# khiner/MeshEditor

Hardware: AMD Instinct MI355X
Metric: eigenpairs/sec (K/M assembly + 50-mode solve, 100k-tet mesh) (higher is better)
Workload: dtype f64; 1 GPU; cube_s100k: Kuhn mesh 105456 tets / 446631 DOF, NumModes=50 NumFemModes=65, P=10 excitation points, one mesh per GPU; eigenpairs_per_mesh=65, kept_modes_per_mesh=50, parallelism=mesh-per-gpu x1

## Files before the change

### mesheditor_amd/csrc/mh_common.h

```cpp
#pragma once
#include "../../include/modalhip.h"

#include <hip/hip_runtime.h>
#include <rocblas/rocblas.h>
#include <rocsolver/rocsolver.h>

#include <algorithm>
#include <cstdarg>
#include <cstdio>
#include <cstdlib>
#include <cstring>
#include <iterator>
#include <limits>
#include <map>
#include <mutex>
#include <stdexcept>
#include <string>
#include <vector>

struct MhError : std::runtime_error {
    int code;
    MhError(int c, const std::string &m) : std::runtime_error(m), code(c) {}
};

// ... 322 lines not shown
        if (ptr && ctx) ctx->pool.release(ptr);
        ptr = nullptr;
        count = 0;
    }
    T *get() const { return ptr; }
    operator T *() const { return ptr; }
    void zero() const { if (ptr) HIP_CHECK(hipMemsetAsync(ptr, 0, count * sizeof(T), ctx->stream)); }
    void upload(const T *src, size_t n) const { HIP_CHECK(hipMemcpyAsync(ptr, src, n * sizeof(T), hipMemcpyHostToDevice, ctx->stream)); }
    void download(T *dst, size_t n) const {
        HIP_CHECK(hipMemcpyAsync(dst, ptr, n * sizeof(T), hipMemcpyDeviceToHost, ctx->stream));
        HIP_CHECK(hipStreamSynchronize(ctx->stream));
    }
    std::vector<T> to_host() const {
        std::vector<T> h(count);
        if (count) download(h.data(), count);
        return h;
    }
};

struct mh_mesh {
    mh_context *ctx;
    uint32_t n_points{0}, n_tets{0};
    DevArray<double> points;
    DevArray<uint32_t> tets;
};

struct BsrLevel {
    int id{0};
    uint32_t n_nodes{0};
    uint64_t n_blocks{0};
    DevArray<uint32_t> row_ptr;
    DevArray<uint32_t> col;
    DevArray<double> kval;
    DevArray<double> mval;
    DevArray<double> aval;
    DevArray<double> dinv;
    DevArray<float> aval32, dinv32;
    double lmax{0};
};

struct PatchSet {
    uint32_t npe{0}, n_patches{0}, n_touched{0};
    DevArray<uint32_t> nodes;
    DevArray<double> inv64;
    DevArray<double> weight;
    DevArray<int> dropped;
    DevArray<float> inv32;
    DevArray<uint32_t> touched, t_ptr, t_patch, t_local;
    uint32_t n_clusters{0}, cluster_rows{0}, cluster_tiles{0};
    uint32_t n_bad_elements{0};
    uint32_t largest_cluster{0};
    std::vector<uint32_t> h_cluster_ptr;
    DevArray<uint32_t> cluster_row;
    DevArray<uint32_t> cluster_ptr;
    DevArray<uint64_t> cluster_inv_ptr;
    DevArray<uint32_t> tile_cluster, tile_row0;
    DevArray<double> cinv64;
    DevArray<float> cinv32;
    bool any() const { return n_patches || n_clusters; }
    static constexpr int kClusterSlices = 8;
    size_t scratch_rows() const { return size_t(n_patches) * 3 * npe + size_t(cluster_rows) * kClusterSlices; }
};

struct mh_system {
    mh_context *ctx;
    uint32_t dropped_patches[2]{0, 0};
    double plain_residual{-1.0};
    mh_material material{};
    uint32_t n_points{0}, kept_tets{0}, n_nodes{0}, n_edges{0};
    bool lmax_widened{false};
    DevArray<double> points;
    DevArray<uint32_t> elem_nodes_ref;
    DevArray<uint32_t> elem_nodes;
    DevArray<double> elem_basis;
    DevArray<uint32_t> perm;
    DevArray<uint32_t> inv_perm;
    DevArray<double> node_xyz;
    DevArray<uint32_t> parent_a, parent_b;
    DevArray<uint32_t> p1_edge_ptr, p1_edge_mid;
    DevArray<uint32_t> p1_corner;
    DevArray<double> p1_xyz;
    BsrLevel L2, L1;
    uint32_t agg_target{16}, n_agg{0};
    DevArray<uint32_t> agg_of, agg_ptr, agg_nodes;
    DevArray<double> agg_t;
    DevArray<double> a0;
    uint32_t n_components{1};
    uint32_t unreferenced_points{0};
    DevArray<uint32_t> node_component;
    DevArray<double> component_centroid;
    PatchSet patches2, patches1;
    DevArray<uint32_t> elem_p1;
    float worst_quality{1.f};
    double sigma_built{0};
    bool hierarchy_ready{false};
    hipEvent_t coarse_done{nullptr};
    bool coarse_pending{false};
    double coarse_lift{0};
    DevArray<double> coarse_ws[5];
    DevArray<int> coarse_info;
    ~mh_system() {
        if (coarse_pending && coarse_done) (void)hipEventSynchronize(coarse_done);
        if (coarse_done) (void)hipEventDestroy(coarse_done);
    }
    DevArray<double> evecs;
    uint32_t evec_cols{0};
    mh_profile profile{};
};

inline int mh_guard(mh_context *ctx, const std::exception &e) {
    if (ctx) ctx->last_error = e.what();
    if (auto *m = dynamic_cast<const MhError *>(&e)) return m->code;
    return MH_EHIP;
}

#define MH_TRY(ctx_expr, body)                         \
    mh_context *ctx_guard_ = (ctx_expr);               \
    try {                                              \
        body;                                          \
        return MH_OK;                                  \
    } catch (const std::exception &e) {                \
        return mh_guard(ctx_guard_, e);                \
    }

inline unsigned div_up(size_t a, size_t b) { return unsigned((a + b - 1) / b); }

void mh_phase_shared_lock(int device);
void mh_phase_shared_unlock(int device);
struct MhSharedPhase {
    const int device;
    explicit MhSharedPhase(int dev) : device(dev) { mh_phase_shared_lock(device); }
    ~MhSharedPhase() { mh_phase_shared_unlock(device); }
    MhSharedPhase(const MhSharedPhase &) = delete;
    MhSharedPhase &operator=(const MhSharedPhase &) = delete;
};
std::mutex &mh_solve_mutex();
void mh_build_system(mh_context *ctx, const mh_mesh *mesh, const mh_material &mat, mh_system *sys);
void mh_build_hierarchy(mh_system *sys, double sigma, bool defer = false);
void mh_finish_hierarchy(mh_system *sys);
uint32_t mh_shift_invert_panel(mh_system *sys, double sigma, const double *b, double *x, uint32_t w, double rel_tol, uint32_t max_iters, double *worst_rel);
struct MhCycleShape {
    int deg2{2}, deg1{5}, gamma{3};
    double ratio{8.0}, ratio1{0.0};
};
void mh_cycle_shape(const mh_system *sys, uint32_t w, MhCycleShape *shape);
double mh_coarse_lift(const mh_system *sys);
void mh_precondition_panel(mh_system *sys, double sigma, int precision, const double *r, double *z, uint32_t w);
uint32_t mh_graph_aggregates(const std::vector<uint32_t> &row_ptr, const std::vector<uint32_t> &col, uint32_t n, uint32_t target, uint32_t max_order, std::vector<uint32_t> &agg_of);
void mh_select_patches(mh_system *sys, float threshold);
void mh_build_patch_inverses(mh_context *ctx, const BsrLevel &lvl, PatchSet &ps);
template<typename T>
void mh_apply_patches(mh_context *ctx, const PatchSet &ps, const T *in, const T *minus, uint32_t w, T coef, T *d, T *x, double *z, uint32_t wz, T *scratch);
void mh_gram(mh_context *ctx, size_t n, const double *x, uint32_t wa, const double *y, uint32_t wb, double *g, uint32_t ld, uint32_t ldy = 0, const uint32_t *ymap = nullptr);
void mh_combine(mh_context *ctx, size_t n, const double *x, uint32_t wx, const double *w, uint32_t ww, const double *p, uint32_t wp, const double *ct, uint32_t nc,
                double *out1, uint32_t n1, double *out2, bool accumulate = false, uint32_t ldx = 0, const uint32_t *xmap = nullptr, uint32_t ld1 = 0,
                const uint32_t *omap = nullptr, uint32_t col_begin = 0, uint32_t col_count = 0);
bool mh_tridiag_lowest_wide(mh_context *ctx, const double *d, const double *e, uint32_t m, uint32_t k, double *w, double *z, uint32_t ldz, double *work, int *info2,
                            double *quality_host);
void mh_apply_q(mh_context *ctx, const double *a, const double *tau, uint32_t m, double *z, uint32_t ldz, uint32_t ncols);
bool mh_tridiag_lowest(mh_context *ctx, const double *d, const double *e, uint32_t m, uint32_t k, double *w, double *z, uint32_t ldz, double *ufac,
                       double *quality, double *lam_scratch);
struct MhRrTrace {
    enum Reduction { GIVEN_IDENTITY = 0, MEASURED_IDENTITY = 1, SERIES = 2, CHOLESKY = 3 };
    enum Solver { SYEVD = 0, SMALL_PARTIAL = 1, SMALL_STEDC = 2, WIDE_PARTIAL = 3, WIDE_STEDC_ORMTR = 4 };
    int reduction{-1};
    double defect{-1};
    int solver{-1};
    double quality{std::numeric_limits<double>::quiet_NaN()};
};
int mh_rr_solve(mh_context *ctx, double *gA, double *gM, uint32_t m, double *evals, double *ework, DevArray<int> &info, uint32_t nwant = 0, bool gm_is_identity = false,
                std::vector<double> *host_evals = nullptr);
void mh_spd_inverse_small(mh_context *ctx, const double *a, uint32_t lda, uint32_t w, double *out, uint32_t ldo, int *info);
void mh_potrf(mh_context *ctx, double *a, uint32_t ld, uint32_t w, int *info);
void mh_potrf_small(mh_context *ctx, double *a, uint32_t w, int *info);
void mh_potrf_small_inverse(mh_context *ctx, double *a, uint32_t w, int *info, const double *dscale, double *linv);
bool mh_sytrd_gave_up(mh_context *ctx);
void mh_sytrd_wide(mh_context *ctx, double *a, uint32_t m, double *d, double *e, double *tau);
void mh_sytrd_small(mh_context *ctx, double *a, uint32_t m, double *d, double *e, double *tau, int variant = -1);
void mh_small_gemm(mh_context *ctx, bool ta, bool tb, uint32_t M, uint32_t N, uint32_t K, double alpha, const double *a, uint32_t lda, const double *b, uint32_t ldb, double beta, double *c,
                   uint32_t ldc);
void mh_short_product(mh_context *ctx, size_t n, const double *a, uint32_t m, const double *ct, uint32_t nc, double *out, double *partial, uint32_t slices);
void mh_pack_stacked(mh_context *ctx, const double *c1, uint32_t r1, const double *c2, uint32_t r2, uint32_t cols, double scale, double *ct);
void mh_pack_coefficients(mh_context *ctx, const double *c1, uint32_t n1, const double *c2, uint32_t n2, uint32_t m, uint32_t ld, double *ct);
void mh_spmm_mapped(mh_context *ctx, const BsrLevel &lvl, const double *vals9, const double *x, double *y, const double *mscal, double *y2, uint32_t w, uint32_t ldy,
                    uint32_t wreal, const uint32_t *omap, const double *res_theta = nullptr, double *res_out = nullptr, double *res_partial = nullptr,
                    const double *res_dinv = nullptr);
bool mh_spmm_f32_cheb_step(mh_context *ctx, const BsrLevel &lvl, const float *d_in, float *d_out, float *r, float *x, const float *dinv, float c1, float c2,
                           uint32_t w);
void mh_spmm_f32(mh_context *ctx, const BsrLevel &lvl, const float *x, float *y, uint32_t w);
void mh_spmm_mixed(mh_context *ctx, const BsrLevel &lvl, const float *x, double *y, uint32_t w);
const uint32_t *mh_identity_map(mh_context *ctx);
void mh_spmm(mh_context *ctx, const BsrLevel &lvl, const double *vals9, const double *x, double *y, const double *mscal, double *y2, uint32_t w);
```

### mesheditor_amd/csrc/mh_dense.hip

```cpp
#include "mh_common.h"

#include <optional>

#include <map>

struct PerDeviceOnce {
    static constexpr int MaxDevices = 64;
    std::once_flag flag[MaxDevices];
    template<typename F> void run(int device, F &&f) { std::call_once(flag[device >= 0 && device < MaxDevices ? device : 0], std::forward<F>(f)); }
};

static bool mh_test_own_gemm() {
    static const bool on = getenv("MH_TEST") && strstr(getenv("MH_TEST"), "own_gemm");
    return on;
}
namespace {
constexpr int KC = 32;

typedef double double4_t __attribute__((ext_vector_type(4)));

__host__ __device__ inline int pad_pitch(int w) {
    int p = ((w + 15) / 16) * 16;
    if ((p % 32) != 16) p += 16;
    return p;
// ... 17 lines not shown
#pragma unroll
        for (int j = 0; j < TJ; ++j) acc[i][j] = double4_t{0, 0, 0, 0};
    const size_t r_begin = size_t(blockIdx.x) * rows_per_wg;
    const size_t r_end = min(n, r_begin + rows_per_wg);
    const int kk_lane = lane >> 4, c_lane = lane & 15;
    constexpr int RPP = NTH / 16;
    static_assert(KC % RPP == 0 || RPP > KC, "staging passes");
    constexpr int PASSES = RPP >= KC ? 1 : KC / RPP;
    const int srow = tid >> 4, scol = tid & 15;
    const bool stager = srow < KC;
    const uint32_t xpitch = uint32_t(ldx) * 8u, ypitch = uint32_t(ldy) * 8u;
    uint32_t xoff[CA], yoff[CB];
#pragma unroll
    for (int c = 0; c < CA; ++c) xoff[c] = uint32_t(min(scol + 16 * c, wa - 1)) * 8u;
#pragma unroll
    for (int c = 0; c < CB; ++c) {
        const int col = min(scol + 16 * c, wb - 1);
        yoff[c] = (ymap ? ymap[col] : uint32_t(col)) * 8u;
    }
    double px[PASSES][CA], py[PASSES][CB];
    auto fetch = [&](size_t r0) {
        const char *xb = reinterpret_cast<const char *>(X + r0 * size_t(ldx)), *yb = reinterpret_cast<const char *>(Y + r0 * size_t(ldy));
        if (r0 + KC <= r_end) {
#pragma unroll
            for (int ps = 0; ps < PASSES; ++ps) {
                const uint32_t xr = uint32_t(stager ? ps * RPP + srow : 0) * xpitch, yr = uint32_t(stager ? ps * RPP + srow : 0) * ypitch;
#pragma unroll
                for (int c = 0; c < CA; ++c) px[ps][c] = *reinterpret_cast<const double *>(xb + size_t(xr + xoff[c]));
#pragma unroll
                for (int c = 0; c < CB; ++c) py[ps][c] = *reinterpret_cast<const double *>(yb + size_t(yr + yoff[c]));
            }
        } else {
#pragma unroll
            for (int ps = 0; ps < PASSES; ++ps) {
                const int k = ps * RPP + srow;
                const uint32_t row = (stager && r0 + k < r_end) ? uint32_t(k) : 0u;
#pragma unroll
                for (int c = 0; c < CA; ++c) px[ps][c] = *reinterpret_cast<const double *>(xb + size_t(row * xpitch + xoff[c]));
#pragma unroll
                for (int c = 0; c < CB; ++c) py[ps][c] = *reinterpret_cast<const double *>(yb + size_t(row * ypitch + yoff[c]));
            }
        }
    };
    auto commit = [&](size_t r0) {
        if (!stager) return;
        if (r0 + KC <= r_end) {
#pragma unroll
            for (int ps = 0; ps < PASSES; ++ps) {
                const int k = ps * RPP + srow;
#pragma unroll
                for (int c = 0; c < CA; ++c) Xs[k * PA + scol + 16 * c] = px[ps][c];
#pragma unroll
                for (int c = 0; c < CB; ++c) Ys[k * PB + scol + 16 * c] = py[ps][c];
            }
        } else {
#pragma unroll
            for (int ps = 0; ps < PASSES; ++ps) {
                const int k = ps * RPP + srow;
                const bool rok = r0 + k < r_end;
#pragma unroll
                for (int c = 0; c < CA; ++c) Xs[k * PA + scol + 16 * c] = rok ? px[ps][c] : 0.0;
#pragma unroll
                for (int c = 0; c < CB; ++c) Ys[k * PB + scol + 16 * c] = rok ? py[ps][c] : 0.0;
            }
        }
    };
    if (r_begin < r_end) fetch(r_begin);
    for (size_t r0 = r_begin; r0 < r_end; r0 += KC) {
        commit(r0);
        __syncthreads();
        if (r0 + KC < r_end) fetch(r0 + KC);
        __builtin_amdgcn_sched_barrier(0);
#pragma unroll
        for (int step = 0; step < KC / (4 * KS); ++step) {
            const int kk = 4 * (ks + KS * step);
            const double *xr = Xs + (kk + kk_lane) * PA + ti0 * 16 + c_lane;
            const double *yr = Ys + (kk + kk_lane) * PB + tj0 * 16 + c_lane;
            double af[TI], bf[TJ];
#pragma unroll
            for (int i = 0; i < TI; ++i) af[i] = xr[i * 16];
#pragma unroll
            for (int j = 0; j < TJ; ++j) bf[j] = yr[j * 16];
#pragma unroll
            for (int i = 0; i < TI; ++i)
#pragma unroll
                for (int j = 0; j < TJ; ++j) acc[i][j] = __builtin_amdgcn_mfma_f64_16x16x4f64(af[i], bf[j], acc[i][j], 0, 0, 0);
        }
        __builtin_amdgcn_sched_barrier(0);
        __syncthreads();
    }
    if (KS > 1) {
        double *fold = smem + size_t(gi * GJ + gj) * (TI * TJ * 256);
        for (int src = 1; src < KS; ++src) {
            if (ks == src) {
#pragma unroll
                for (int i = 0; i < TI; ++i)
#pragma unroll
                    for (int j = 0; j < TJ; ++j)
#pragma unroll
                        for (int reg = 0; reg < 4; ++reg) fold[((i * TJ + j) * 4 + reg) * 64 + lane] = acc[i][j][reg];
            }
            __syncthreads();
            if (ks == 0) {
#pragma unroll
                for (int i = 0; i < TI; ++i)
#pragma unroll
                    for (int j = 0; j < TJ; ++j)
#pragma unroll
                        for (int reg = 0; reg < 4; ++reg) acc[i][j][reg] += fold[((i * TJ + j) * 4 + reg) * 64 + lane];
            }
            __syncthreads();
        }
    }
    if (ks != 0) return;
    double *out = partial + size_t(blockIdx.x) * wa * wb;
#pragma unroll
    for (int i = 0; i < TI; ++i) {
#pragma unroll
        for (int j = 0; j < TJ; ++j) {
            const int col = (tj0 + j) * 16 + c_lane;
#pragma unroll
            for (int reg = 0; reg < 4; ++reg) {
                const int row = (ti0 + i) * 16 + kk_lane + 4 * reg;
                if (row < wa && col < wb) out[size_t(col) * wa + row] = acc[i][j][reg];
            }
        }
    }
}

__global__ void __launch_bounds__(1024) k_gram_reduce(const double *__restrict__ partial, int nwg, int wa, int wb, double *__restrict__ g, int ld) {
    __shared__ double s[16][64];
    const int lane = threadIdx.x & 63, wv = threadIdx.x >> 6, idx = blockIdx.x * 64 + lane, total = wa * wb;
    double acc = 0;
    if (idx < total) {
#pragma unroll 8
        for (int w = wv; w < nwg; w += 16) acc += partial[size_t(w) * total + idx];
    }
    s[wv][lane] = acc;
    __syncthreads();
    if (wv == 0 && idx < total) {
        double t = 0;
#pragma unroll
        for (int k = 0; k < 16; ++k) t += s[k][lane];
        g[size_t(idx / wa) * ld + idx % wa] = t;
    }
}

typedef __attribute__((address_space(1))) double GlobalDouble;
constexpr int CK = 16;
template<int NT, bool ACCUMULATE, bool MAPPED>
__global__ void __launch_bounds__(256) k_combine(const double *__restrict__ X, int wx, int ldx, const uint32_t *__restrict__ xmap, const double *__restrict__ W, int ww,
                                                const double *__restrict__ P, int wp,
                                                const double *__restrict__ Ct, int ldc, int c0, int nc, size_t n, double *__restrict__ out1, int n1,
                                                double *__restrict__ out2, size_t split_stride, int ld1, const uint32_t *__restrict__ omap) {
    extern __shared__ __attribute__((aligned(16))) double smem[];
    const int m = wx + ww + wp;
    const int kslice = (((m + int(gridDim.y) - 1) / int(gridDim.y)) + CK - 1) / CK * CK;
    const int kb = int(blockIdx.y) * kslice, ke = min(m, kb + kslice);
    if (gridDim.y > 1) out1 += size_t(blockIdx.y) * split_stride;
    constexpr int CP = (NT * 16) % 32 == 16 ? NT * 16 : NT * 16 + 16;
    constexpr int SP = CK + 2;
    constexpr int STAGE = 64 * SP + CK * CP;
    unsigned long long *kaddr = reinterpret_cast<unsigned long long *>(smem + 2 * STAGE);
    uint32_t *kpitch = reinterpret_cast<uint32_t *>(kaddr + (ke - kb + CK));
    for (int i = threadIdx.x; i < ke - kb + CK; i += 256) {
        const int k = min(kb + i, m - 1);
        const double *base = X;
        int col = MAPPED ? (k < wx ? int(xmap[k]) : 0) : k, pitch = ldx;
        if (k >= wx + ww) base = P, col = k - wx - ww, pitch = wp;
        else if (k >= wx) base = W, col = k - wx, pitch = ww;
        kaddr[i] = reinterpret_cast<unsigned long long>(base + col);
        kpitch[i] = uint32_t(pitch) * 8u;
    }
    __syncthreads();
    const int tid = threadIdx.x, lane = tid & 63, wave = tid >> 6;
    static_assert(CK == 16, "one pass of 16 coefficient rows per chunk");
    constexpr int SJ = CK / 4;
    const int srow = tid >> 2, sk = (tid & 3) * SJ;
    const int ck = tid >> 4, cc = tid & 15;
    const char *cbytes = reinterpret_cast<const char *>(Ct + c0);
    const uint32_t row_bytes = uint32_t(ldc) * 8u;
    const uint32_t coff = uint32_t(ck) * row_bytes + uint32_t(cc) * 8u;
    const uint32_t ctail0 = uint32_t(ck) * row_bytes + uint32_t(min(cc + 16 * (NT - 2), nc - 1)) * 8u, ctail1 = uint32_t(ck) * row_bytes + uint32_t(min(cc + 16 * (NT - 1), nc - 1)) * 8u;
    const int col_l = lane & 15, row_l = lane >> 4;
    const int pitch2 = ldc - n1;
    uint32_t ocol[MAPPED ? NT : 1];
    if (MAPPED) {
#pragma unroll
        for (int t = 0; t < NT; ++t) ocol[t] = omap[min(c0 + 16 * t + col_l, max(n1, 1) - 1)] * 8u;
    }
    double ps[SJ], pc[NT];
    const size_t tiles = (n + 63) / 64;
    for (size_t tile = blockIdx.x; tile < tiles; tile += gridDim.x) {
        const size_t r0 = tile * 64;
        const uint32_t rs = uint32_t(min(r0 + srow, n - 1));
        double4_t acc[NT];
#pragma unroll
        for (int t = 0; t < NT; ++t) acc[t] = double4_t{0, 0, 0, 0};
        auto fetch = [&](int k0) {
#pragma unroll
            for (int j = 0; j < SJ; ++j) {
                const int i = k0 - kb + sk + j;
                ps[j] = *reinterpret_cast<const GlobalDouble *>(kaddr[i] + (unsigned long long)(rs) * kpitch[i]);
            }
            const char *cchunk = cbytes + size_t(k0) * row_bytes;
            uint32_t o = coff, o0 = ctail0, o1 = ctail1;
            if (k0 + CK > m) {
                const uint32_t back = uint32_t(ck - min(ck, m - 1 - k0)) * row_bytes;
                o -= back, o0 -= back, o1 -= back;
            }
#pragma unroll
            for (int t = 0; t < NT; ++t) pc[t] = *reinterpret_cast<const double *>(cchunk + (t < NT - 2 ? size_t(o) + 128 * t : size_t(t == NT - 2 ? o0 : o1)));
        };
        auto commit = [&](int k0, double *stage) {
            double *Ss = stage + srow * SP + sk, *Cs = stage + 64 * SP + ck * CP + cc;
            if (k0 + CK <= ke) {
#pragma unroll
                for (int j = 0; j < SJ; ++j) Ss[j] = ps[j];
            } else {
#pragma unroll
                for (int j = 0; j < SJ; ++j) Ss[j] = k0 + sk + j < ke ? ps[j] : 0.0;
            }
#pragma unroll
            for (int t = 0; t < NT; ++t) Cs[16 * t] = pc[t];
        };
        auto chunk = [&](int k0, int B) {
            const bool more = k0 + CK < ke;
            if (more) fetch(k0 + CK);
            const double *Ss = smem + B * STAGE, *Cs = Ss + 64 * SP;
#pragma unroll
            for (int kk = 0; kk < CK; kk += 4) {
                const double a = Ss[(wave * 16 + col_l) * SP + kk + row_l];
                const double *brow = Cs + (kk + row_l) * CP + col_l;
                double bf[NT];
#pragma unroll
                for (int t = 0; t < NT; ++t) bf[t] = brow[t * 16];
#pragma unroll
                for (int t = 0; t < NT; ++t) acc[t] = __builtin_amdgcn_mfma_f64_16x16x4f64(a, bf[t], acc[t], 0, 0, 0);
            }
            if (more) commit(k0 + CK, smem + (B ^ 1) * STAGE);
            __syncthreads();
        };
        if (kb < ke) {
            fetch(kb);
            commit(kb, smem);
        }
        __syncthreads();
        for (int k0 = kb, buf = 0; k0 < ke; k0 += CK, buf ^= 1) chunk(k0, buf);
#pragma unroll
        for (int reg = 0; reg < 4; ++reg) {
            const size_t r = r0 + wave * 16 + row_l + 4 * reg;
            if (r >= n) continue;
            char *row1 = reinterpret_cast<char *>(out1 + r * size_t(ld1)) + (MAPPED ? 0 : (c0 + col_l) * 8);
            char *row2 = reinterpret_cast<char *>(out2 + r * size_t(pitch2)) + (c0 + col_l - n1) * 8;
#pragma unroll
            for (int t = 0; t < NT; ++t) {
                if (t >= NT - 2 && t * 16 + col_l >= nc) continue;
                const int s0 = c0 + 16 * t;
                double *dst;
                if (s0 + 16 <= n1) dst = reinterpret_cast<double *>(row1 + (MAPPED ? size_t(ocol[t]) : size_t(128 * t)));
                else if (s0 >= n1) dst = reinterpret_cast<double *>(row2 + 128 * t);
                else dst = s0 + col_l < n1 ? reinterpret_cast<double *>(row1 + (MAPPED ? size_t(ocol[t]) : size_t(128 * t))) : reinterpret_cast<double *>(row2 + 128 * t);
                *dst = ACCUMULATE ? *dst + acc[t][reg] : acc[t][reg];
            }
        }
    }
}
__global__ void k_transpose_small(const double *__restrict__ c, int rows, int cols, int ld, double *__restrict__ ct, int col_off, int ct_cols, double scale = 1.0) {
    const int i = blockIdx.x * blockDim.x + threadIdx.x;
    if (i >= rows * cols) return;
    const int r = i % rows, cc = i / rows;
    ct[size_t(r) * ct_cols + col_off + cc] = scale * c[size_t(cc) * ld + r];
}
}

namespace {
void gram_block(mh_context *ctx, size_t n, const double *x, uint32_t ldx, uint32_t wa, const double *y, uint32_t ldy, const uint32_t *ymap, uint32_t wb, double *g,
                uint32_t ld) {
    const int ti_n = int((wa + 15) / 16), tj_n = int((wb + 15) / 16);
    constexpr size_t nwg_cap = 512;
    int nwg = int(std::min<size_t>(nwg_cap, (n + KC - 1) / KC));
    size_t rows_per_wg = ((n + nwg - 1) / nwg + KC - 1) / KC * KC;
    nwg = int((n + rows_per_wg - 1) / rows_per_wg);
    const size_t need = size_t(nwg) * wa * wb * sizeof(double);
    if (ctx->gram_ws_bytes < need) {
        ctx->pool.release(ctx->gram_ws);
        ctx->gram_ws = ctx->pool.alloc(need + need / 4);
        ctx->gram_ws_bytes = need + need / 4;
    }
    double *workspace = static_cast<double *>(ctx->gram_ws);
    auto blocked = [&](auto ti, auto tj, auto gi, auto gj, auto ks, auto occ) {
        constexpr int TI = decltype(ti)::value, TJ = decltype(tj)::value, GI = decltype(gi)::value, GJ = decltype(gj)::value, KS = decltype(ks)::value, OCC = decltype(occ)::value;
        constexpr int CA = TI * GI, CB = TJ * GJ;
        constexpr int PA = (CA * 16) % 32 == 16 ? CA * 16 : CA * 16 + 16, PB = (CB * 16) % 32 == 16 ? CB * 16 : CB * 16 + 16;
        const size_t fold = KS > 1 ? size_t(GI * GJ) * TI * TJ * 256 * sizeof(double) : 0;
        const size_t bytes = std::max(size_t(KC) * (PA + PB) * sizeof(double), fold);
        static PerDeviceOnce attr;
        attr.run(ctx->device, [] { HIP_CHECK(hipFuncSetAttribute(reinterpret_cast<const void *>(&k_gram_blocked<TI, TJ, GI, GJ, KS, OCC>), hipFuncAttributeMaxDynamicSharedMemorySize, 160 * 1024)); });
        k_gram_blocked<TI, TJ, GI, GJ, KS, OCC><<<nwg, GI * GJ * KS * 64, bytes, ctx->stream>>>(x, int(ldx), int(wa), y, int(ldy), ymap, int(wb), n, rows_per_wg, workspace);
    };
#define IC(v) std::integral_constant<int, v>{}
    if (ti_n <= 1 && tj_n <= 1) blocked(IC(1), IC(1), IC(1), IC(1), IC(4), IC(2));
    else if (ti_n <= 2 && tj_n <= 2) blocked(IC(2), IC(2), IC(1), IC(1), IC(4), IC(2));
    else if (ti_n <= 3 && tj_n <= 3) blocked(IC(3), IC(3), IC(1), IC(1), IC(4), IC(2));
    else if (ti_n <= 4 && tj_n <= 4) blocked(IC(4), IC(4), IC(1), IC(1), IC(4), IC(2));
    else if (ti_n <= 5 && tj_n <= 3) blocked(IC(5), IC(3), IC(1), IC(1), IC(4), IC(2));
    else if (ti_n <= 3 && tj_n <= 5) blocked(IC(3), IC(5), IC(1), IC(1), IC(4), IC(2));
    else if (ti_n <= 5 && tj_n <= 6) blocked(IC(5), IC(3), IC(1), IC(2), IC(2), IC(2));
    else if (ti_n <= 6 && tj_n <= 5) blocked(IC(3), IC(5), IC(2), IC(1), IC(2), IC(2));
    else if (ti_n <= 10 && tj_n <= 6) blocked(IC(5), IC(3), IC(2), IC(2), IC(1), IC(2));
    else if (ti_n <= 6 && tj_n <= 10) blocked(IC(3), IC(5), IC(2), IC(2), IC(1), IC(2));
    else mh_throw(MH_EINVAL, "gram block %u x %u too wide", wa, wb);
#undef IC
    KERNEL_CHECK();
    k_gram_reduce<<<div_up(size_t(wa) * wb, 64), 1024, 0, ctx->stream>>>(workspace, nwg, int(wa), int(wb), g, int(ld));
    KERNEL_CHECK();
}
}

void mh_gram(mh_context *ctx, size_t n, const double *x, uint32_t wa, const double *y, uint32_t wb, double *g, uint32_t ld, uint32_t ldy, const uint32_t *ymap) {
    if (!wa || !wb) return;
    if (!ldy) ldy = wb;
    if (wa >= 128 && wb >= 128 && n >= 65536 && !ymap && !mh_test_own_gemm()) {
        const uint32_t slabs = 128;
        const size_t rows = n / slabs, rest = n - rows * slabs;
        const size_t members = slabs + (rest ? 1 : 0), need = members * size_t(wa) * wb * sizeof(double);
        if (ctx->gram_ws_bytes < need) {
            ctx->pool.release(ctx->gram_ws);
            ctx->gram_ws = ctx->pool.alloc(need + need / 4);
            ctx->gram_ws_bytes = need + need / 4;
        }
        double *ws = static_cast<double *>(ctx->gram_ws);
        const double one = 1, zero = 0;
        ROCBLAS_CHECK(rocblas_dgemm_strided_batched(ctx->blas, rocblas_operation_none, rocblas_operation_transpose, rocblas_int(wa), rocblas_int(wb), rocblas_int(rows), &one, x,
                                                    rocblas_int(wa), rocblas_stride(rows * wa), y, rocblas_int(ldy), rocblas_stride(rows * ldy), &zero, ws, rocblas_int(wa),
                                                    rocblas_stride(size_t(wa) * wb), rocblas_int(slabs)));
        if (rest)
            ROCBLAS_CHECK(rocblas_dgemm(ctx->blas, rocblas_operation_none, rocblas_operation_transpose, rocblas_int(wa), rocblas_int(wb), rocblas_int(rest), &one, x + rows * slabs * wa,
                                        rocblas_int(wa), y + rows * slabs * ldy, rocblas_int(ldy), &zero, ws + size_t(slabs) * wa * wb, rocblas_int(wa)));
        k_gram_reduce<<<div_up(size_t(wa) * wb, 64), 1024, 0, ctx->stream>>>(ws, int(members), int(wa), int(wb), g, int(ld));
        KERNEL_CHECK();
        return;
    }
    const bool a_long = wa >= wb;
    const uint32_t cap_long = 160, cap_short = 96;
    const uint32_t w_long = a_long ? wa : wb, w_short = a_long ? wb : wa;
    const uint32_t n_short = div_up(w_short, cap_short), step_short = (div_up(w_short, n_short) + 15) / 16 * 16;
    const uint32_t rest = w_long % cap_long, n_long = div_up(w_long, cap_long);
    const uint32_t step_long = rest && rest < 32 ? (div_up(w_long, n_long) + 15) / 16 * 16 : cap_long;
    for (uint32_t l0 = 0; l0 < w_long; l0 += step_long)
        for (uint32_t s0 = 0; s0 < w_short; s0 += step_short) {
            const uint32_t i0 = a_long ? l0 : s0, j0 = a_long ? s0 : l0;
            const uint32_t ca = std::min(a_long ? step_long : step_short, wa - i0), cb = std::min(a_long ? step_short : step_long, wb - j0);
            gram_block(ctx, n, x + i0, wa, ca, ymap ? y : y + j0, ldy, ymap ? ymap + j0 : nullptr, cb, g + size_t(j0) * ld + i0, ld);
        }
}

void mh_pack_coefficients(mh_context *ctx, const double *c1, uint32_t n1, const double *c2, uint32_t n2, uint32_t m, uint32_t ld, double *ct) {
    if (n1) {
        k_transpose_small<<<div_up(size_t(m) * n1, 256), 256, 0, ctx->stream>>>(c1, int(m), int(n1), int(ld), ct, 0, int(n1 + n2));
        KERNEL_CHECK();
    }
    if (n2) {
        k_transpose_small<<<div_up(size_t(m) * n2, 256), 256, 0, ctx->stream>>>(c2, int(m), int(n2), int(ld), ct, int(n1), int(n1 + n2));
        KERNEL_CHECK();
    }
}

namespace {
__global__ void k_spread_rows(const double *__restrict__ ct, const uint32_t *__restrict__ xmap, uint32_t wx, uint32_t nc, double *__restrict__ full) {
    const size_t i = size_t(blockIdx.x) * blockDim.x + threadIdx.x;
    if (i >= size_t(wx) * nc) return;
    full[size_t(xmap[i / nc]) * nc + i % nc] = ct[i];
}
__global__ void k_iota(uint32_t *p, uint32_t n) {
    const uint32_t i = blockIdx.x * blockDim.x + threadIdx.x;
    if (i < n) p[i] = i;
}
}

namespace {
template<int NT, bool ACCUMULATE, bool MAPPED> int combine_residency(mh_context *ctx, size_t lds) {
    static PerDeviceOnce attr;
    attr.run(ctx->device, [] { HIP_CHECK(hipFuncSetAttribute(reinterpret_cast<const void *>(&k_combine<NT, ACCUMULATE, MAPPED>), hipFuncAttributeMaxDynamicSharedMemorySize, 160 * 1024)); });
    static std::mutex guard;
    static std::map<std::pair<int, size_t>, int> known;
    std::lock_guard<std::mutex> lock(guard);
    auto [it, fresh] = known.try_emplace({ctx->device, lds >> 12}, 1);
    if (fresh) {
        int nb = 0;
        if (hipOccupancyMaxActiveBlocksPerMultiprocessor(&nb, reinterpret_cast<const void *>(&k_combine<NT, ACCUMULATE, MAPPED>), 256, ((lds >> 12) + 1) << 12) == hipSuccess && nb > 0) it->second = std::min(nb, 8);
    }
    return it->second;
}
}

const uint32_t *mh_identity_map(mh_context *ctx) {
    if (!ctx->iota) {
        ctx->iota = static_cast<uint32_t *>(ctx->pool.alloc(1024 * sizeof(uint32_t)));
        k_iota<<<4, 256, 0, ctx->stream>>>(ctx->iota, 1024);
        KERNEL_CHECK();
    }
    return ctx->iota;
}

void mh_combine(mh_context *ctx, size_t n, const double *x, uint32_t wx, const double *w, uint32_t ww, const double *p, uint32_t wp, const double *ct, uint32_t nc,
                double *out1, uint32_t n1, double *out2, bool accumulate, uint32_t ldx, const uint32_t *xmap, uint32_t ld1, const uint32_t *omap, uint32_t col_begin,
                uint32_t col_count) {
    if (!nc) return;
    if (!col_count) { col_begin = 0; col_count = nc; }
    const bool caller_omap = omap != nullptr;
    if (col_begin + col_count > nc) mh_throw(MH_EINVAL, "combine: columns %u + %u exceed %u", col_begin, col_count, nc);
    const bool mapped = xmap != nullptr;
    if (mapped && accumulate) mh_throw(MH_EINVAL, "combine: column maps are not supported with accumulate");
    if (mapped && !omap) {
        if (n1 > 1024) mh_throw(MH_EINVAL, "combine: %u mapped output columns exceed 1024", n1);
        omap = mh_identity_map(ctx);
    }
    constexpr bool wide_blas = true;
    const uint32_t m_total = wx + ww + wp;
    TimedLaunch timed(ctx, MH_KERNEL_COMBINE, 2.0 * double(n) * double(m_total) * double(col_count));
    std::optional<TimedLaunch> timed_full;
    if (m_total >= 200 && col_count >= 128) timed_full.emplace(ctx, MH_KERNEL_COMBINE_FULL, 2.0 * double(n) * double(m_total) * double(col_count));
    if (ctx->time_kernels) ctx->totals[MH_KERNEL_COMBINE_BYTES].work += 8.0 * double(n) * (double(m_total) + double(col_count)), ctx->totals[MH_KERNEL_COMBINE_BYTES].launches += 1;
    if (wide_blas && !mh_test_own_gemm() && m_total >= 400 && col_count >= 128 && !caller_omap && out1 != x && out2 != x && n >= 65536) {
        const uint32_t px = ldx ? ldx : wx;
        const double *cx = ct;
        DevArray<double> ct_full;
        if (mapped) {
            ct_full.reset(ctx, size_t(px) * nc);
            ct_full.zero();
            k_spread_rows<<<div_up(size_t(wx) * nc, 256), 256, 0, ctx->stream>>>(ct, xmap, wx, nc, ct_full.get());
            KERNEL_CHECK();
            cx = ct_full.get();
        }
        const double one = 1, zero = 0;
        struct Part { const double *panel; uint32_t width, pitch; const double *coeff; };
        const Part parts[3] = {{x, mapped ? px : wx, px, cx}, {w, ww, ww, ct + size_t(wx) * nc}, {p, wp, wp, ct + size_t(wx + ww) * nc}};
        auto emit = [&](double *out, uint32_t pitch, uint32_t c_begin, uint32_t c_count) {
            if (!c_count) return;
            bool first = true;
            for (const Part &part : parts) {
                if (!part.panel || !part.width) continue;
                ROCBLAS_CHECK(rocblas_dgemm(ctx->blas, rocblas_operation_none, rocblas_operation_none, rocblas_int(c_count), rocblas_int(n), rocblas_int(part.width), &one,
                                            part.coeff + c_begin, rocblas_int(nc), part.panel, rocblas_int(part.pitch), (first && !accumulate) ? &zero : &one, out, rocblas_int(pitch)));
                first = false;
            }
        };
        const uint32_t c_end = col_begin + col_count;
        if (col_begin < n1) emit(out1 + col_begin, ld1 ? ld1 : n1, col_begin, std::min(c_end, n1) - col_begin);
        if (c_end > n1) emit(out2 + (std::max(col_begin, n1) - n1), nc - n1, std::max(col_begin, n1), c_end - std::max(col_begin, n1));
        if (mapped) HIP_CHECK(hipStreamSynchronize(ctx->stream));
        return;
    }
    const uint32_t chunks = div_up(col_count, 256), step = (div_up(col_count, chunks) + 15) / 16 * 16;
    for (uint32_t c0 = col_begin; c0 < col_begin + col_count; c0 += step) {
        const uint32_t ncc = std::min(step, col_begin + col_count - c0);
        auto go = [&](auto nt_tag) {
            constexpr int NT = decltype(nt_tag)::value;
            constexpr int CP = (NT * 16) % 32 == 16 ? NT * 16 : NT * 16 + 16;
            const size_t lds = 2 * (size_t(64) * (CK + 2) + size_t(CK) * CP) * sizeof(double) + size_t(m_total + CK) * 12;
            const size_t lds_m = lds;
            const int per_cu = accumulate ? combine_residency<NT, true, false>(ctx, lds) : mapped ? combine_residency<NT, false, true>(ctx, lds) : combine_residency<NT, false, false>(ctx, lds);
            const unsigned grid = unsigned(std::min<size_t>(div_up(n, 64), size_t(per_cu) * ctx->cu_count));
#define MH_COMBINE_ARGS x, int(wx), int(ldx ? ldx : wx), xmap, w, int(ww), p, int(wp), ct, int(nc), int(c0), int(ncc), n, out1, int(n1), out2, 0, int(ld1 ? ld1 : n1), omap
            if (accumulate) k_combine<NT, true, false><<<grid, 256, lds, ctx->stream>>>(MH_COMBINE_ARGS);
            else if (mapped) k_combine<NT, false, true><<<grid, 256, lds_m, ctx->stream>>>(MH_COMBINE_ARGS);
            else k_combine<NT, false, false><<<grid, 256, lds, ctx->stream>>>(MH_COMBINE_ARGS);
#undef MH_COMBINE_ARGS
        };
        const int ntile = int((ncc + 15) / 16);
        switch ((ntile + 1) / 2) {
            case 1: go(std::integral_constant<int, 2>{}); break;
            case 2: go(std::integral_constant<int, 4>{}); break;
            case 3: go(std::integral_constant<int, 6>{}); break;
            case 4: go(std::integral_constant<int, 8>{}); break;
            case 5: go(std::integral_constant<int, 10>{}); break;
            case 6: go(std::integral_constant<int, 12>{}); break;
            case 7: go(std::integral_constant<int, 14>{}); break;
            default: go(std::integral_constant<int, 16>{}); break;
        }
        KERNEL_CHECK();
    }
}

namespace {
__global__ void k_sum_slices(const double *__restrict__ partial, int slices, size_t count, double *__restrict__ out) {
    const size_t i = size_t(blockIdx.x) * blockDim.x + threadIdx.x;
    if (i >= count) return;
    double s = 0;
    for (int q = 0; q < slices; ++q) s += partial[size_t(q) * count + i];
    out[i] = s;
}
}

void mh_short_product(mh_context *ctx, size_t n, const double *a, uint32_t m, const double *ct, uint32_t nc, double *out, double *partial, uint32_t slices) {
    if (!nc || !n) return;
    if (nc > 256) mh_throw(MH_EINVAL, "short product: %u columns exceed 256", nc);
    const size_t stride = n * nc;
    auto go = [&](auto nt_tag) {
        constexpr int NT = decltype(nt_tag)::value;
        constexpr int CP = (NT * 16) % 32 == 16 ? NT * 16 : NT * 16 + 16;
        const uint32_t kslice = (div_up(m, slices) + CK - 1) / CK * CK;
        const size_t lds = 2 * (size_t(64) * (CK + 2) + size_t(CK) * CP) * sizeof(double) + size_t(std::min(kslice, m) + CK) * 12;
        if (lds > 160 * 1024) mh_throw(MH_EINVAL, "short product: %u basis columns per slice exceed the staging table", kslice);
        (void)combine_residency<NT, false, false>(ctx, lds);
        const dim3 grid(div_up(n, 64), slices);
        k_combine<NT, false, false><<<grid, 256, lds, ctx->stream>>>(a, int(m), int(m), nullptr, nullptr, 0, nullptr, 0, ct, int(nc), 0, int(nc), n, slices > 1 ? partial : out, int(nc), nullptr, stride,
                                                             int(nc), nullptr);
    };
    const int ntile = int((nc + 15) / 16);
    switch ((ntile + 1) / 2) {
        case 1: go(std::integral_constant<int, 2>{}); break;
        case 2: go(std::integral_constant<int, 4>{}); break;
        case 3: go(std::integral_constant<int, 6>{}); break;
        case 4: go(std::integral_constant<int, 8>{}); break;
        case 5: go(std::integral_constant<int, 10>{}); break;
        case 6: go(std::integral_constant<int, 12>{}); break;
        case 7: go(std::integral_constant<int, 14>{}); break;
        default: go(std::integral_constant<int, 16>{}); break;
    }
    KERNEL_CHECK();
    if (slices > 1) {
        k_sum_slices<<<div_up(stride, 256), 256, 0, ctx->stream>>>(partial, int(slices), stride, out);
        KERNEL_CHECK();
    }
}

void mh_pack_stacked(mh_context *ctx, const double *c1, uint32_t r1, const double *c2, uint32_t r2, uint32_t cols, double scale, double *ct) {
    if (r1) {
        k_transpose_small<<<div_up(size_t(r1) * cols, 256), 256, 0, ctx->stream>>>(c1, int(r1), int(cols), int(r1), ct, 0, int(cols), scale);
        KERNEL_CHECK();
    }
    if (r2) {
        k_transpose_small<<<div_up(size_t(r2) * cols, 256), 256, 0, ctx->stream>>>(c2, int(r2), int(cols), int(r2), ct + size_t(r1) * cols, 0, int(cols), scale);
        KERNEL_CHECK();
    }
}

namespace {
__device__ inline double wave_sum_lds(const double *buf, int count, int lane) {
    double s = 0.0;
#pragma unroll
    for (int q = 0; q < 4; ++q) {
        const int i = lane + 64 * q;
        s += i < count ? buf[i] : 0.0;
    }
    return mh_wave_sum(s);
}

__global__ void __launch_bounds__(1024) k_sytrd_small(double *__restrict__ A, int m, double *__restrict__ D, double *__restrict__ E, double *__restrict__ TAU) {
    __shared__ double xs[256], v[256], wv[256], sq[256], part[1024];
    const int tid = threadIdx.x, lane = tid & 63;
    for (int k = 0; k + 1 < m; ++k) {
        const int l = m - k - 1;
        int rb = 32;
        while (rb < l) rb <<= 1;
        const int ng = 1024 / rb, rr = tid & (rb - 1), cq = tid / rb;
        double *col = A + size_t(k) * m + (k + 1);
        if (tid < l) {
            const double x = col[tid];
            xs[tid] = x;
            sq[tid] = tid >= 1 ? x * x : 0.0;
        }
        __syncthreads();
        const double xnorm2 = wave_sum_lds(sq, l, lane);
        const double alpha = xs[0];
        double tau = 0.0, beta = alpha, scale = 0.0;
        if (xnorm2 > 0.0) {
            beta = -copysign(sqrt(alpha * alpha + xnorm2), alpha);
            tau = (beta - alpha) / beta;
            scale = 1.0 / (alpha - beta);
        }
        if (tid == 0) {
            D[k] = A[size_t(k) * m + k];
            E[k] = beta;
            TAU[k] = tau;
        }
        if (tau == 0.0) {
            __syncthreads();
            continue;
        }
        if (tid < l) {
            const double vi = tid == 0 ? 1.0 : xs[tid] * scale;
            v[tid] = vi;
            col[tid] = tid == 0 ? beta : vi;
        }
        __syncthreads();
        double *a22 = A + size_t(k + 1) * m + (k + 1);
        double acc = 0.0;
        if (rr < l)
            for (int c = cq; c < l; c += ng) acc += a22[size_t(c) * m + rr] * v[c];
        part[cq * rb + rr] = acc;
        __syncthreads();
        double p = 0.0;
        if (tid < l) {
            double sum = 0.0;
            for (int g = 0; g < ng; ++g) sum += part[g * rb + tid];
            p = tau * sum;
            sq[tid] = p * v[tid];
        }
        __syncthreads();
        const double pv = wave_sum_lds(sq, l, lane);
        if (tid < l) wv[tid] = p - 0.5 * tau * pv * v[tid];
        __syncthreads();
        if (rr < l) {
            const double vr = v[rr], wr = wv[rr];
            double *arow = a22 + rr;
            for (int c = cq; c < l; c += ng) arow[size_t(c) * m] -= vr * wv[c] + wr * v[c];
        }
        __syncthreads();
    }
    if (tid == 0) {
        D[m - 1] = A[size_t(m - 1) * m + (m - 1)];
        TAU[m - 1] = 0.0;
    }
}
}

#ifndef MH_SYTRD_THREADS
#define MH_SYTRD_THREADS 1024
#endif
__global__ void __launch_bounds__(MH_SYTRD_THREADS) k_sytrd_small_fused(double *__restrict__ A, int m, double *__restrict__ D, double *__restrict__ E, double *__restrict__ TAU) {
    __shared__ double xs[256], v[256], vp[256], wp[256], sq[256], xnext[256], part[MH_SYTRD_THREADS];
    const int tid = threadIdx.x, lane = tid & 63;
    bool pending = false;
    for (int k = 0; k + 1 < m; ++k) {
        const int l = m - k - 1;
        int rb = 32;
        while (rb < l) rb <<= 1;
        const int ng = max(1, MH_SYTRD_THREADS / rb), rr = tid & (rb - 1), cq = tid / rb;
        double *col = A + size_t(k) * m + (k + 1);
        if (tid < l) {
            double x = pending ? xnext[tid + 1] : col[tid];
            if (pending) x -= vp[tid + 1] * wp[0] + wp[tid + 1] * vp[0];
            xs[tid] = x;
// ... 1502 lines not shown
```

### mesheditor_amd/csrc/mh_eigs.hip

```cpp
#include "mh_common.h"

#include <algorithm>
#include <cmath>
#include <memory>
#include <condition_variable>
#include <mutex>
#include <numeric>
#include <optional>
#include <type_traits>

__global__ void k_shift_values(const double *kval, const double *mval, size_t nblocks, double sigma, double *aval);
__global__ void k_diag_inverse(const uint32_t *row_ptr, const uint32_t *col, const double *aval, uint32_t nnodes, double *dinv);
__global__ void k_coarse_matrix(const uint32_t *row_ptr, const uint32_t *col, const double *aval, const double *tmat, const uint32_t *agg_of, const uint32_t *agg_ptr,
                                const uint32_t *agg_nodes, uint32_t nagg, double *a0);
__global__ void k_fix_coarse_diag(double *a0, uint32_t n0, double rel);

namespace {
constexpr int TB = 256;

std::mutex g_solve_mutex;
struct Switches {
    bool verbose = getenv("MH_VERBOSE") != nullptr;
    bool fp32_prec = !(getenv("MH_PRECOND_FP64") && atoi(getenv("MH_PRECOND_FP64")) != 0);
    int deg2 = 0, deg1 = 0, gamma = 0;
    double cheb_ratio = 0.0, cheb_ratio1 = 0.0;
    bool test_sytrd_giveup = getenv("MH_TEST") && strstr(getenv("MH_TEST"), "sytrd_giveup");
    bool no_tridiag_wide = getenv("MH_TEST") && strstr(getenv("MH_TEST"), "no_tridiag_wide");
    bool test_last_resort = getenv("MH_TEST") && strstr(getenv("MH_TEST"), "last_resort");
    bool test_coarse_pivot = getenv("MH_TEST") && strstr(getenv("MH_TEST"), "coarse_pivot");
    bool test_selfcheck_fail = getenv("MH_TEST") && strstr(getenv("MH_TEST"), "selfcheck_fail");
    bool lmax_low = getenv("MH_TEST") && strstr(getenv("MH_TEST"), "lmax_low");
    bool potrf_chain = getenv("MH_TEST") && strstr(getenv("MH_TEST"), "potrf_chain");
    bool no_poly_start = getenv("MH_TEST") && strstr(getenv("MH_TEST"), "no_poly_start");
    Switches() {
        if (const char *c = getenv("MH_CYCLE")) {
            double v[5] = {0, 0, 0, 0, 0};
            sscanf(c, "%lf,%lf,%lf,%lf,%lf", &v[0], &v[1], &v[2], &v[3], &v[4]);
            deg2 = std::max(0, int(v[0])), deg1 = std::max(0, int(v[1])), gamma = std::max(0, int(v[2]));
            cheb_ratio = v[3];
            cheb_ratio1 = v[4];
        }
    }
};
const Switches &switches() {
    static const Switches s;
    return s;
}
constexpr int kPowerIterations = 20;
constexpr uint32_t kPrecondColumns = 256;
constexpr uint32_t kSkipP = 4;
constexpr uint32_t kGuardPercent = 10;
constexpr float kFlatShape = 1e-4f;
constexpr size_t kDenseLastResort = 12288;
constexpr int kLastResortCg = 8;

struct PhaseLock {
    std::mutex m;
    std::condition_variable cv;
    int readers = 0, writers_waiting = 0;
    bool writer = false;
    void lock_shared() {
        std::unique_lock<std::mutex> l(m);
        cv.wait(l, [&] { return !writer && writers_waiting == 0; });
        ++readers;
    }
    void unlock_shared() {
        std::unique_lock<std::mutex> l(m);
        if (--readers == 0) cv.notify_all();
    }
    void lock() {
        std::unique_lock<std::mutex> l(m);
        ++writers_waiting;
        cv.wait(l, [&] { return !writer && readers == 0; });
        --writers_waiting;
        writer = true;
    }
    void unlock() {
        std::unique_lock<std::mutex> l(m);
        writer = false;
        cv.notify_all();
    }
};
constexpr int kMaxDevices = 64;
PhaseLock g_phase_of_device[kMaxDevices];
PhaseLock &phase_of(int device) { return g_phase_of_device[unsigned(device) % kMaxDevices]; }
const bool g_concurrent = !(getenv("MH_CONCURRENT_SOLVES") && atoi(getenv("MH_CONCURRENT_SOLVES")) == 0);
struct SharedPhase {
    PhaseLock &phase;
    bool held = false, enabled = true;
    explicit SharedPhase(int device, bool on = true) : phase(phase_of(device)), enabled(on) { acquire(); }
    ~SharedPhase() { release(); }
    void acquire() { if (g_concurrent && enabled && !held) { phase.lock_shared(); held = true; } }
    void release() { if (held) { phase.unlock_shared(); held = false; } }
};
struct ExclusivePhase {
    PhaseLock &phase;
    bool held = false;
    explicit ExclusivePhase(int device) : phase(phase_of(device)) {
        if (g_concurrent) {
            phase.lock();
            held = true;
            (void)hipSetDevice(device);
            (void)hipDeviceSynchronize();
        }
    }
    ~ExclusivePhase() { if (held) phase.unlock(); }
};

struct Timer {
    mh_context *ctx;
    hipEvent_t a, b;
    explicit Timer(mh_context *c) : ctx(c) {
        HIP_CHECK(hipEventCreate(&a));
        HIP_CHECK(hipEventCreate(&b));
        HIP_CHECK(hipEventRecord(a, ctx->stream));
    }
    double stop() {
        HIP_CHECK(hipEventRecord(b, ctx->stream));
        HIP_CHECK(hipEventSynchronize(b));
        float ms = 0;
        HIP_CHECK(hipEventElapsedTime(&ms, a, b));
        return ms * 1e-3;
    }
    ~Timer() {
        (void)hipEventDestroy(a);
        (void)hipEventDestroy(b);
    }
};

__global__ void k_random_panel(double *__restrict__ x, size_t count, uint64_t seed) {
    const size_t i = size_t(blockIdx.x) * blockDim.x + threadIdx.x;
    if (i >= count) return;
    auto mix = [](uint64_t z) {
        z += 0x9e3779b97f4a7c15ull;
        z = (z ^ (z >> 30)) * 0xbf58476d1ce4e5b9ull;
        z = (z ^ (z >> 27)) * 0x94d049bb133111ebull;
        return z ^ (z >> 31);
    };
    const uint64_t a = mix(seed + 2 * i), b = mix(seed + 2 * i + 1);
    const double u1 = (double(a >> 11) + 1.0) * (1.0 / 9007199254740993.0), u2 = double(b >> 11) * (1.0 / 9007199254740992.0);
    x[i] = sqrt(-2.0 * log(u1)) * cos(6.283185307179586 * u2);
}

template<typename T>
__global__ void k_cheb_init(const T *__restrict__ b, const T *__restrict__ t, const T *__restrict__ dinv, T inv_theta, T *__restrict__ r, T *__restrict__ d,
                            T *__restrict__ x, int accumulate, size_t rows, uint32_t w) {
    const size_t i = size_t(blockIdx.x) * blockDim.x + threadIdx.x;
    if (i >= rows * w) return;
    const T rv = t ? b[i] - t[i] : b[i];
    const T dv = dinv[i / w] * rv * inv_theta;
    r[i] = rv;
    d[i] = dv;
    x[i] = accumulate ? x[i] + dv : dv;
}
typedef float f4_t __attribute__((ext_vector_type(4)));
__global__ void k_cheb_init_v4(const f4_t *__restrict__ b, const f4_t *__restrict__ t, const float *__restrict__ dinv, float inv_theta, f4_t *__restrict__ r,
                               f4_t *__restrict__ d, f4_t *__restrict__ x, int accumulate, size_t rows, uint32_t w4) {
    const size_t i = size_t(blockIdx.x) * blockDim.x + threadIdx.x;
    if (i >= rows * w4) return;
    const f4_t rv = t ? b[i] - t[i] : b[i];
    const f4_t dv = (dinv[i / w4] * inv_theta) * rv;
    r[i] = rv;
    d[i] = dv;
    x[i] = accumulate ? x[i] + dv : dv;
}
__global__ void k_cheb_last_v4(const f4_t *__restrict__ t, const float *__restrict__ dinv, float c1, float c2, const f4_t *__restrict__ r, const f4_t *__restrict__ d,
                               const f4_t *__restrict__ x, double *__restrict__ z, size_t rows, uint32_t w4, uint32_t wo) {
    const size_t i = size_t(blockIdx.x) * blockDim.x + threadIdx.x;
    if (i >= rows * w4) return;
    const size_t row = i / w4;
    const uint32_t c = uint32_t(i % w4) * 4;
    const f4_t rv = r[i] - t[i];
    const f4_t zv = x[i] + (c1 * d[i] + (c2 * dinv[row]) * rv);
#pragma unroll
    for (int e = 0; e < 4; ++e)
        if (c + e < wo) z[row * wo + c + e] = double(zv[e]);
}
__global__ void k_prolong_p1_v4(const f4_t *__restrict__ x1, const uint32_t *__restrict__ pa, const uint32_t *__restrict__ pb, f4_t *__restrict__ x2, uint32_t nnodes,
                                uint32_t w4) {
    const size_t i = size_t(blockIdx.x) * blockDim.x + threadIdx.x;
    if (i >= size_t(nnodes) * 3 * w4) return;
    const uint32_t c = uint32_t(i % w4), comp = uint32_t((i / w4) % 3), node = uint32_t(i / (size_t(3) * w4));
    const uint32_t a = pa[node], bb = pb[node];
    const f4_t va = x1[(size_t(3) * a + comp) * w4 + c];
    x2[i] += a == bb ? va : 0.5f * (va + x1[(size_t(3) * bb + comp) * w4 + c]);
}
__global__ void k_cheb_init_convert(const double *__restrict__ src, uint32_t ws, const float *__restrict__ dinv, float inv_theta, float *__restrict__ b32,
                                    float *__restrict__ r, float *__restrict__ d, float *__restrict__ x, size_t rows, uint32_t w) {
    const size_t i = size_t(blockIdx.x) * blockDim.x + threadIdx.x;
    if (i >= rows * w) return;
    const size_t row = i / w;
    const uint32_t c = uint32_t(i % w);
    const float rv = c < ws ? float(src[row * ws + c]) : 0.f;
    const float dv = dinv[row] * rv * inv_theta;
    b32[i] = rv;
    r[i] = rv;
    d[i] = dv;
    x[i] = dv;
}
template<typename T>
__global__ void k_cheb_step(const T *__restrict__ t, const T *__restrict__ dinv, T c1, T c2, T *__restrict__ r, T *__restrict__ d, T *__restrict__ x, size_t rows,
                            uint32_t w) {
    const size_t i = size_t(blockIdx.x) * blockDim.x + threadIdx.x;
    if (i >= rows * w) return;
    const T rv = r[i] - t[i];
    const T dv = c1 * d[i] + c2 * dinv[i / w] * rv;
    r[i] = rv;
    d[i] = dv;
    x[i] += dv;
}
template<typename T>
__global__ void k_cheb_last(const T *__restrict__ t, const T *__restrict__ dinv, T c1, T c2, const T *__restrict__ r, const T *__restrict__ d, const T *__restrict__ x,
                            double *__restrict__ z, size_t rows, uint32_t w, uint32_t wo) {
    const size_t i = size_t(blockIdx.x) * blockDim.x + threadIdx.x;
    if (i >= rows * w) return;
    const size_t row = i / w;
    const uint32_t c = uint32_t(i % w);
    if (c >= wo) return;
    const T rv = r[i] - t[i];
    z[row * wo + c] = double(x[i] + (c1 * d[i] + c2 * dinv[row] * rv));
}
template<typename S, typename D> __global__ void k_convert(const S *__restrict__ src, D *__restrict__ dst, size_t count) {
    const size_t i = size_t(blockIdx.x) * blockDim.x + threadIdx.x;
    if (i < count) dst[i] = D(src[i]);
}
template<typename S, typename D> __global__ void k_convert_pitch(const S *__restrict__ src, uint32_t ws, D *__restrict__ dst, uint32_t wd, size_t rows) {
    const size_t i = size_t(blockIdx.x) * blockDim.x + threadIdx.x;
    if (i >= rows * wd) return;
    const size_t row = i / wd;
    const uint32_t c = uint32_t(i % wd);
    dst[i] = c < ws ? D(src[row * ws + c]) : D(0);
}

template<typename T>
__global__ void k_restrict_p1(const T *__restrict__ b, const T *__restrict__ t, const uint32_t *__restrict__ p1_corner, const uint32_t *__restrict__ eptr,
                              const uint32_t *__restrict__ emid, T *__restrict__ r1, uint32_t npts, uint32_t w, uint32_t wb = 0) {
    const size_t i = size_t(blockIdx.x) * blockDim.x + threadIdx.x;
    if (i >= size_t(npts) * 3 * w) return;
    const uint32_t c = uint32_t(i % w), comp = uint32_t((i / w) % 3), p = uint32_t(i / (size_t(3) * w));
    const uint32_t pb = wb ? wb : w;
    auto res = [&](uint32_t node) {
        const size_t row = size_t(3) * node + comp;
        return (c < pb ? b[row * pb + c] : T(0)) - t[row * w + c];
    };
    T s = res(p1_corner[p]);
    T h = 0;
    for (uint32_t e = eptr[p]; e < eptr[p + 1]; ++e) h += res(emid[e]);
    r1[i] = s + T(0.5) * h;
}
template<typename T>
__global__ void k_prolong_p1(const T *__restrict__ x1, const uint32_t *__restrict__ pa, const uint32_t *__restrict__ pb, T *__restrict__ x2, uint32_t nnodes,
                             uint32_t w) {
    const size_t i = size_t(blockIdx.x) * blockDim.x + threadIdx.x;
    if (i >= size_t(nnodes) * 3 * w) return;
    const uint32_t c = uint32_t(i % w), comp = uint32_t((i / w) % 3), node = uint32_t(i / (size_t(3) * w));
    const uint32_t a = pa[node], bb = pb[node];
    const T va = x1[(size_t(3) * a + comp) * w + c];
    x2[i] += a == bb ? va : T(0.5) * (va + x1[(size_t(3) * bb + comp) * w + c]);
}
template<typename T>
__global__ void k_restrict_agg(const T *__restrict__ b, const T *__restrict__ t, const double *__restrict__ tmat, double *__restrict__ r0,
                               const uint32_t *__restrict__ agg_ptr, const uint32_t *__restrict__ agg_nodes, uint32_t nagg, uint32_t w) {
    const size_t i = size_t(blockIdx.x) * blockDim.x + threadIdx.x;
    if (i >= size_t(nagg) * 6 * w) return;
    const uint32_t c = uint32_t(i % w), q = uint32_t((i / w) % 6), a = uint32_t(i / (size_t(6) * w));
    double s = 0;
    for (uint32_t l = agg_ptr[a]; l < agg_ptr[a + 1]; ++l) {
        const uint32_t nd = agg_nodes[l];
        const double *tm = tmat + 18 * size_t(nd);
        for (int p = 0; p < 3; ++p) {
            const size_t o = (size_t(3) * nd + p) * w + c;
            s += tm[6 * p + q] * double(b[o] - t[o]);
        }
    }
    r0[i] = s;
}
template<typename T>
__global__ void k_prolong_agg(const double *__restrict__ x0, const double *__restrict__ tmat, T *__restrict__ x1, const uint32_t *__restrict__ agg_of, uint32_t npts,
                              uint32_t w) {
    const size_t i = size_t(blockIdx.x) * blockDim.x + threadIdx.x;
    if (i >= size_t(npts) * 3 * w) return;
    const uint32_t c = uint32_t(i % w), p = uint32_t((i / w) % 3), nd = uint32_t(i / (size_t(3) * w));
    const uint32_t a = agg_of[nd];
    const double *tm = tmat + 18 * size_t(nd) + 6 * p;
    double s = 0;
    for (int q = 0; q < 6; ++q) s += tm[q] * x0[(size_t(6) * a + q) * w + c];
    x1[i] += T(s);
}

__global__ void k_residual(const double *__restrict__ ax, const double *__restrict__ mx, const double *__restrict__ theta, const uint32_t *__restrict__ idx,
                           double *__restrict__ r, size_t rows, uint32_t b, uint32_t w) {
    const size_t i = size_t(blockIdx.x) * blockDim.x + threadIdx.x;
    if (i >= rows * w) return;
    const uint32_t k = uint32_t(i % w);
    const size_t row = i / w;
    const uint32_t src = idx ? idx[k] : k;
    r[i] = ax[row * b + src] - theta[src] * mx[row * b + src];
}

__global__ void k_residual_norms(const double *__restrict__ ax, const double *__restrict__ mx, const double *__restrict__ xx, const double *__restrict__ theta,
                                 double near_limit, double *__restrict__ r, size_t rows, uint32_t b, uint32_t rows_per_block, double *__restrict__ partial,
                                 const double *__restrict__ dinv) {
    const uint32_t c = blockIdx.y * blockDim.x + threadIdx.x;
    if (c >= b) return;
    const size_t r0 = size_t(blockIdx.x) * rows_per_block, r1 = min(rows, r0 + rows_per_block);
    const double th = theta[c];
    const bool need_x = fabs(th) < near_limit;
    double sr = 0, sm = 0, sx = 0;
    for (size_t row = r0; row < r1; ++row) {
        const size_t i = row * b + c;
        const double m = mx[i], res = ax[i] - th * m;
        const double wgt = dinv ? dinv[row] : 1.0;
        r[i] = res;
        sr += res * res * wgt;
        sm += m * m * wgt;
        if (need_x) {
            const double x = xx[i];
            sx += dinv ? x * x / wgt : x * x;
        }
    }
    double *p = partial + size_t(blockIdx.x) * 3 * b;
    p[c] = sr;
    p[b + c] = sm;
    p[2 * size_t(b) + c] = sx;
}

__global__ void k_colsumsq_partial(const double *__restrict__ x, size_t rows, uint32_t w, double *__restrict__ partial, uint32_t rows_per_block) {
    const uint32_t c = blockIdx.y * blockDim.x + threadIdx.x;
    if (c >= w) return;
    const size_t r0 = size_t(blockIdx.x) * rows_per_block, r1 = min(rows, r0 + rows_per_block);
    double s = 0;
    for (size_t r = r0; r < r1; ++r) {
        const double v = x[r * w + c];
        s += v * v;
    }
    partial[size_t(blockIdx.x) * w + c] = s;
}
__global__ void k_colsum_partial(const double *__restrict__ x, size_t rows, uint32_t w, double *__restrict__ partial, uint32_t rows_per_block) {
    const uint32_t c = blockIdx.y * blockDim.x + threadIdx.x;
    if (c >= w) return;
    const size_t r0 = size_t(blockIdx.x) * rows_per_block, r1 = min(rows, r0 + rows_per_block);
    double s = 0;
    for (size_t r = r0; r < r1; ++r) s += x[r * w + c];
    partial[size_t(blockIdx.x) * w + c] = s;
}
__global__ void k_colsumsq_final(const double *__restrict__ partial, uint32_t nblocks, uint32_t w, double *__restrict__ out) {
    __shared__ double s[256];
    const uint32_t c = blockIdx.x;
    double acc = 0;
    for (uint32_t b = threadIdx.x; b < nblocks; b += 256) acc += partial[size_t(b) * w + c];
    s[threadIdx.x] = acc;
// ... 134 lines not shown
        for (int d = 2; d < 7; ++d) L[a][d] = ((2 * d - 1) * t[a] * L[a][d - 1] - (d - 1) * L[a][d - 2]) / d;
    }
    double *row[3] = {x + (size_t(3) * i) * b + col0, x + (size_t(3) * i + 1) * b + col0, x + (size_t(3) * i + 2) * b + col0};
    uint32_t col = 0;
    auto put = [&](double v0, double v1, double v2) {
        row[0][col] = v0, row[1][col] = v1, row[2][col] = v2;
        ++col;
    };
    put(t[0], 0, 0), put(0, t[1], 0), put(0, 0, t[2]), put(t[1], t[0], 0), put(t[2], 0, t[0]), put(0, t[2], t[1]);
    for (uint32_t q = 0; q < ntriples; ++q) {
        const uint32_t tr = triples[q];
        const double v = L[0][tr & 0xff] * L[1][(tr >> 8) & 0xff] * L[2][(tr >> 16) & 0xff];
        put(v, 0, 0), put(0, v, 0), put(0, 0, v);
    }
}
__global__ void k_copy_cols(const double *__restrict__ src, uint32_t wsrc, double *__restrict__ dst, uint32_t wdst, size_t rows, uint32_t ncols) {
    const size_t i = size_t(blockIdx.x) * blockDim.x + threadIdx.x;
    if (i >= rows * ncols) return;
    dst[(i / ncols) * wdst + i % ncols] = src[(i / ncols) * wsrc + i % ncols];
}
__global__ void k_bsr_to_dense(const uint32_t *__restrict__ row_ptr, const uint32_t *__restrict__ col, const double *__restrict__ v9, const double *__restrict__ ms,
                               uint32_t nnodes, double *__restrict__ a, double *__restrict__ m) {
    const uint32_t r = blockIdx.x * blockDim.x + threadIdx.x;
    if (r >= nnodes) return;
    const size_t n = size_t(3) * nnodes;
    for (uint32_t p = row_ptr[r]; p < row_ptr[r + 1]; ++p) {
        const uint32_t c = col[p];
        for (int i = 0; i < 3; ++i) {
            for (int j = 0; j < 3; ++j) a[(size_t(3) * c + j) * n + size_t(3) * r + i] = v9[9 * size_t(p) + 3 * i + j];
            m[(size_t(3) * c + i) * n + size_t(3) * r + i] = ms[p];
        }
    }
}
__global__ void k_colmajor_to_panel(const double *__restrict__ z, size_t n, uint32_t ncols, double *__restrict__ x) {
    const size_t i = size_t(blockIdx.x) * blockDim.x + threadIdx.x;
    if (i >= n * ncols) return;
    x[i] = z[size_t(i % ncols) * n + i / ncols];
}

__global__ void k_symmetrize_lower(double *__restrict__ a, uint32_t n, uint32_t ld) {
    const size_t i = size_t(blockIdx.x) * blockDim.x + threadIdx.x;
    if (i >= size_t(n) * n) return;
    const uint32_t r = uint32_t(i % n), c = uint32_t(i / n);
    if (r < c) a[size_t(c) * ld + r] = a[size_t(r) * ld + c];
}

unsigned grid1(size_t count) { return div_up(count, TB); }

void gram(mh_context *ctx, size_t n, const double *xa, uint32_t wa, const double *yb, uint32_t wb, double *g, uint32_t ld) {
    mh_gram(ctx, n, xa, wa, yb, wb, g, ld);
}
void panel_mul(mh_context *ctx, size_t n, const double *x, uint32_t wa, const double *c, uint32_t ld, double *z, uint32_t wz, double alpha, double beta) {
    if (!wz) return;
    if (!wa) return;
    ROCBLAS_CHECK(rocblas_dgemm(ctx->blas, rocblas_operation_transpose, rocblas_operation_none, wz, rocblas_int(n), wa, &alpha, c, ld, x, wa, &beta, z, wz));
}
void panel_trsm(mh_context *ctx, size_t n, double *wp, uint32_t w, const double *l, uint32_t ld) {
    const double one = 1;
    ROCBLAS_CHECK(rocblas_dtrsm(ctx->blas, rocblas_side_left, rocblas_fill_lower, rocblas_operation_none, rocblas_diagonal_non_unit, w, rocblas_int(n), &one, l, ld, wp, w));
}


void small_dgemm(mh_context *ctx, rocblas_operation ta, rocblas_operation tb, rocblas_int M, rocblas_int N, rocblas_int K, const double *alpha, const double *a, rocblas_int lda, const double *b,
                 rocblas_int ldb, const double *beta, double *c, rocblas_int ldc) {
    if (M <= 1024 && N <= 1024 && K <= 4096)
        mh_small_gemm(ctx, ta != rocblas_operation_none, tb != rocblas_operation_none, uint32_t(M), uint32_t(N), uint32_t(K), *alpha, a, uint32_t(lda), b, uint32_t(ldb), *beta, c, uint32_t(ldc));
    else
        ROCBLAS_CHECK(rocblas_dgemm(ctx->blas, ta, tb, M, N, K, alpha, a, lda, b, ldb, beta, c, ldc));
}

__global__ void k_identity_defect(const double *__restrict__ g, uint32_t m, unsigned long long *__restrict__ out) {
    const uint32_t i = blockIdx.x * blockDim.x + threadIdx.x;
    double d = 0;
    if (i < m * m) {
        const uint32_t r = i % m, c = i / m;
        if (r >= c) d = fabs(g[i] - (r == c ? 1.0 : 0.0));
    }
    for (int off = 32; off > 0; off >>= 1) d = fmax(d, __shfl_xor(d, off, 64));
    if ((threadIdx.x & 63) == 0 && d > 0) atomicMax(out, (unsigned long long)__double_as_longlong(d));
}

__global__ void k_defect_matrix(const double *__restrict__ g, uint32_t m, double *__restrict__ e) {
    const uint32_t i = blockIdx.x * blockDim.x + threadIdx.x;
    if (i >= m * m) return;
    const uint32_t r = i % m, c = i / m;
    e[i] = (r >= c ? g[i] : g[size_t(r) * m + c]) - (r == c ? 1.0 : 0.0);
}
__global__ void k_inverse_sqrt_series(const double *__restrict__ e, const double *__restrict__ e2, uint32_t m, double *__restrict__ s) {
    const uint32_t i = blockIdx.x * blockDim.x + threadIdx.x;
    if (i >= m * m) return;
    s[i] = (i % m == i / m ? 1.0 : 0.0) - 0.5 * e[i] + 0.375 * e2[i];
}

__global__ void __launch_bounds__(256) k_rr_selfcheck(const double *__restrict__ a, uint32_t m, const double *__restrict__ z, uint32_t ldz, const double *__restrict__ theta, uint32_t ncols,
                                                      unsigned long long *__restrict__ worst) {
    __shared__ double zs[768], red[3][256];
    const uint32_t tid = threadIdx.x, j = blockIdx.x == 0 ? 0 : (blockIdx.x == 1 ? ncols / 2 : ncols - 1);
    for (uint32_t i = tid; i < m; i += 256) zs[i] = z[size_t(j) * ldz + i];
    __syncthreads();
    const double th = theta[j];
    double rmax = 0, azmax = 0, zmax = 0;
    bool nan = false;
    for (uint32_t i = tid; i < m; i += 256) {
        double az = 0, abs_az = 0;
        for (uint32_t c = 0; c < m; ++c) {
            const double t = a[size_t(c) * m + i] * zs[c];
            az += t, abs_az += fabs(t);
        }
        const double r = az - th * zs[i];
        nan = nan || !(r == r);
        rmax = fmax(rmax, fabs(r)), azmax = fmax(azmax, abs_az), zmax = fmax(zmax, fabs(zs[i]));
    }
    red[0][tid] = nan ? INFINITY : rmax, red[1][tid] = azmax, red[2][tid] = zmax;
    __syncthreads();
    for (int h = 128; h > 0; h >>= 1) {
        if (tid < uint32_t(h))
            for (int q = 0; q < 3; ++q) red[q][tid] = fmax(red[q][tid], red[q][tid + h]);
        __syncthreads();
    }
    if (tid == 0) {
        const double rel = red[0][0] / fmax(red[1][0] + fabs(th) * red[2][0], 1e-300);
        atomicMax(worst, (unsigned long long)__double_as_longlong(rel == rel ? rel : INFINITY));
    }
}
void rr_selfcheck(mh_context *ctx, const double *saved, uint32_t m, const double *z, uint32_t ldz, const double *theta, uint32_t ncols) {
    if (!ncols) return;
    if (!ctx->rr_check) {
        ctx->rr_check = static_cast<unsigned long long *>(ctx->pool.alloc(256));
        HIP_CHECK(hipMemsetAsync(ctx->rr_check, 0, 256, ctx->stream));
    }
    k_rr_selfcheck<<<3, 256, 0, ctx->stream>>>(saved, m, z, ldz, theta, ncols, ctx->rr_check);
    KERNEL_CHECK();
}

int host_info(DevArray<int> &info) { int hinfo = 0; info.download(&hinfo, 1); return hinfo; }
bool sytrd_gave_up(mh_context *ctx, int flag, double *gA, const double *saved, uint32_t m) {
    if (!flag && !switches().test_sytrd_giveup) return false;
    ++ctx->sytrd_redos;
    HIP_CHECK(hipMemcpyAsync(gA, saved, size_t(m) * m * sizeof(double), hipMemcpyDeviceToDevice, ctx->stream));
    return true;
}
bool accept_partial(mh_context *ctx, double quality, double *evals, const double *lam, uint32_t nwant) {
    if (!(quality < 1e-10)) return false;
    HIP_CHECK(hipMemcpyAsync(evals, lam, size_t(nwant) * sizeof(double), hipMemcpyDeviceToDevice, ctx->stream));
    return true;
}

int eig_tridiag_small(mh_context *ctx, double *gA, uint32_t m, double *evals, double *ework, DevArray<int> &info, uint32_t nwant, std::vector<double> *host_evals) {
    DevArray<double> z(ctx, size_t(m) * m), tau(ctx, m);
    const bool partial = nwant && nwant < m;
    DevArray<double> zl(ctx, partial ? size_t(m) * nwant : 0);
    double *zres = z.get();
    uint32_t ncols = m;
    HIP_CHECK(hipMemcpyAsync(z.get(), gA, size_t(m) * m * sizeof(double), hipMemcpyDeviceToDevice, ctx->stream));
    for (int attempt = 0; attempt < 2; ++attempt) {
        mh_sytrd_small(ctx, gA, m, evals, ework, tau, attempt == 0 ? -1 : 0);
        int gave_up = 0;
        const bool flagged = attempt == 0 && ctx->sytrd_flag;
        if (flagged) HIP_CHECK(hipMemcpyAsync(&gave_up, ctx->sytrd_flag, sizeof(int), hipMemcpyDeviceToHost, ctx->stream));
        if (partial) {
            DevArray<double> wv(ctx, 2 * m + 8), ufac(ctx, size_t(3) * m * nwant);
            double *zout = attempt == 0 ? zl.get() : z.get();
            if (mh_tridiag_lowest(ctx, evals, ework, m, nwant, wv, zout, m, ufac, wv.get() + m, wv.get() + m + 8)) {
                double qv[5] = {1, 0, 0, 0, 0};
                std::vector<double> lam_host(host_evals ? nwant : 0);
                HIP_CHECK(hipMemcpyAsync(qv, wv.get() + m, sizeof(qv), hipMemcpyDeviceToHost, ctx->stream));
                if (host_evals) HIP_CHECK(hipMemcpyAsync(lam_host.data(), wv.get(), size_t(nwant) * sizeof(double), hipMemcpyDeviceToHost, ctx->stream));
                HIP_CHECK(hipStreamSynchronize(ctx->stream));
                if (flagged && sytrd_gave_up(ctx, gave_up, gA, z, m)) continue;
                if (switches().verbose)
                    fprintf(stderr, "[rr] tridiagonal m %u lowest %u: residual / ||T|| %.2e; us: multisection %.0f, inverse iteration %.0f, Gram-Schmidt %.0f, output %.0f\n", m,
                            nwant, qv[0], qv[1] * 0.01, qv[2] * 0.01, qv[3] * 0.01, qv[4] * 0.01);
                if (ctx->rr_trace) ctx->rr_trace->quality = qv[0];
                if (accept_partial(ctx, qv[0], evals, wv, nwant)) {
                    if (host_evals) host_evals->swap(lam_host);
                    zres = zout, ncols = nwant;
                    break;
                }
            }
        }
        if (flagged) {
            HIP_CHECK(hipStreamSynchronize(ctx->stream));
            if (sytrd_gave_up(ctx, gave_up, gA, z, m)) continue;
        }
        ROCBLAS_CHECK(rocsolver_dstedc(ctx->blas, rocblas_evect_tridiagonal, m, evals, ework, z, m, info));
        if (const int hinfo = host_info(info)) return hinfo;
        break;
    }
    if (ctx->rr_trace) ctx->rr_trace->solver = ncols < m ? MhRrTrace::SMALL_PARTIAL : MhRrTrace::SMALL_STEDC;
    mh_apply_q(ctx, gA, tau, m, zres, m, ncols);
    if (zres == zl.get()) rr_selfcheck(ctx, z.get(), m, zres, m, evals, ncols);
    HIP_CHECK(hipMemcpyAsync(gA, zres, size_t(m) * ncols * sizeof(double), hipMemcpyDeviceToDevice, ctx->stream));
    return 0;
}

std::optional<int> eig_tridiag_wide(mh_context *ctx, double *gA, uint32_t m, double *evals, double *ework, DevArray<int> &info, uint32_t nwant) {
    DevArray<double> z(ctx, size_t(m) * m), saved(ctx, size_t(m) * m), tau(ctx, m);
    HIP_CHECK(hipMemcpyAsync(saved.get(), gA, size_t(m) * m * sizeof(double), hipMemcpyDeviceToDevice, ctx->stream));
    mh_sytrd_wide(ctx, gA, m, evals, ework, tau);
    int gave_up = 0;
    HIP_CHECK(hipMemcpyAsync(&gave_up, ctx->sytrd_flag, sizeof(int), hipMemcpyDeviceToHost, ctx->stream));
    HIP_CHECK(hipStreamSynchronize(ctx->stream));
    if (sytrd_gave_up(ctx, gave_up, gA, saved, m)) return std::nullopt;
    if (nwant && nwant < m && nwant <= 256 && !switches().no_tridiag_wide) {
        DevArray<double> work(ctx, size_t(5) * nwant * m + size_t(2) * nwant * nwant + 8), lam(ctx, nwant);
        double quality = 1.0;
        if (mh_tridiag_lowest_wide(ctx, evals, ework, m, nwant, lam, z, m, work, info, &quality)) {
            if (switches().verbose) fprintf(stderr, "[rr] tridiagonal m %u lowest %u (wide): residual / ||T|| %.2e\n", m, nwant, quality);
            if (ctx->rr_trace) ctx->rr_trace->quality = quality;
            if (accept_partial(ctx, quality, evals, lam, nwant)) {
                if (ctx->rr_trace) ctx->rr_trace->solver = MhRrTrace::WIDE_PARTIAL;
                mh_apply_q(ctx, gA, tau, m, z, m, nwant);
                rr_selfcheck(ctx, saved.get(), m, z, m, evals, nwant);
                HIP_CHECK(hipMemcpyAsync(gA, z.get(), size_t(m) * nwant * sizeof(double), hipMemcpyDeviceToDevice, ctx->stream));
                HIP_CHECK(hipStreamSynchronize(ctx->stream));
                return 0;
            }
        }
    }
    ROCBLAS_CHECK(rocsolver_dstedc(ctx->blas, rocblas_evect_tridiagonal, m, evals, ework, z, m, info));
    if (const int hinfo = host_info(info)) return hinfo;
    ROCBLAS_CHECK(rocsolver_dormtr(ctx->blas, rocblas_side_left, rocblas_fill_lower, rocblas_operation_none, m, m, gA, m, tau, z, m));
    if (ctx->rr_trace) ctx->rr_trace->solver = MhRrTrace::WIDE_STEDC_ORMTR;
    HIP_CHECK(hipMemcpyAsync(gA, z.get(), size_t(m) * m * sizeof(double), hipMemcpyDeviceToDevice, ctx->stream));
    HIP_CHECK(hipStreamSynchronize(ctx->stream));
    return 0;
}

}

int mh_rr_solve(mh_context *ctx, double *gA, double *gM, uint32_t m, double *evals, double *ework, DevArray<int> &info, uint32_t nwant, bool gm_is_identity,
                std::vector<double> *host_evals) {
    const double one = 1, zero = 0;
    k_symmetrize_lower<<<grid1(size_t(m) * m), TB, 0, ctx->stream>>>(gA, m, m);
    KERNEL_CHECK();
    bool identity = gm_is_identity, series = false;
    if (!identity) {
        static_assert(sizeof(unsigned long long) == sizeof(double), "defect word");
        unsigned long long *defect = reinterpret_cast<unsigned long long *>(ework);
        HIP_CHECK(hipMemsetAsync(defect, 0, sizeof(unsigned long long), ctx->stream));
        k_identity_defect<<<grid1(size_t(m) * m), TB, 0, ctx->stream>>>(gM, m, defect);
        KERNEL_CHECK();
        unsigned long long bits = 0;
        HIP_CHECK(hipMemcpyAsync(&bits, defect, sizeof(bits), hipMemcpyDeviceToHost, ctx->stream));
        HIP_CHECK(hipStreamSynchronize(ctx->stream));
        double d;
        memcpy(&d, &bits, sizeof(d));
        identity = d < 1e-11;
        if (switches().verbose) fprintf(stderr, "[rr] m %u identity defect %.2e\n", m, d);
        series = !identity && d < 1e-7;
        if (ctx->rr_trace) ctx->rr_trace->defect = d;
    }
    if (ctx->rr_trace) ctx->rr_trace->reduction = gm_is_identity ? MhRrTrace::GIVEN_IDENTITY : identity ? MhRrTrace::MEASURED_IDENTITY : series ? MhRrTrace::SERIES : MhRrTrace::CHOLESKY;
    DevArray<double> sroot, stmp;
    if (series) {
        sroot.reset(ctx, size_t(m) * m);
        stmp.reset(ctx, size_t(m) * m * 2);
        double *e = stmp.get(), *e2 = stmp.get() + size_t(m) * m;
        k_defect_matrix<<<grid1(size_t(m) * m), TB, 0, ctx->stream>>>(gM, m, e);
        KERNEL_CHECK();
        small_dgemm(ctx, rocblas_operation_none, rocblas_operation_none, m, m, m, &one, e, m, e, m, &zero, e2, m);
        k_inverse_sqrt_series<<<grid1(size_t(m) * m), TB, 0, ctx->stream>>>(e, e2, m, sroot);
        KERNEL_CHECK();
        small_dgemm(ctx, rocblas_operation_none, rocblas_operation_none, m, m, m, &one, sroot, m, gA, m, &zero, e, m);
        small_dgemm(ctx, rocblas_operation_none, rocblas_operation_none, m, m, m, &one, e, m, sroot, m, &zero, gA, m);
        k_symmetrize_lower<<<grid1(size_t(m) * m), TB, 0, ctx->stream>>>(gA, m, m);
        KERNEL_CHECK();
        identity = true;
    }
    if (!identity) {
        mh_potrf(ctx, gM, m, m, info);
        if (const int hinfo = host_info(info)) return hinfo;
        ROCBLAS_CHECK(rocblas_dtrsm(ctx->blas, rocblas_side_left, rocblas_fill_lower, rocblas_operation_none, rocblas_diagonal_non_unit, m, m, &one, gM, m, gA, m));
        ROCBLAS_CHECK(rocblas_dtrsm(ctx->blas, rocblas_side_right, rocblas_fill_lower, rocblas_operation_transpose, rocblas_diagonal_non_unit, m, m, &one, gM, m, gA, m));
    }
    std::optional<int> hinfo;
    if (m >= 8 && m <= 256) hinfo = eig_tridiag_small(ctx, gA, m, evals, ework, info, nwant, host_evals);
    else if (m > 256 && m <= 768 && !ctx->exchange_disabled) hinfo = eig_tridiag_wide(ctx, gA, m, evals, ework, info, nwant);
    if (!hinfo) {
        ROCBLAS_CHECK(rocsolver_dsyevd(ctx->blas, rocblas_evect_original, rocblas_fill_lower, m, gA, m, evals, ework, info));
        hinfo = host_info(info);
        if (ctx->rr_trace) ctx->rr_trace->solver = MhRrTrace::SYEVD;
    }
    if (*hinfo != 0) return *hinfo;
    if (series) {
        small_dgemm(ctx, rocblas_operation_none, rocblas_operation_none, m, m, m, &one, sroot, m, gA, m, &zero, stmp, m);
        HIP_CHECK(hipMemcpyAsync(gA, stmp.get(), size_t(m) * m * sizeof(double), hipMemcpyDeviceToDevice, ctx->stream));
        HIP_CHECK(hipStreamSynchronize(ctx->stream));
    } else if (!identity)
        ROCBLAS_CHECK(rocblas_dtrsm(ctx->blas, rocblas_side_left, rocblas_fill_lower, rocblas_operation_transpose, rocblas_diagonal_non_unit, m, m, &one, gM, m, gA, m));
    return 0;
}

namespace {

void colsumsq(mh_context *ctx, const double *x, size_t rows, uint32_t w, double *out, DevArray<double> &scratch) {
    const uint32_t rpb = 256;
    const uint32_t nb = div_up(rows, rpb);
    if (scratch.count < size_t(nb) * w) scratch.reset(ctx, size_t(nb) * w);
    dim3 grid(nb, div_up(w, 64));
    k_colsumsq_partial<<<grid, 64, 0, ctx->stream>>>(x, rows, w, scratch, rpb);
    KERNEL_CHECK();
    k_colsumsq_final<<<w, 256, 0, ctx->stream>>>(scratch, nb, w, out);
    KERNEL_CHECK();
}

template<typename F> void precondition_in_slabs(mh_context *ctx, size_t n, const double *r, double *z, uint32_t w, F &&one) {
    if (w <= kPrecondColumns) return one(r, z, w);
    const hipStream_t st = ctx->stream;
    const uint32_t slabs = div_up(w, kPrecondColumns), step = (div_up(w, slabs) + 3u) & ~3u;
    if (w > 1024) mh_throw(MH_EINVAL, "a block of %u columns exceeds the 1 024 the column maps cover", w);
    DevArray<double> rs(ctx, n * step), zs(ctx, n * step);
    const uint32_t *iota = mh_identity_map(ctx);
    for (uint32_t c0 = 0; c0 < w; c0 += step) {
        const uint32_t wc = std::min(step, w - c0);
        k_gather_cols<<<grid1(n * wc), TB, 0, st>>>(r, iota + c0, rs.get(), n, w, wc);
        KERNEL_CHECK();
        one(rs, zs, wc);
        k_scatter_cols<<<grid1(n * wc), TB, 0, st>>>(zs.get(), iota + c0, z, n, w, wc);
        KERNEL_CHECK();
    }
    HIP_CHECK(hipStreamSynchronize(st));
}

template<typename T> struct Precond {
    mh_system *sys;
    mh_context *ctx;
    uint32_t wmax;
    int deg2, deg1, gamma;
    double ratio, ratio1;
    DevArray<T> rin, z2, d2, t2, r2, r1, x1, d1, t1, rr1;
    DevArray<double> r0, x0, x0_partial;
    static constexpr uint32_t COARSE_SLICES = 8;
    DevArray<double> t2d, r1d, t1d;
    DevArray<T> patch_y;
    static constexpr bool kDouble = std::is_same<T, double>::value;
    static uint32_t pitch(uint32_t w) { return kDouble ? w : (w + 3u) & ~3u; }
    Precond(mh_system *s, uint32_t w_in) : sys(s), ctx(s->ctx), wmax(w_in) {
        const uint32_t w = pitch(w_in);
        const size_t n2 = size_t(3) * s->n_nodes, n1 = size_t(3) * s->n_points, n0 = size_t(6) * s->n_agg;
        d2.reset(ctx, n2 * w); t2.reset(ctx, n2 * w); r2.reset(ctx, n2 * w); z2.reset(ctx, n2 * w);
        if (!kDouble) {
            rin.reset(ctx, n2 * w);
            t2d.reset(ctx, n2 * w);
            r1d.reset(ctx, n1 * w); t1d.reset(ctx, n1 * w);
        }
        r1.reset(ctx, n1 * w); x1.reset(ctx, n1 * w); d1.reset(ctx, n1 * w); t1.reset(ctx, n1 * w); rr1.reset(ctx, n1 * w);
        r0.reset(ctx, n0 * w);
        x0.reset(ctx, n0 * w);
        x0_partial.reset(ctx, n0 * w * COARSE_SLICES);
        patch_y.reset(ctx, std::max(s->patches2.scratch_rows(), s->patches1.scratch_rows()) * w);
        MhCycleShape shape;
        mh_cycle_shape(s, w_in, &shape);
        deg2 = shape.deg2, deg1 = shape.deg1, gamma = shape.gamma, ratio = shape.ratio, ratio1 = shape.ratio1;
    }
    void spmm(const BsrLevel &lvl, const T *x, T *y, uint32_t w) {
        if constexpr (kDouble) mh_spmm(ctx, lvl, lvl.aval, x, y, nullptr, nullptr, w);
        else mh_spmm_f32(ctx, lvl, x, y, w);
    }
    static const T *dinv_of(const BsrLevel &lvl) {
        if constexpr (kDouble) return lvl.dinv.get();
        else return lvl.dinv32.get();
    }
    const PatchSet &patches_of(const BsrLevel &lvl) const { return lvl.id == 2 ? sys->patches2 : sys->patches1; }
    void cheb(const BsrLevel &lvl, int deg, const T *b, T *x, bool zero_init, T *r, T *d, T *t, uint32_t w, double *z_out = nullptr, uint32_t w_out = 0,
              const double *b_src = nullptr, uint32_t w_src = 0, T *b_copy = nullptr) {
        const size_t rows = size_t(3) * lvl.n_nodes;
        const double lmax = lvl.lmax, lmin = lvl.lmax / (lvl.id == 1 && ratio1 > 0 ? ratio1 : ratio);
        const double theta = 0.5 * (lmax + lmin), delta = 0.5 * (lmax - lmin), sig = theta / delta;
        double rho = 1.0 / sig;
        const T *dinv = dinv_of(lvl);
        if (!zero_init) spmm(lvl, x, t, w);
        if constexpr (!kDouble) {
            if (b_src && zero_init) k_cheb_init_convert<<<grid1(rows * w), TB, 0, ctx->stream>>>(b_src, w_src, dinv, float(1.0 / theta), b_copy, r, d, x, rows, w);
            else k_cheb_init_v4<<<grid1(rows * (w / 4)), TB, 0, ctx->stream>>>(reinterpret_cast<const f4_t *>(b), zero_init ? nullptr : reinterpret_cast<const f4_t *>(t), dinv,
                                                                               float(1.0 / theta), reinterpret_cast<f4_t *>(r), reinterpret_cast<f4_t *>(d),
                                                                               reinterpret_cast<f4_t *>(x), zero_init ? 0 : 1, rows, w / 4);
        } else {
            k_cheb_init<T><<<grid1(rows * w), TB, 0, ctx->stream>>>(b, zero_init ? nullptr : t, dinv, T(1.0 / theta), r, d, x, zero_init ? 0 : 1, rows, w);
        }
        KERNEL_CHECK();
        const PatchSet &ps = patches_of(lvl);
        mh_apply_patches<T>(ctx, ps, r, nullptr, w, T(1.0 / theta), d, x, nullptr, 0, patch_y.get());
        constexpr bool fuse_steps = true;
        T *cur = d, *alt = t;
        for (int k = 1; k < deg; ++k) {
            const double rho_new = 1.0 / (2 * sig - rho);
            const bool last = z_out && k + 1 == deg;
            bool fused = false;
            if constexpr (!kDouble) {
                if (fuse_steps && !last) fused = mh_spmm_f32_cheb_step(ctx, lvl, cur, alt, r, x, dinv, float(rho_new * rho), float(2 * rho_new / delta), w);
            }
            if (fused) {
                std::swap(cur, alt);
                mh_apply_patches<T>(ctx, ps, r, nullptr, w, T(2 * rho_new / delta), cur, x, nullptr, 0, patch_y.get());
            } else {
                spmm(lvl, cur, alt, w);
                if (!last) {
                    k_cheb_step<T><<<grid1(rows * w), TB, 0, ctx->stream>>>(alt, dinv, T(rho_new * rho), T(2 * rho_new / delta), r, cur, x, rows, w);
                } else if constexpr (kDouble) {
                    k_cheb_last<T><<<grid1(rows * w), TB, 0, ctx->stream>>>(alt, dinv, T(rho_new * rho), T(2 * rho_new / delta), r, cur, x, z_out, rows, w, w_out);
                } else {
                    k_cheb_last_v4<<<grid1(rows * (w / 4)), TB, 0, ctx->stream>>>(reinterpret_cast<const f4_t *>(alt), dinv, float(rho_new * rho), float(2 * rho_new / delta),
                                                                             reinterpret_cast<const f4_t *>(r), reinterpret_cast<const f4_t *>(cur),
                                                                             reinterpret_cast<const f4_t *>(x), z_out, rows, w / 4, w_out);
                }
                KERNEL_CHECK();
                if (!last) mh_apply_patches<T>(ctx, ps, r, nullptr, w, T(2 * rho_new / delta), cur, x, nullptr, 0, patch_y.get());
                else mh_apply_patches<T>(ctx, ps, r, alt, w, T(2 * rho_new / delta), nullptr, nullptr, z_out, w_out, patch_y.get());
            }
            rho = rho_new;
        }
        if (z_out && deg == 1) {
            k_convert_pitch<T, double><<<grid1(rows * w_out), TB, 0, ctx->stream>>>(x, w, z_out, w_out, rows);
            KERNEL_CHECK();
        }
    }
    void apply(const double *r_in, double *z_out, uint32_t w_in) {
        mh_finish_hierarchy(sys);
        const uint32_t w = pitch(w_in);
        const uint32_t nn = sys->n_nodes, np = sys->n_points, na = sys->n_agg;
        const size_t n2 = size_t(3) * nn, n1 = size_t(3) * np, n0 = size_t(6) * na;
        const T *r;
        if constexpr (kDouble) r = r_in;
        else r = rin.get();
        T *z = z2.get();
        if constexpr (kDouble) cheb(sys->L2, deg2, r, z, true, r2, d2, t2, w);
        else cheb(sys->L2, deg2, r, z, true, r2, d2, t2, w, nullptr, 0, r_in, w_in, rin.get());
        if constexpr (kDouble) {
            spmm(sys->L2, z, t2, w);
            k_restrict_p1<double><<<grid1(n1 * w), TB, 0, ctx->stream>>>(r, t2.get(), sys->p1_corner, sys->p1_edge_ptr, sys->p1_edge_mid, r1.get(), np, w);
            KERNEL_CHECK();
        } else {
            mh_spmm_mixed(ctx, sys->L2, z, t2d, w);
            k_restrict_p1<double><<<grid1(n1 * w), TB, 0, ctx->stream>>>(r_in, t2d.get(), sys->p1_corner, sys->p1_edge_ptr, sys->p1_edge_mid, r1d.get(), np, w, w_in);
            KERNEL_CHECK();
            k_convert<double, T><<<grid1(n1 * w), TB, 0, ctx->stream>>>(r1d.get(), r1.get(), n1 * w);
            KERNEL_CHECK();
        }
        for (int g = 0; g < gamma; ++g) {
            cheb(sys->L1, deg1, r1, x1, g == 0, rr1, d1, t1, w);
            if constexpr (kDouble) {
                spmm(sys->L1, x1, t1, w);
                k_restrict_agg<double><<<grid1(n0 * w), TB, 0, ctx->stream>>>(r1.get(), t1.get(), sys->agg_t, r0, sys->agg_ptr, sys->agg_nodes, na, w);
            } else {
                mh_spmm_mixed(ctx, sys->L1, x1, t1d, w);
                k_restrict_agg<double><<<grid1(n0 * w), TB, 0, ctx->stream>>>(r1d.get(), t1d.get(), sys->agg_t, r0, sys->agg_ptr, sys->agg_nodes, na, w);
            }
            KERNEL_CHECK();
            mh_short_product(ctx, n0, sys->a0, uint32_t(n0), r0, w, x0, x0_partial, COARSE_SLICES);
            k_prolong_agg<T><<<grid1(n1 * w), TB, 0, ctx->stream>>>(x0, sys->agg_t, x1.get(), sys->agg_of, np, w);
            KERNEL_CHECK();
            cheb(sys->L1, deg1, r1, x1, false, rr1, d1, t1, w);
        }
        if constexpr (kDouble) k_prolong_p1<T><<<grid1(n2 * w), TB, 0, ctx->stream>>>(x1.get(), sys->parent_a, sys->parent_b, z, nn, w);
        else k_prolong_p1_v4<<<grid1(n2 * (w / 4)), TB, 0, ctx->stream>>>(reinterpret_cast<const f4_t *>(x1.get()), sys->parent_a, sys->parent_b, reinterpret_cast<f4_t *>(z), nn, w / 4);
        KERNEL_CHECK();
        cheb(sys->L2, deg2, r, z, false, r2, d2, t2, w, z_out, w_in);
    }
};

double estimate_lmax(mh_context *ctx, BsrLevel &lvl, const PatchSet &ps) {
    const uint32_t w = 8;
    const size_t rows = size_t(3) * lvl.n_nodes;
    DevArray<double> v(ctx, rows * w), t(ctx, rows * w), nrm(ctx, w), scratch, py(ctx, ps.scratch_rows() * w);
    k_random_panel<<<grid1(rows * w), TB, 0, ctx->stream>>>(v, rows * w, 0x5eedull);
    KERNEL_CHECK();
    colsumsq(ctx, v, rows, w, nrm, scratch);
    k_scale_cols_inv_sqrt<<<grid1(rows * w), TB, 0, ctx->stream>>>(v, nrm, rows, w);
    KERNEL_CHECK();
    constexpr int power_its = kPowerIterations;
    for (int it = 0; it < power_its; ++it) {
        mh_spmm(ctx, lvl, lvl.aval, v, t, nullptr, nullptr, w);
        k_dinv_mul<<<grid1(rows * w), TB, 0, ctx->stream>>>(t, lvl.dinv, v, rows, w);
        KERNEL_CHECK();
        mh_apply_patches<double>(ctx, ps, t, nullptr, w, 1.0, v, nullptr, nullptr, 0, py.get());
        const bool last = it + 1 == power_its, rescale = !last && (it % 4 == 3 || it + 2 == power_its);
        if (last || rescale) colsumsq(ctx, v, rows, w, nrm, scratch);
        if (rescale) {
            k_scale_cols_inv_sqrt<<<grid1(rows * w), TB, 0, ctx->stream>>>(v, nrm, rows, w);
            KERNEL_CHECK();
        }
    }
    auto h = nrm.to_host();
    double m = 0;
    for (double s : h) m = std::max(m, std::sqrt(s));
    return 1.1 * m * (switches().lmax_low ? 0.88 : 1.0);
}
}

void mh_cycle_shape(const mh_system *s, uint32_t w_in, MhCycleShape *shape) {
    MhCycleShape sh;
    const Switches &sw = switches();
    const bool surface_dominated = s->kept_tets < 4.5 * s->n_points;
    if (s->patches2.any()) {
        sh.deg2 = 5;
        sh.ratio = 60.0;
        const bool few_patches = uint64_t(s->patches2.n_bad_elements) * 500 < s->kept_tets;
        if (w_in > 128 || few_patches) sh.deg1 = 28, sh.gamma = 1, sh.ratio1 = 800.0;
    } else if (surface_dominated) {
        sh.deg2 = 5;
        sh.ratio = 60.0;
        sh.deg1 = 16, sh.gamma = 1, sh.ratio1 = 250.0;
    } else {
        sh.deg1 = 12, sh.gamma = 1, sh.ratio1 = 100.0;
    }
    if (sw.deg2 > 0) sh.deg2 = sw.deg2;
    if (sw.deg1 > 0) sh.deg1 = sw.deg1;
    if (sw.gamma > 0) sh.gamma = sw.gamma;
    if (sw.cheb_ratio > 0) sh.ratio = std::max(1.5, sw.cheb_ratio), sh.ratio1 = 0.0;
    if (sw.cheb_ratio1 > 0) sh.ratio1 = std::max(1.5, sw.cheb_ratio1);
    *shape = sh;
}

double mh_coarse_lift(const mh_system *sys) { return std::max(sys->coarse_lift, sys->worst_quality < kFlatShape ? 1e-8 : 1e-12); }

void mh_finish_hierarchy(mh_system *sys) {
    if (!sys->coarse_pending) return;
    mh_context *ctx = sys->ctx;
    sys->coarse_pending = false;
    HIP_CHECK(hipStreamWaitEvent(ctx->stream, sys->coarse_done, 0));
    int hinfo = 0;
    sys->coarse_info.download(&hinfo, 1);
    for (auto &ws : sys->coarse_ws) ws.reset(ctx, 0);
    for (PatchSet *ps : {&sys->patches2, &sys->patches1}) {
        if (!ps->any() || !ps->dropped.count) continue;
        int dropped[2] = {0, 0};
        ps->dropped.download(dropped, 2);
        sys->dropped_patches[ps->npe == 10 ? 0 : 1] = uint32_t(dropped[0]);
        if (dropped[0] && switches().verbose)
            fprintf(stderr, "[lobpcg] %d of %u + %u sliver patches / clusters of the %s level dropped (e.g. patch %d; clusters count from 1000000): their nodes keep the diagonal scaling only\n", dropped[0], ps->n_patches, ps->n_clusters,
                    ps->npe == 10 ? "P2" : "P1", dropped[1] - 1);
    }
    if (switches().test_coarse_pivot && sys->coarse_lift == 0) hinfo = 1;
    if (hinfo != 0) {
        sys->hierarchy_ready = false;
        mh_throw(MH_EFACTOR, "coarse operator not positive definite (pivot %d of a diagonal block): shift must be negative", hinfo);
    }
}

void mh_build_hierarchy(mh_system *sys, double sigma, bool defer) {
    mh_context *ctx = sys->ctx;
    if (sys->hierarchy_ready && sys->sigma_built == sigma) {
        if (!defer) mh_finish_hierarchy(sys);
        return;
    }
    mh_finish_hierarchy(sys);
    hipStream_t main_stream = ctx->stream;
    for (BsrLevel *lvl : {&sys->L2, &sys->L1}) {
        lvl->aval.reset(ctx, lvl->n_blocks * 9);
        lvl->dinv.reset(ctx, size_t(3) * lvl->n_nodes);
        k_shift_values<<<grid1(lvl->n_blocks * 9), TB, 0, ctx->stream>>>(lvl->kval, lvl->mval, lvl->n_blocks, sigma, lvl->aval);
        KERNEL_CHECK();
        k_diag_inverse<<<grid1(lvl->n_nodes), TB, 0, ctx->stream>>>(lvl->row_ptr, lvl->col, lvl->aval, lvl->n_nodes, lvl->dinv);
        KERNEL_CHECK();
        mh_build_patch_inverses(ctx, *lvl, lvl->id == 2 ? sys->patches2 : sys->patches1);
    }
    const size_t n0 = size_t(6) * sys->n_agg;
    sys->a0.reset(ctx, n0 * n0);
    sys->a0.zero();
    k_coarse_matrix<<<sys->n_agg, 64, 0, ctx->stream>>>(sys->L1.row_ptr, sys->L1.col, sys->L1.aval, sys->agg_t, sys->agg_of, sys->agg_ptr, sys->agg_nodes, sys->n_agg, sys->a0);
    KERNEL_CHECK();
    k_fix_coarse_diag<<<grid1(n0), TB, 0, ctx->stream>>>(sys->a0, uint32_t(n0), mh_coarse_lift(sys));
    KERNEL_CHECK();
    DevArray<int> &info = sys->coarse_info;
    info.reset(ctx, 1);
    auto smoother_setup = [&] {
        for (BsrLevel *lvl : {&sys->L2, &sys->L1}) {
            lvl->lmax = estimate_lmax(ctx, *lvl, lvl->id == 2 ? sys->patches2 : sys->patches1);
            if (sys->lmax_widened) lvl->lmax *= 1.25;
            lvl->aval32.reset(ctx, lvl->n_blocks * 9);
            lvl->dinv32.reset(ctx, size_t(3) * lvl->n_nodes);
            k_convert<double, float><<<grid1(lvl->n_blocks * 9), TB, 0, ctx->stream>>>(lvl->aval.get(), lvl->aval32.get(), lvl->n_blocks * 9);
            KERNEL_CHECK();
            k_convert<double, float><<<grid1(size_t(3) * lvl->n_nodes), TB, 0, ctx->stream>>>(lvl->dinv.get(), lvl->dinv32.get(), size_t(3) * lvl->n_nodes);
            KERNEL_CHECK();
        }
    };
    {
        const uint32_t nb = 128;
        DevArray<double> &cblk = sys->coarse_ws[0], &rblk = sys->coarse_ws[1], &pnext = sys->coarse_ws[4];
        DevArray<double> *pinv2[2] = {&sys->coarse_ws[2], &sys->coarse_ws[3]};
        cblk.reset(ctx, n0 * nb);
        rblk.reset(ctx, n0 * nb);
        pinv2[0]->reset(ctx, size_t(nb) * nb);
        pinv2[1]->reset(ctx, size_t(nb) * nb);
        pnext.reset(ctx, size_t(nb) * nb);
        info.zero();
        const bool side = ctx->aux_stream_ready();
        struct StreamGuard {
            mh_context *c;
            hipStream_t s;
            bool swapped{false};
            ~StreamGuard() {
                if (c->stream != s) {
                    c->stream = s;
                    if (swapped) std::swap(c->blas, c->blas_aux);
                    (void)hipStreamSynchronize(c->aux_stream);
                    if (c->aux2_stream) (void)hipStreamSynchronize(c->aux2_stream);
                }
            }
        } guard{ctx, main_stream};
        hipEvent_t forked = nullptr;
        if (side) {
            HIP_CHECK(hipEventCreateWithFlags(&forked, hipEventDisableTiming));
            HIP_CHECK(hipEventRecord(forked, main_stream));
            HIP_CHECK(hipStreamWaitEvent(ctx->aux_stream, forked, 0));
            ctx->stream = ctx->aux_stream;
            std::swap(ctx->blas, ctx->blas_aux);
            guard.swapped = true;
        }
        const size_t steps_total = div_up(n0, size_t(nb));
        const bool ahead = side && ctx->aux2_stream_ready(2 * steps_total);
        hipEvent_t *ev_piv = ctx->ahead_ev.data(), *ev_inv = ctx->ahead_ev.data() + steps_total;
        const double one = 1, zero = 0, mone = -1;
        const rocblas_int ld = rocblas_int(n0);
        double *a = sys->a0.get();
        uint32_t step = 0;
        for (size_t k0 = 0; k0 < n0; k0 += nb, ++step) {
            const rocblas_int w = rocblas_int(std::min<size_t>(nb, n0 - k0));
            double *pinv = pinv2[step & 1]->get();
            if (step == 0 || !ahead) mh_spd_inverse_small(ctx, a + k0 * n0 + k0, uint32_t(n0), uint32_t(w), pinv, uint32_t(w), info);
            else HIP_CHECK(hipStreamWaitEvent(ctx->stream, ev_inv[step], 0));
            HIP_CHECK(hipMemcpyAsync(cblk, a + k0 * n0, n0 * size_t(w) * sizeof(double), hipMemcpyDeviceToDevice, ctx->stream));
            ROCBLAS_CHECK(rocblas_dgemm(ctx->blas, rocblas_operation_none, rocblas_operation_none, w, ld, w, &one, pinv, w, a + k0, ld, &zero, rblk, w));
            const size_t k1 = k0 + nb;
            if (ahead && k1 < n0) {
                const uint32_t wn = uint32_t(std::min<size_t>(nb, n0 - k1));
                HIP_CHECK(hipMemcpy2DAsync(pnext.get(), size_t(wn) * sizeof(double), a + k1 * n0 + k1, n0 * sizeof(double), size_t(wn) * sizeof(double), wn, hipMemcpyDeviceToDevice, ctx->stream));
                mh_small_gemm(ctx, false, false, wn, wn, uint32_t(w), -1.0, cblk.get() + k1, uint32_t(n0), rblk.get() + k1 * size_t(w), uint32_t(w), 1.0, pnext.get(), wn);
                HIP_CHECK(hipEventRecord(ev_piv[step], ctx->stream));
                HIP_CHECK(hipStreamWaitEvent(ctx->aux2_stream, ev_piv[step], 0));
                hipStream_t elimination = ctx->stream;
                ctx->stream = ctx->aux2_stream;
                try {
                    mh_spd_inverse_small(ctx, pnext.get(), wn, wn, pinv2[(step + 1) & 1]->get(), wn, info);
                } catch (...) {
                    ctx->stream = elimination;
                    throw;
                }
                ctx->stream = elimination;
                HIP_CHECK(hipEventRecord(ev_inv[step + 1], ctx->aux2_stream));
            }
            ROCBLAS_CHECK(rocblas_dgemm(ctx->blas, rocblas_operation_none, rocblas_operation_none, ld, ld, w, &mone, cblk, ld, rblk, w, &one, a, ld));
            HIP_CHECK(hipMemcpy2DAsync(a + k0, n0 * sizeof(double), rblk.get(), size_t(w) * sizeof(double), size_t(w) * sizeof(double), n0, hipMemcpyDeviceToDevice, ctx->stream));
            ROCBLAS_CHECK(rocblas_dgemm(ctx->blas, rocblas_operation_none, rocblas_operation_none, ld, w, w, &mone, cblk, ld, pinv, w, &zero, a + k0 * n0, ld));
            HIP_CHECK(hipMemcpy2DAsync(a + k0 * n0 + k0, n0 * sizeof(double), pinv, size_t(w) * sizeof(double), size_t(w) * sizeof(double), size_t(w), hipMemcpyDeviceToDevice, ctx->stream));
        }
        k_symmetrize_lower<<<grid1(n0 * n0), TB, 0, ctx->stream>>>(sys->a0, uint32_t(n0), uint32_t(n0));
        KERNEL_CHECK();
        if (side) {
            ctx->stream = main_stream;
            std::swap(ctx->blas, ctx->blas_aux);
        }
        if (!sys->coarse_done) HIP_CHECK(hipEventCreateWithFlags(&sys->coarse_done, hipEventDisableTiming));
        HIP_CHECK(hipEventRecord(sys->coarse_done, side ? ctx->aux_stream : main_stream));
        sys->coarse_pending = true;
        smoother_setup();
        if (side) (void)hipEventDestroy(forked);
    }
    sys->sigma_built = sigma;
    sys->hierarchy_ready = true;
    if (!defer) {
        mh_finish_hierarchy(sys);
        HIP_CHECK(hipStreamSynchronize(ctx->stream));
    }
}

namespace {
__global__ void k_last_columns_to_panel(const double *__restrict__ z, size_t n, uint32_t ncols, const double *__restrict__ scale, double *__restrict__ x) {
    const size_t i = size_t(blockIdx.x) * blockDim.x + threadIdx.x;
    if (i >= n * ncols) return;
    const uint32_t j = uint32_t(i % ncols);
    x[i] = scale[j] * z[(n - 1 - j) * n + i / ncols];
}

void dense_eigs(mh_system *sys, uint32_t nev, double sigma, double *eigenvalues, bool inverse = false) {
    mh_context *ctx = sys->ctx;
    const size_t n = size_t(3) * sys->n_nodes;
    auto &lvl = sys->L2;
    DevArray<double> a(ctx, n * n), m(ctx, n * n), d(ctx, n), e(ctx, n);
    DevArray<int> info(ctx, 1);
    a.zero();
    m.zero();
    lvl.aval.reset(ctx, lvl.n_blocks * 9);
    k_shift_values<<<grid1(lvl.n_blocks * 9), TB, 0, ctx->stream>>>(lvl.kval, lvl.mval, lvl.n_blocks, sigma, lvl.aval);
    KERNEL_CHECK();
    k_bsr_to_dense<<<grid1(lvl.n_nodes), TB, 0, ctx->stream>>>(lvl.row_ptr, lvl.col, lvl.aval, lvl.mval, lvl.n_nodes, a, m);
    KERNEL_CHECK();
    HIP_CHECK(hipStreamSynchronize(ctx->stream));
    ExclusivePhase alone_on_the_device(ctx->device);
    double *lhs = inverse ? m.get() : a.get(), *rhs = inverse ? a.get() : m.get();
    ROCBLAS_CHECK(rocsolver_dsygvd(ctx->blas, rocblas_eform_ax, rocblas_evect_original, rocblas_fill_lower, rocblas_int(n), lhs, rocblas_int(n), rhs, rocblas_int(n), d, e, info));
    int hinfo = 0;
    info.download(&hinfo, 1);
    if (hinfo != 0) mh_throw(hinfo > int(n) ? MH_EFACTOR : MH_ENOTCONVERGED, "dense sygvd failed (info %d)", hinfo);
    std::vector<double> th(n);
    d.download(th.data(), n);
    sys->evecs.reset(ctx, n * nev);
    sys->evec_cols = nev;
    if (!inverse) {
        for (uint32_t i = 0; i < nev; ++i) eigenvalues[i] = th[i] + sigma;
        k_colmajor_to_panel<<<grid1(n * nev), TB, 0, ctx->stream>>>(lhs, n, nev, sys->evecs);
    } else {
        std::vector<double> scale(nev);
        for (uint32_t i = 0; i < nev; ++i) {
            const double nu = th[n - 1 - i];
            if (!(nu > 0)) mh_throw(MH_ENOTCONVERGED, "dense inverse eigensolve: non-positive eigenvalue %g at position %u", nu, i);
            eigenvalues[i] = 1.0 / nu + sigma;
            scale[i] = 1.0 / std::sqrt(nu);
        }
        DevArray<double> dscale(ctx, nev);
        dscale.upload(scale.data(), nev);
        k_last_columns_to_panel<<<grid1(n * nev), TB, 0, ctx->stream>>>(lhs, n, nev, dscale, sys->evecs);
    }
    KERNEL_CHECK();
    HIP_CHECK(hipStreamSynchronize(ctx->stream));
}
}

namespace {
__global__ void k_axpy_panel(double *__restrict__ y, const double *__restrict__ b, size_t count) {
    const size_t i = size_t(blockIdx.x) * blockDim.x + threadIdx.x;
    if (i < count) y[i] = b[i] - y[i];
}
__global__ void k_coldot_partial(const double *__restrict__ x, const double *__restrict__ y, size_t rows, uint32_t w, double *__restrict__ partial, uint32_t rows_per_block) {
    const uint32_t c = blockIdx.y * blockDim.x + threadIdx.x;
    if (c >= w) return;
    const size_t r0 = size_t(blockIdx.x) * rows_per_block, r1 = min(rows, r0 + rows_per_block);
    double s = 0;
    for (size_t r = r0; r < r1; ++r) s += x[r * w + c] * y[r * w + c];
    partial[size_t(blockIdx.x) * w + c] = s;
}
__global__ void k_cg_advance(double *__restrict__ x, double *__restrict__ r, const double *__restrict__ p, const double *__restrict__ ap, const double *__restrict__ rz, const double *__restrict__ pap,
                             size_t count, uint32_t w) {
    const size_t i = size_t(blockIdx.x) * blockDim.x + threadIdx.x;
    if (i >= count) return;
    const uint32_t c = uint32_t(i % w);
    const double alpha = pap[c] > 0 ? rz[c] / pap[c] : 0.0;
    x[i] += alpha * p[i];
    r[i] -= alpha * ap[i];
}
__global__ void k_cg_direction(double *__restrict__ p, const double *__restrict__ z, const double *__restrict__ rz_new, const double *__restrict__ rz_old, size_t count, uint32_t w) {
    const size_t i = size_t(blockIdx.x) * blockDim.x + threadIdx.x;
    if (i >= count) return;
    const uint32_t c = uint32_t(i % w);
    const double beta = rz_old[c] > 0 ? rz_new[c] / rz_old[c] : 0.0;
    p[i] = z[i] + beta * p[i];
}
}

namespace {
struct PanelCg {
    mh_system *sys;
    mh_context *ctx;
    size_t n;
    uint32_t wmax;
    DevArray<double> rr, zz, p, ap, rz, rz_new, pap, scratch;
    static constexpr uint32_t rpb = 256;
    PanelCg(mh_system *s, uint32_t w) : sys(s), ctx(s->ctx), n(size_t(3) * s->n_nodes), wmax(w), rr(s->ctx, n * w), zz(s->ctx, n * w), p(s->ctx, n * w), ap(s->ctx, n * w), rz(s->ctx, w), rz_new(s->ctx, w),
                                        pap(s->ctx, w), scratch(s->ctx, size_t(div_up(n, rpb)) * w) {}
    void dot(const double *u, const double *v, double *out, uint32_t w) {
        const uint32_t nb = uint32_t(div_up(n, rpb));
        k_coldot_partial<<<dim3(nb, div_up(w, 64)), 64, 0, ctx->stream>>>(u, v, n, w, scratch, rpb);
        KERNEL_CHECK();
        k_colsumsq_final<<<w, 256, 0, ctx->stream>>>(scratch, nb, w, out);
        KERNEL_CHECK();
    }
    template<typename Prec> void solve(Prec &prec, const double *r, double *z, uint32_t w, int iters) {
        hipStream_t st = ctx->stream;
        HIP_CHECK(hipMemsetAsync(z, 0, n * w * sizeof(double), st));
        HIP_CHECK(hipMemcpyAsync(rr.get(), r, n * w * sizeof(double), hipMemcpyDeviceToDevice, st));
        prec.apply(rr, zz, w);
        HIP_CHECK(hipMemcpyAsync(p.get(), zz.get(), n * w * sizeof(double), hipMemcpyDeviceToDevice, st));
        dot(rr, zz, rz, w);
        for (int k = 0; k < iters; ++k) {
            mh_spmm(ctx, sys->L2, sys->L2.aval, p, ap, nullptr, nullptr, w);
            dot(p, ap, pap, w);
            k_cg_advance<<<grid1(n * w), TB, 0, st>>>(z, rr, p, ap, rz, pap, n * w, w);
            KERNEL_CHECK();
            if (k + 1 == iters) break;
            prec.apply(rr, zz, w);
            dot(rr, zz, rz_new, w);
            k_cg_direction<<<grid1(n * w), TB, 0, st>>>(p, zz, rz_new, rz, n * w, w);
            KERNEL_CHECK();
            HIP_CHECK(hipMemcpyAsync(rz.get(), rz_new.get(), w * sizeof(double), hipMemcpyDeviceToDevice, st));
        }
    }
};
}

namespace {
struct BlockLobpcg {
    mh_system *sys;
    mh_context *ctx;
    hipStream_t st;
    const size_t n;
    const uint32_t nev, b, mmax;
    const double sigma, residual_tol;
    const uint32_t max_iters;
    const float *seed_basis;
    const uint32_t seed_rows, seed_cols;
    const volatile unsigned char *cancel;
    volatile float *progress;
    mh_profile &prof;
    mh_profile *profile;
    SharedPhase iterating;
    Timer t_iter;
    double precond_seconds = 0;
    double best_worst_active = 1e300;
    int floor_strikes = 0;
    std::vector<double> hist_active;
    uint32_t pairs_at_floor = 0;
    DevArray<double> X, AX, MX, Xn, AXn, MXn, W, AW, MW, P, MP, Pn, MPn, R, Rw;
    DevArray<double> gA, gM, gM0, gA0, App, evals, ework, Cp, T1, H, H2, G, dscale, Linv, theta_d, rn_d, mn_d, scratch, Ct, norms_d, theta_act_d, Hp, Up, Vp, T1p;
    DevArray<double> Linv_p, T1p2;
    DevArray<uint32_t> idx_d, pos_d;
    DevArray<double> Rr, res_partial, res_blocks, res_norms_d;
    std::vector<double> rr_evals;
    std::vector<uint32_t> res_act, res_pos;
    std::vector<double> res_norms;
    uint32_t res_pitch = 0;
    bool res_ready = false, rw_from_rr = false;
    DevArray<int> info;
    int inner_cg = 0;
    std::unique_ptr<Precond<float>> prec32;
    std::unique_ptr<Precond<double>> prec64;
    std::unique_ptr<PanelCg> panel_cg;
    const bool verbose = switches().verbose, fp32_prec = switches().fp32_prec;
    const bool pproj_ok;
    const bool scaled_norms;
    bool warm = false;
    bool w_implicit = false;
    int last_spread = 1 << 20;
    bool p_needs_explicit = false;
    uint32_t wp = 0;
    uint32_t iters = 0, nconv = 0, redos_at_start = 0;
    bool poly_allowed = true;
    std::vector<double> theta, rn, mn, xn, norms, theta_act, hist_worst;
    double anorm = 0;
    std::vector<uint32_t> act, order, hist_nconv;
    std::vector<uint8_t> locked;
    bool converged = false;
    bool gm_identity = false;
    bool p_implicit = false;
    bool lazy_images = false;
    uint32_t w = 0, wa = 0, m = 0, wp_new = 0;

    BlockLobpcg(mh_system *system, uint32_t nev_, uint32_t block, double sigma_, double residual_tol_, uint32_t max_iters_, const float *seed_basis_, uint32_t seed_rows_,
                uint32_t seed_cols_, const volatile unsigned char *cancel_, volatile float *progress_, mh_profile &prof_, mh_profile *profile_, int inner_cg_ = 0)
        : sys(system), ctx(system->ctx), st(system->ctx->stream), n(size_t(3) * system->n_nodes), nev(nev_), b(block), mmax(3 * block), sigma(sigma_), residual_tol(residual_tol_),
          max_iters(max_iters_), seed_basis(seed_basis_), seed_rows(seed_rows_), seed_cols(seed_cols_), cancel(cancel_), progress(progress_), prof(prof_), profile(profile_),
          iterating(system->ctx->device, true), t_iter(system->ctx), pproj_ok(block <= 128), scaled_norms(system->patches2.any()), theta(block), rn(block), mn(block), xn(block), norms(3 * size_t(block)),
          theta_act(block), order(block), locked(block, 0) {
        inner_cg = inner_cg_;
        for (DevArray<double> *panel : {&X, &AX, &MX, &Xn, &AXn, &MXn, &W, &AW, &MW, &P, &Pn, &R, &Rw}) panel->reset(ctx, n * b);
        if (!pproj_ok)
            for (DevArray<double> *panel : {&MP, &MPn}) panel->reset(ctx, n * b);
        for (DevArray<double> *small : {&gA, &gM, &gM0, &gA0}) small->reset(ctx, size_t(mmax) * mmax);
        for (DevArray<double> *small : {&App, &H, &H2, &Linv, &Hp, &Up, &Vp, &T1p}) small->reset(ctx, size_t(b) * b);
        Linv_p.reset(ctx, size_t(b) * b);
        T1p2.reset(ctx, size_t(mmax) * b);
        for (DevArray<double> *small : {&Cp, &T1}) small->reset(ctx, size_t(mmax) * b);
        for (DevArray<double> *small : {&evals, &ework}) small->reset(ctx, mmax);
        for (DevArray<double> *small : {&dscale, &theta_d, &rn_d, &mn_d, &theta_act_d}) small->reset(ctx, b);
        G.reset(ctx, size_t(b) * 2 * b);
        Ct.reset(ctx, size_t(mmax) * 2 * b);
        norms_d.reset(ctx, 3 * size_t(b));
        idx_d.reset(ctx, b);
        pos_d.reset(ctx, b);
        if (b <= 128) {
            const uint32_t pmax = (b + 1u) & ~1u;
            Rr.reset(ctx, n * pmax);
            res_partial.reset(ctx, size_t(2) * sys->n_nodes * pmax);
            res_blocks.reset(ctx, size_t(div_up(sys->n_nodes, 48)) * 2 * pmax);
            res_norms_d.reset(ctx, size_t(2) * pmax);
            res_norms.resize(size_t(2) * pmax);
        }
        info.reset(ctx, 2);
        if (fp32_prec && !(sys->worst_quality < kFlatShape) && !inner_cg) prec32 = std::make_unique<Precond<float>>(sys, std::min(b, kPrecondColumns));
        else prec64 = std::make_unique<Precond<double>>(sys, std::min(b, kPrecondColumns));
        if (inner_cg) panel_cg = std::make_unique<PanelCg>(sys, std::min(b, kPrecondColumns));
        auto hd = sys->L2.dinv.to_host();
        double dmin = 1e300;
        for (double v : hd) dmin = std::min(dmin, v);
        anorm = sys->L2.lmax / dmin;
    }


    bool chol_orthonormalise(double *V, double *MV, double *AV, uint32_t w, bool transform_images = true, bool allow_implicit = false,
                             const double *hp = nullptr, uint32_t hp_rows = 0) {
        gram(ctx, n, V, w, MV, w, G, w);
        if (hp) {
            const double minus = -1, plus = 1;
            small_dgemm(ctx, rocblas_operation_transpose, rocblas_operation_none, rocblas_int(w), rocblas_int(w), rocblas_int(hp_rows), &minus, hp,
                                        rocblas_int(hp_rows), hp, rocblas_int(hp_rows), &plus, G, rocblas_int(w));
        }
        k_scale_gram<<<grid1(size_t(w) * w), TB, 0, st>>>(G, w, w, dscale);
        KERNEL_CHECK();
        double *Gs = G.get() + size_t(w) * w;
        int hinfo = 0;
        bool fused_inverse = false;
        {
            last_spread = 1 << 20;
            if (w <= 128) {
                fused_inverse = !switches().potrf_chain;
                if (fused_inverse) mh_potrf_small_inverse(ctx, Gs, w, info, dscale, Linv);
                else mh_potrf_small(ctx, Gs, w, info);
                int both[2] = {0, 0};
                info.download(both, 2);
                hinfo = both[0];
                last_spread = both[1];
            } else {
                mh_potrf(ctx, Gs, w, w, info);
                info.download(&hinfo, 1);
            }
        }
        p_needs_explicit = false;
        if (hp && (hinfo != 0 || last_spread >= 16 * 8)) {
            p_needs_explicit = true;
            return true;
        }
        if (hinfo != 0) return false;
        if (!fused_inverse) {
            k_unscale_chol<<<grid1(size_t(w) * w), TB, 0, st>>>(Gs, w, w, dscale);
            KERNEL_CHECK();
        }
        if (w > 256) {
            panel_trsm(ctx, n, V, w, Gs, w);
            if (MV) panel_trsm(ctx, n, MV, w, Gs, w);
            if (AV) panel_trsm(ctx, n, AV, w, Gs, w);
        } else {
            if (!fused_inverse) {
                HIP_CHECK(hipMemsetAsync(Linv, 0, size_t(w) * w * sizeof(double), st));
                ROCBLAS_CHECK(rocblas_dtrtri(ctx->blas, rocblas_fill_lower, rocblas_diagonal_non_unit, w, Gs, w, Linv, w));
            }
            w_implicit = allow_implicit && !transform_images && last_spread < 16 * 8;
            if (!w_implicit) mh_combine(ctx, n, V, w, nullptr, 0, nullptr, 0, Linv, w, V, w, nullptr);
            if (MV && transform_images) mh_combine(ctx, n, MV, w, nullptr, 0, nullptr, 0, Linv, w, MV, w, nullptr);
            if (AV && transform_images) mh_combine(ctx, n, AV, w, nullptr, 0, nullptr, 0, Linv, w, AV, w, nullptr);
        }
        return true;
    }

    void precondition(const double *r, double *z, uint32_t w) {
        precondition_in_slabs(ctx, n, r, z, w, [&](const double *rp, double *zp, uint32_t wc) {
            if (panel_cg) panel_cg->solve(*prec64, rp, zp, wc, inner_cg);
            else if (prec32) prec32->apply(rp, zp, wc);
            else prec64->apply(rp, zp, wc);
        });
    }

    void start() {
        redos_at_start = ctx->sytrd_redos;
        if (ctx->rr_check) HIP_CHECK(hipMemsetAsync(ctx->rr_check, 0, sizeof(unsigned long long), st));
        k_random_panel<<<grid1(n * b), TB, 0, st>>>(X, n * b, 20260710ull);
        KERNEL_CHECK();
        warm = seed_basis && seed_rows == n && seed_cols >= nev;
        if (warm) {
            const uint32_t ncols = std::min(seed_cols, b);
            DevArray<float> seed(ctx, n * ncols);
            seed.upload(seed_basis, n * ncols);
            k_load_seed<<<grid1(n * ncols), TB, 0, st>>>(seed, sys->perm, sys->n_nodes, ncols, b, X);
            KERNEL_CHECK();
            HIP_CHECK(hipStreamSynchronize(st));
        }
        const uint32_t n_rigid = 6 * sys->n_components;
        const bool seed_rigid = b >= n_rigid + 6;
        if (!seed_rigid && sys->n_components > 1)
            mh_throw(MH_EINVAL, "the mesh consists of %u disconnected bodies (%u zero modes): more than a block of %u columns can seed", sys->n_components, n_rigid, b);
        const auto inject_rigid_modes = [&] {
            k_inject_rbm<<<grid1(sys->n_nodes), TB, 0, st>>>(sys->node_xyz, sys->node_component, sys->component_centroid, sys->n_components, sys->n_nodes, X, b, 0);
            KERNEL_CHECK();
        };
        if (seed_rigid) inject_rigid_modes();
        bool with_poly = !warm && seed_rigid && !switches().no_poly_start && sys->n_components == 1 && poly_allowed;
        if (with_poly) {
            DevArray<unsigned long long> keys(ctx, 6);
            const unsigned long long init[6] = {~0ull, ~0ull, ~0ull, 0, 0, 0};
            keys.upload(init, 6);
            k_bbox<<<grid1(sys->n_nodes), TB, 0, st>>>(sys->node_xyz, sys->n_nodes, keys);
            KERNEL_CHECK();
            unsigned long long hk[6];
            keys.download(hk, 6);
            double box[6], longest = 0, shortest = 1e300;
            for (int a = 0; a < 6; ++a) {
                const unsigned long long u = (hk[a] >> 63) ? (hk[a] & 0x7fffffffffffffffull) : ~hk[a];
                memcpy(&box[a], &u, sizeof(double));
            }
            for (int a = 0; a < 3; ++a) longest = std::max(longest, box[3 + a] - box[a]), shortest = std::min(shortest, box[3 + a] - box[a]);
            with_poly = shortest >= 0.25 * longest;
            if (with_poly) {
                const uint32_t room = b - n_rigid, want = room - room / 4;
                std::vector<uint32_t> triples;
                for (uint32_t deg = 2; deg <= 6 && 6 + 3 * (triples.size() + (deg + 1) * (deg + 2) / 2) <= want; ++deg)
                    for (uint32_t a = deg + 1; a-- > 0;)
                        for (uint32_t bb = deg - a + 1; bb-- > 0;) triples.push_back(a | bb << 8 | (deg - a - bb) << 16);
                DevArray<double> box_d(ctx, 6);
                DevArray<uint32_t> tri_d(ctx, std::max<size_t>(1, triples.size()));
                box_d.upload(box, 6);
                if (!triples.empty()) tri_d.upload(triples.data(), triples.size());
                k_inject_poly<<<grid1(sys->n_nodes), TB, 0, st>>>(sys->node_xyz, box_d, sys->n_nodes, tri_d, uint32_t(triples.size()), X, b, n_rigid);
                KERNEL_CHECK();
                HIP_CHECK(hipStreamSynchronize(st));
            }
        }
        if (!warm) {
            {
                mh_spmm(ctx, sys->L2, nullptr, X, nullptr, sys->L2.mval, MX, b);
                Timer tp(ctx);
                precondition(MX, Xn, b);
                precond_seconds += tp.stop();
                prof.op_applications += b;
                HIP_CHECK(hipMemcpyAsync(X, Xn.get(), n * b * sizeof(double), hipMemcpyDeviceToDevice, st));
            }
            if (seed_rigid) inject_rigid_modes();
        }
        mh_spmm(ctx, sys->L2, nullptr, X, nullptr, sys->L2.mval, MX, b);
        if (!chol_orthonormalise(X, MX, nullptr, b)) {
            if (with_poly) {
                if (verbose) fprintf(stderr, "[lobpcg] polynomial start block rank deficient: random block instead\n");
                poly_allowed = false;
                start();
                return;
            }
            mh_throw(MH_ENOTCONVERGED, "initial block is rank deficient");
        }
        mh_spmm(ctx, sys->L2, sys->L2.aval, X, AX, sys->L2.mval, MX, b);
        {
            gram(ctx, n, X, b, AX, b, gA, b);
            gram(ctx, n, X, b, MX, b, gM, b);
            const int hinfo = mh_rr_solve(ctx, gA, gM, b, evals, ework, info);
            if (hinfo != 0) mh_throw(MH_ENOTCONVERGED, "initial Rayleigh-Ritz failed (info %d)", hinfo);
            panel_mul(ctx, n, X, b, gA, b, Xn, b, 1.0, 0.0);
            panel_mul(ctx, n, AX, b, gA, b, AXn, b, 1.0, 0.0);
            panel_mul(ctx, n, MX, b, gA, b, MXn, b, 1.0, 0.0);
            std::swap(X, Xn); std::swap(AX, AXn); std::swap(MX, MXn);
            evals.download(theta.data(), b);
        }
    }

    bool converged_or_locked(uint32_t it) {
        if (cancel && *cancel) mh_throw(MH_ECANCELLED, "cancelled");
        if (g_concurrent) {
            iterating.release();
            iterating.acquire();
        }
        bool fused = res_ready;
        if (fused)
            for (const uint32_t i : res_act) fused = fused && !(std::abs(theta[i]) < 10.0 * std::abs(sigma));
        res_ready = false;
        rw_from_rr = fused;
        if (fused) {
            res_norms_d.download(res_norms.data(), size_t(2) * res_pitch);
            for (size_t k = 0; k < res_act.size(); ++k) {
                rn[res_act[k]] = res_norms[k];
                mn[res_act[k]] = res_norms[res_pitch + k];
            }
        } else {
        theta_d.upload(theta.data(), b);
        {
            const uint32_t rpb = 256, nblk = div_up(n, rpb);
            if (scratch.count < size_t(nblk) * 3 * b) scratch.reset(ctx, size_t(nblk) * 3 * b);
            dim3 grid(nblk, div_up(b, 64));
            k_residual_norms<<<grid, 64, 0, st>>>(AX, MX, X, theta_d, 10.0 * std::abs(sigma), R, n, b, rpb, scratch, scaled_norms ? sys->L2.dinv.get() : nullptr);
            KERNEL_CHECK();
            k_colsumsq_final<<<3 * b, 256, 0, st>>>(scratch, nblk, 3 * b, norms_d);
            KERNEL_CHECK();
            norms_d.download(norms.data(), 3 * size_t(b));
            std::copy(norms.begin(), norms.begin() + b, rn.begin());
            std::copy(norms.begin() + b, norms.begin() + 2 * b, mn.begin());
            std::copy(norms.begin() + 2 * b, norms.end(), xn.begin());
        }
        }
        act.clear();
        for (uint32_t i = 0; i < b; ++i) {
            const double rel = std::sqrt(rn[i]) / (std::abs(theta[i]) * std::sqrt(mn[i]));
            const bool near_shift = std::abs(theta[i]) < 10.0 * std::abs(sigma);
            const double floor_norm = scaled_norms ? sys->L2.lmax * std::sqrt(xn[i]) : anorm * std::sqrt(xn[i]);
            const double floor_factor = it == 0 && !warm && sys->worst_quality < kFlatShape ? 65536.0 : 256.0;
            const bool ok = rel < residual_tol || (near_shift && std::sqrt(rn[i]) < floor_factor * 2.2e-16 * floor_norm);
            if (ok) locked[i] = 1;
            if (!locked[i]) act.push_back(i);
        }
        std::iota(order.begin(), order.end(), 0u);
        std::stable_sort(order.begin(), order.end(), [&](uint32_t a, uint32_t c) { return theta[a] < theta[c]; });
        nconv = 0;
        for (uint32_t k = 0; k < nev; ++k) nconv += locked[order[k]];
        if (progress) *progress = 0.3f + 0.65f * float(nconv) / float(nev);
        if (verbose) {
            double worst = 0;
            for (uint32_t k = 0; k < nev; ++k) { const uint32_t i = order[k]; worst = std::max(worst, std::sqrt(rn[i]) / (std::abs(theta[i]) * std::sqrt(mn[i]))); }
            if (it == 0) fprintf(stderr, "[lobpcg] ||A|| <= %.3e, sliver patches %u + %u clusters (largest %u nodes; worst element shape %.2e), aggregates %u, lmax %.4f / %.4f\n", anorm, sys->patches2.n_patches, sys->patches2.n_clusters, sys->patches2.largest_cluster, double(sys->worst_quality), sys->n_agg, sys->L2.lmax, sys->L1.lmax);
            fprintf(stderr, "[lobpcg] it %3u conv %3u/%u active %zu wp %u worst %.2e  floor-ratio[0..7]:", it, nconv, nev, act.size(), wp, worst);
            for (uint32_t i = 0; i < std::min(8u, b); ++i) fprintf(stderr, " %.1f", xn[i] > 0 ? std::sqrt(rn[i]) / (2.2e-16 * (scaled_norms ? sys->L2.lmax : anorm) * std::sqrt(xn[i])) : 0.0);
            fprintf(stderr, "  theta0 %.6e\n", theta[0]);
        }
        iters = it;
        if (nconv >= nev || act.empty()) { converged = nconv >= nev; return true; }
        if (it == max_iters) return true;
        {
            double worst = 0;
            for (uint32_t k = 0; k < nev; ++k) { const uint32_t i = order[k]; worst = std::max(worst, std::sqrt(rn[i]) / (std::abs(theta[i]) * std::sqrt(mn[i]))); }
            hist_worst.push_back(worst);
            hist_nconv.push_back(nconv);
            const size_t h = hist_worst.size();
            if (prec32 && it >= 10 && h > 6 && hist_nconv[h - 7] == nconv && worst > 0.5 * hist_worst[h - 7]) {
                if (verbose) fprintf(stderr, "[lobpcg] it %3u stagnation: switching the preconditioner to double precision\n", it);
                prec32.reset();
                prec64 = std::make_unique<Precond<double>>(sys, std::min(b, kPrecondColumns));
            }
            double worst_active = 0;
            for (uint32_t k = 0; k < nev; ++k) {
                const uint32_t i = order[k];
                if (!locked[i]) worst_active = std::max(worst_active, std::sqrt(rn[i]) / (std::abs(theta[i]) * std::sqrt(mn[i])));
            }
            best_worst_active = std::min(best_worst_active, worst_active);
            hist_active.push_back(worst_active);
            if (inner_cg > 0 && it >= 40) {
                const size_t h = hist_active.size();
                if (h > 30 && hist_nconv[h - 31] == nconv && worst_active > 0.9 * hist_active[h - 31] && worst_active <= 10.0 * residual_tol) {
                    pairs_at_floor = nev > nconv ? nev - nconv : 0;
                    if (verbose) fprintf(stderr, "[lobpcg] it %3u: %u pairs have sat at a residual of %.2e (tolerance %.1e) for thirty iterations -- the rounding floor of this mesh; handed on as they are\n", it, pairs_at_floor, worst_active, residual_tol);
                    converged = true;
                    return true;
                }
            }
            floor_strikes = it >= 20 && worst_active > 1e3 * best_worst_active ? floor_strikes + 1 : 0;
            if (floor_strikes >= 3)
                mh_throw(MH_ENOTCONVERGED, "LOBPCG: %u of %u pairs converged; the others sit at the rounding floor (residual %.1e and growing, best %.1e, tolerance %.1e)", nconv, nev,
                         worst_active, best_worst_active, residual_tol);
        }
        return false;
    }

    void search_directions(uint32_t it) {
        w = uint32_t(act.size());
        idx_d.upload(act.data(), w);
        const double *residuals = Rw.get();
        if (rw_from_rr) {
            if (act == res_act && res_pitch == w) {
                residuals = Rr.get();
            } else {
                std::vector<uint32_t> &pos = res_pos;
                pos.assign(w, 0);
                size_t q = 0;
                for (uint32_t k = 0; k < w; ++k) {
                    while (q < res_act.size() && res_act[q] != act[k]) ++q;
                    if (q == res_act.size()) mh_throw(MH_EHIP, "active column %u was not active before", act[k]);
                    pos[k] = uint32_t(q);
                }
                pos_d.upload(pos.data(), w);
                k_gather_cols<<<grid1(n * w), TB, 0, st>>>(Rr, pos_d, Rw, n, res_pitch, w);
                KERNEL_CHECK();
            }
        } else {
            k_gather_cols<<<grid1(n * w), TB, 0, st>>>(R, idx_d, Rw, n, b, w);
            KERNEL_CHECK();
        }
        for (uint32_t k = 0; k < w; ++k) theta_act[k] = theta[act[k]];
        theta_act_d.upload(theta_act.data(), w);
        {
            Timer tp(ctx);
            precondition(residuals, W, w);
            precond_seconds += tp.stop();
            prof.op_applications += w;
        }
        bool ok = true;
        p_implicit = false;
        if (pproj_ok && wp) {
            gram(ctx, n, MX, b, W, w, H, b);
            mh_pack_stacked(ctx, H, b, nullptr, 0, w, -1.0, Ct);
            mh_combine(ctx, n, X, b, nullptr, 0, nullptr, 0, Ct, w, W, w, nullptr, true);
            mh_spmm(ctx, sys->L2, sys->L2.aval, W, AW, sys->L2.mval, MW, w);
            gram(ctx, n, P, wp, MW, w, Hp, wp);
            lazy_images = true;
            w_implicit = false;
            ok = chol_orthonormalise(W, MW, AW, w, false, true, Hp, wp);
            if (!ok) mh_throw(MH_ENOTCONVERGED, "search directions lost rank at iteration %u", it);
            if (p_needs_explicit) {
                mh_pack_stacked(ctx, Hp, wp, nullptr, 0, w, -1.0, Ct);
                mh_combine(ctx, n, P, wp, nullptr, 0, nullptr, 0, Ct, w, W, w, nullptr, true);
                mh_spmm(ctx, sys->L2, sys->L2.aval, W, AW, sys->L2.mval, MW, w);
                lazy_images = w <= 256;
                ok = chol_orthonormalise(W, MW, AW, w, !lazy_images, lazy_images);
                if (!ok) mh_throw(MH_ENOTCONVERGED, "search directions lost rank at iteration %u", it);
            } else {
                p_implicit = true;
            }
        } else {
            gram(ctx, n, MX, b, W, w, H, b);
            if (wp) gram(ctx, n, MP, wp, W, w, H2, wp);
            mh_pack_stacked(ctx, H, b, H2, wp, w, -1.0, Ct);
            mh_combine(ctx, n, X, b, P, wp, nullptr, 0, Ct, w, W, w, nullptr, true);
            mh_spmm(ctx, sys->L2, sys->L2.aval, W, AW, sys->L2.mval, MW, w);
            lazy_images = w <= 256;
            w_implicit = false;
            ok = chol_orthonormalise(W, MW, AW, w, !lazy_images, lazy_images);
            if (!ok) mh_throw(MH_ENOTCONVERGED, "search directions lost rank at iteration %u", it);
        }
    }

    void rayleigh_ritz(uint32_t it) {
        wa = w;
        m = wa + w + wp;
        for (int attempt = 0; attempt < 2; ++attempt) {
            HIP_CHECK(hipMemsetAsync(gA, 0, size_t(m) * m * sizeof(double), st));
            HIP_CHECK(hipMemsetAsync(gM, 0, size_t(m) * m * sizeof(double), st));
            k_set_identity_blocks<<<grid1(wa), TB, 0, st>>>(gA, gM, theta_act_d, wa, m);
            KERNEL_CHECK();
            const double unit_one = 1;
            auto left_corrected = [&](double *block, uint32_t cols) {
                if (w_implicit)
                    ROCBLAS_CHECK(rocblas_dtrmm(ctx->blas, rocblas_side_left, rocblas_fill_lower, rocblas_operation_none, rocblas_diagonal_non_unit, rocblas_int(w),
                                                rocblas_int(cols), &unit_one, Linv, rocblas_int(w), block, rocblas_int(m), block, rocblas_int(m)));
            };
            mh_gram(ctx, n, W, w, AX, wa, gA.get() + wa, m, b, idx_d);
            left_corrected(gA.get() + wa, wa);
            const double unit = 1;
            auto untransformed = [&](double *block, uint32_t rows) {
                if (lazy_images)
                    ROCBLAS_CHECK(rocblas_dtrmm(ctx->blas, rocblas_side_right, rocblas_fill_lower, rocblas_operation_transpose, rocblas_diagonal_non_unit, rocblas_int(rows),
                                                rocblas_int(w), &unit, Linv, rocblas_int(w), block, rocblas_int(m), block, rocblas_int(m)));
            };
            gram(ctx, n, W, w, AW, w, gA.get() + size_t(wa) * m + wa, m);
            if (p_implicit && wp) {
                const double plus = 1, nil = 0;
                double *bw = gA.get() + size_t(wa) * m + wa, *bp = gA.get() + size_t(wa) * m + wa + w;
                gram(ctx, n, P, wp, AW, w, bp, m);
                small_dgemm(ctx, rocblas_operation_transpose, rocblas_operation_none, rocblas_int(w), rocblas_int(w), rocblas_int(wp), &plus, Hp, rocblas_int(wp), bp,
                                            rocblas_int(m), &nil, Up, rocblas_int(w));
                small_dgemm(ctx, rocblas_operation_none, rocblas_operation_none, rocblas_int(wp), rocblas_int(w), rocblas_int(wp), &plus, App, rocblas_int(wp), Hp,
                                            rocblas_int(wp), &nil, T1p, rocblas_int(wp));
                small_dgemm(ctx, rocblas_operation_transpose, rocblas_operation_none, rocblas_int(w), rocblas_int(w), rocblas_int(wp), &plus, Hp, rocblas_int(wp), T1p,
                                            rocblas_int(wp), &nil, Vp, rocblas_int(w));
                k_sub_block<<<grid1(size_t(wp) * w), TB, 0, st>>>(bp, m, T1p, wp, wp, w);
                k_wblock_fix<<<grid1(size_t(w) * w), TB, 0, st>>>(bw, m, Up, Vp, w);
                KERNEL_CHECK();
            }
            untransformed(gA.get() + size_t(wa) * m + wa, w);
            left_corrected(gA.get() + size_t(wa) * m + wa, w);
            const bool w_block_trusted = last_spread < 16 * 8 && !(p_implicit && wp == 0);
            gm_identity = w_block_trusted;
            if (w_block_trusted) {
                k_place_block<<<grid1(size_t(w) * w), TB, 0, st>>>(gM.get() + size_t(wa) * m + wa, m, nullptr, w);
                KERNEL_CHECK();
            } else {
                gram(ctx, n, W, w, MW, w, gM.get() + size_t(wa) * m + wa, m);
                untransformed(gM.get() + size_t(wa) * m + wa, w);
            }
            if (verbose) fprintf(stderr, "[lobpcg] it %3u Cholesky-QR diagonal spread 2^%.1f%s\n", it, last_spread / 16.0, w_block_trusted ? "" : " (W block measured)");
            if (wp) {
                if (!p_implicit) gram(ctx, n, P, wp, AW, w, gA.get() + size_t(wa) * m + wa + w, m);
                untransformed(gA.get() + size_t(wa) * m + wa + w, wp);
                {
                    k_place_block<<<grid1(size_t(wp) * wp), TB, 0, st>>>(gA.get() + size_t(wa + w) * m + wa + w, m, App, wp);
                    k_place_block<<<grid1(size_t(wp) * wp), TB, 0, st>>>(gM.get() + size_t(wa + w) * m + wa + w, m, nullptr, wp);
                    KERNEL_CHECK();
                }
            }
            k_symmetrize_lower<<<grid1(size_t(m) * m), TB, 0, st>>>(gA, m, m);
            KERNEL_CHECK();
            HIP_CHECK(hipMemcpyAsync(gA0, gA, size_t(m) * m * sizeof(double), hipMemcpyDeviceToDevice, st));
            HIP_CHECK(hipMemcpyAsync(gM0, gM, size_t(m) * m * sizeof(double), hipMemcpyDeviceToDevice, st));
            rr_evals.clear();
            const int hinfo = mh_rr_solve(ctx, gA, gM, m, evals, ework, info, wa, gm_identity, &rr_evals);
            if (hinfo == 0) break;
            if (attempt == 1 || wp == 0) mh_throw(MH_ENOTCONVERGED, "Rayleigh-Ritz failed at iteration %u (info %d)", it, hinfo);
            wp = 0;
            m = wa + w;
        }
        if (rr_evals.size() == wa) std::copy(rr_evals.begin(), rr_evals.end(), theta_act.begin());
        else evals.download(theta_act.data(), wa);
        for (uint32_t k = 0; k < wa; ++k) theta[act[k]] = theta_act[k];
    }

    void conjugate_directions(uint32_t it) {
        const double one = 1, zero = 0, mone = -1;
        wp_new = w;
        k_build_cp<<<grid1(size_t(m) * w), TB, 0, st>>>(gA, nullptr, wa, m, w, m, Cp, m);
        KERNEL_CHECK();
        const double *mcp = gm_identity ? Cp.get() : T1.get();
        if (!gm_identity) ROCBLAS_CHECK(rocblas_dsymm(ctx->blas, rocblas_side_left, rocblas_fill_lower, m, w, &one, gM0, m, Cp, m, &zero, T1, m));
        small_dgemm(ctx, rocblas_operation_transpose, rocblas_operation_none, wa, w, m, &one, gA, m, mcp, m, &zero, H, wa);
        small_dgemm(ctx, rocblas_operation_none, rocblas_operation_none, m, w, wa, &mone, gA, m, H, wa, &one, Cp, m);
        if (!gm_identity) ROCBLAS_CHECK(rocblas_dsymm(ctx->blas, rocblas_side_left, rocblas_fill_lower, m, w, &one, gM0, m, Cp, m, &zero, T1, m));
        small_dgemm(ctx, rocblas_operation_transpose, rocblas_operation_none, w, w, m, &one, Cp, m, mcp, m, &zero, G, w);
        k_scale_gram<<<grid1(size_t(w) * w), TB, 0, st>>>(G, w, w, dscale);
        KERNEL_CHECK();
        {
            double *Gs = G.get() + size_t(w) * w;
            int hinfo = 0;
            const bool fused = w <= 128 && !switches().potrf_chain;
            {
                if (fused) mh_potrf_small_inverse(ctx, Gs, w, info, dscale, Linv_p);
                else mh_potrf(ctx, Gs, w, w, info);
                info.download(&hinfo, 1);
            }
            if (hinfo != 0) {
                wp_new = 0;
            } else if (fused) {
                mh_small_gemm(ctx, false, true, m, w, w, 1.0, Cp, m, Linv_p, w, 0.0, T1p2, m);
                HIP_CHECK(hipMemcpyAsync(Cp, T1p2, size_t(m) * w * sizeof(double), hipMemcpyDeviceToDevice, st));
            } else {
                k_unscale_chol<<<grid1(size_t(w) * w), TB, 0, st>>>(Gs, w, w, dscale);
                KERNEL_CHECK();
                ROCBLAS_CHECK(rocblas_dtrsm(ctx->blas, rocblas_side_right, rocblas_fill_lower, rocblas_operation_transpose, rocblas_diagonal_non_unit, m, w, &one, Gs, w, Cp, m));
            }
        }
        if (!warm && it < kSkipP && !hist_worst.empty() && hist_worst.back() > 0.5) wp_new = 0;
        if (wp_new) {
            small_dgemm(ctx, rocblas_operation_none, rocblas_operation_none, m, wp_new, m, &one, gA0, m, Cp, m, &zero, T1, m);
            small_dgemm(ctx, rocblas_operation_transpose, rocblas_operation_none, wp_new, wp_new, m, &one, Cp, m, T1, m, &zero, App, wp_new);
        }
    }

    void update_basis(uint32_t it) {
        mh_pack_coefficients(ctx, gA, wa, Cp, wp_new, m, m, Ct);
        {
            const uint32_t pitch = (wa + 1u) & ~1u;
            if (w_implicit) {
                const double unit = 1;
                double *rows = Ct.get() + size_t(wa) * (wa + wp_new);
                ROCBLAS_CHECK(rocblas_dtrmm(ctx->blas, rocblas_side_right, rocblas_fill_lower, rocblas_operation_none, rocblas_diagonal_non_unit, rocblas_int(wa + wp_new),
                                            rocblas_int(w), &unit, Linv, rocblas_int(w), rows, rocblas_int(wa + wp_new), rows, rocblas_int(wa + wp_new)));
            }
            if (p_implicit && wp) {
                const double minus = -1, plus = 1;
                const rocblas_int pitchc = rocblas_int(wa + wp_new);
                double *rows_w = Ct.get() + size_t(wa) * (wa + wp_new), *rows_p = Ct.get() + size_t(wa + w) * (wa + wp_new);
                ROCBLAS_CHECK(rocblas_dgemm(ctx->blas, rocblas_operation_none, rocblas_operation_transpose, pitchc, rocblas_int(wp), rocblas_int(w), &minus, rows_w, pitchc, Hp,
                                            rocblas_int(wp), &plus, rows_p, pitchc));
            }
            mh_combine(ctx, n, X, wa, W, w, P, wp, Ct, wa + wp_new, Xn, wa, Pn, false, b, idx_d, pitch);
            if (wp_new && !pproj_ok) mh_spmm(ctx, sys->L2, nullptr, Pn, nullptr, sys->L2.mval, MPn, wp_new);
            if (pitch == wa) k_scatter_cols<<<grid1(n * wa), TB, 0, st>>>(Xn.get(), idx_d, X.get(), n, b, wa);
            else k_scatter_cols_pitch<<<grid1(n * wa), TB, 0, st>>>(Xn.get(), pitch, idx_d, X.get(), n, b, wa);
            KERNEL_CHECK();
            if (Rr.count) {
                mh_spmm_mapped(ctx, sys->L2, sys->L2.aval, Xn, AX, sys->L2.mval, MX, pitch, b, wa, idx_d, evals, Rr, res_partial, scaled_norms ? sys->L2.dinv.get() : nullptr);
                const uint32_t rpb = 48, nblk = div_up(sys->n_nodes, rpb), w2 = 2 * pitch;
                dim3 grid(nblk, div_up(w2, 64));
                k_colsum_partial<<<grid, 64, 0, st>>>(res_partial, sys->n_nodes, w2, res_blocks, rpb);
                KERNEL_CHECK();
                k_colsumsq_final<<<w2, 256, 0, st>>>(res_blocks, nblk, w2, res_norms_d);
                KERNEL_CHECK();
                res_act = act;
                res_pitch = pitch;
                res_ready = true;
            } else {
                mh_spmm_mapped(ctx, sys->L2, sys->L2.aval, Xn, AX, sys->L2.mval, MX, pitch, b, wa, idx_d);
            }
        }
        std::swap(P, Pn); std::swap(MP, MPn);
        wp = wp_new;
    }

    void finish(double *eigenvalues) {
        prof.restarts = iters;
        prof.op_solve = precond_seconds;
        if (!converged) mh_throw(MH_ENOTCONVERGED, "LOBPCG: %u of %u pairs converged in %u iterations", nconv, nev, iters);
        for (uint32_t k = 0; k < nev; ++k) eigenvalues[k] = theta[order[k]] + sigma;
        sys->plain_residual = -1.0;
        if (scaled_norms) {
            theta_d.upload(theta.data(), b);
            const uint32_t rpb = 256, nblk = div_up(n, rpb);
            if (scratch.count < size_t(nblk) * 3 * b) scratch.reset(ctx, size_t(nblk) * 3 * b);
            k_residual_norms<<<dim3(nblk, div_up(b, 64)), 64, 0, st>>>(AX, MX, X, theta_d, 10.0 * std::abs(sigma), R, n, b, rpb, scratch, nullptr);
            KERNEL_CHECK();
            k_colsumsq_final<<<3 * b, 256, 0, st>>>(scratch, nblk, 3 * b, norms_d);
            KERNEL_CHECK();
            norms_d.download(norms.data(), 3 * size_t(b));
            double worst = 0;
            for (uint32_t k = 0; k < nev; ++k) {
                const uint32_t i = order[k];
                if (std::abs(theta[i]) < 10.0 * std::abs(sigma)) continue;
                worst = std::max(worst, std::sqrt(norms[i]) / (std::abs(theta[i]) * std::sqrt(norms[b + i])));
            }
            sys->plain_residual = worst;
            if (verbose) fprintf(stderr, "[lobpcg] accepted in the Jacobi-scaled norm at %.1e; worst elastic pair in the plain 2-norm: %.2e\n", residual_tol, worst);
        }
        sys->evecs.reset(ctx, n * nev);
        sys->evec_cols = nev;
        idx_d.upload(order.data(), nev);
        k_gather_cols<<<grid1(n * nev), TB, 0, st>>>(X, idx_d, sys->evecs, n, b, nev);
        KERNEL_CHECK();
        HIP_CHECK(hipStreamSynchronize(st));
        prof.iterate = t_iter.stop();
        read_health();
        sys->profile = prof;
        if (profile) *profile = prof;
        if (switches().test_selfcheck_fail && !ctx->exchange_disabled) prof.rr_selfcheck = 1.0;
        if (!(prof.rr_selfcheck < 1e-6))
            mh_throw(MH_EHIP, "Rayleigh-Ritz self-check failed: a step's eigenpairs leave a relative residual of %.2e against the step's own matrix", prof.rr_selfcheck);
    }
    void read_health() {
        prof.sytrd_redos = ctx->sytrd_redos - redos_at_start;
        prof.pairs_at_floor = pairs_at_floor;
        prof.rr_selfcheck = 0.0;
        if (ctx->rr_check) {
            unsigned long long bits = 0;
            HIP_CHECK(hipMemcpyAsync(&bits, ctx->rr_check, sizeof(bits), hipMemcpyDeviceToHost, st));
            HIP_CHECK(hipStreamSynchronize(st));
            memcpy(&prof.rr_selfcheck, &bits, sizeof(double));
        }
    }

    void run(double *eigenvalues) {
        start();
        for (uint32_t it = 0; it <= max_iters; ++it) {
            if (converged_or_locked(it)) break;
            search_directions(it);
            rayleigh_ritz(it);
            conjugate_directions(it);
            update_basis(it);
        }
        finish(eigenvalues);
    }
};
struct Attempt {
    mh_system *sys;
    uint32_t nev, b;
    double sigma, residual_tol;
    const float *seed;
    uint32_t srows, scols;
    const volatile unsigned char *cancel;
    volatile float *progress;
    double *eigenvalues;
    mh_profile &prof;
    mh_profile *profile;
    std::optional<MhError> run(uint32_t max_iters, int inner_cg = 0) {
        try {
            BlockLobpcg solver(sys, nev, b, sigma, residual_tol, max_iters, seed, srows, scols, cancel, progress, prof, profile, inner_cg);
            solver.run(eigenvalues);
            return std::nullopt;
        } catch (const MhError &e) {
            return e;
        }
    }
    void reset_profile() {
        prof = sys->profile;
        prof.dofs = uint32_t(size_t(3) * sys->n_nodes);
    }
    void widen_lmax() {
        if (sys->lmax_widened) return;
        sys->L1.lmax *= 1.25;
        sys->L2.lmax *= 1.25;
        sys->lmax_widened = true;
    }
};
}

static void eigs_impl(mh_system *sys, uint32_t nev, double sigma, double residual_tol, uint32_t max_iters, const float *seed_basis, uint32_t seed_rows,
                      uint32_t seed_cols, const volatile unsigned char *cancel, volatile float *progress, double *eigenvalues, mh_profile *profile) {
    mh_context *ctx = sys->ctx;
    HIP_CHECK(hipSetDevice(ctx->device));
    const size_t n = size_t(3) * sys->n_nodes;
    if (nev >= n) mh_throw(MH_EINVAL, "nev %u must be below the %zu unknowns", nev, n);
    if (!(sigma < 0)) mh_throw(MH_EFACTOR, "shift must be negative for a positive-definite shifted operator");
    if (sys->unreferenced_points) mh_throw(MH_EFACTOR, "%u mesh point(s) belong to no tetrahedron: the shifted operator is singular", sys->unreferenced_points);
    mh_profile prof = sys->profile;
    prof.dofs = uint32_t(n);
    prof.stiffness_nonzeros = uint32_t((sys->L2.n_blocks - sys->n_nodes) / 2 * 9 + uint64_t(6) * sys->n_nodes);
    if (cancel && *cancel) mh_throw(MH_ECANCELLED, "cancelled");
    const uint32_t guards = std::max(15u, nev * kGuardPercent / 100);
    const uint32_t b = (nev + guards + 6u * (sys->n_components - 1u) + 15u) / 16u * 16u;
    if (n <= 768 || n < size_t(5) * b) {
        Timer t(ctx);
        dense_eigs(sys, nev, sigma, eigenvalues);
        prof.iterate = t.stop();
        prof.restarts = 1;
        sys->profile = prof;
        if (profile) *profile = prof;
        return;
    }
    const Switches &sw = switches();
    Attempt attempt{sys, nev, b, sigma, residual_tol, seed_basis, seed_rows, seed_cols, cancel, progress, eigenvalues, prof, profile};
    for (int lifted = 0;; ++lifted) {
        try {
            {
                Timer t(ctx);
                mh_build_hierarchy(sys, sigma, true);
                prof.factorize = t.stop();
            }
            if (progress) *progress = 0.3f;
            std::optional<MhError> err;
            if (sw.test_last_resort) err = MhError(MH_ENOTCONVERGED, "MH_TEST=last_resort");
            else err = attempt.run(max_iters);
            if (err && !sw.test_last_resort && attempt.seed && err->code == MH_ENOTCONVERGED && max_iters >= 50) {
                if (sw.verbose) fprintf(stderr, "[lobpcg] %s -- the seeded basis did not serve: once more from a cold start\n", err->what());
                attempt.seed = nullptr, attempt.srows = 0, attempt.scols = 0;
                attempt.reset_profile();
                err = attempt.run(max_iters);
            }
            if (err && err->code == MH_EHIP && strstr(err->what(), "self-check") && !ctx->exchange_disabled) {
                if (sw.verbose) fprintf(stderr, "[lobpcg] %s -- once more without the exchange kernels\n", err->what());
                ctx->exchange_disabled = true;
                attempt.reset_profile();
                err = attempt.run(max_iters);
            }
            if (err && err->code == MH_ENOTCONVERGED && max_iters >= 50 && !sys->lmax_widened && !sw.test_last_resort && !(sys->worst_quality < kFlatShape)) {
                if (sw.verbose) fprintf(stderr, "[lobpcg] %s -- once more with the smoothers' spectral bounds widened by 25 %%\n", err->what());
                attempt.widen_lmax();
                err = attempt.run(max_iters);
            }
            if (err && err->code == MH_ENOTCONVERGED && n > kDenseLastResort && max_iters >= 50) {
                if (sw.verbose) fprintf(stderr, "[lobpcg] %s -- last resort: conjugate-gradient search directions\n", err->what());
                const MhError stopped = *err;
                attempt.reset_profile();
                attempt.widen_lmax();
                err = attempt.run(max_iters, kLastResortCg);
                if (err && err->code == MH_ENOTCONVERGED) {
                    if (sw.verbose) fprintf(stderr, "[lobpcg] the last resort with %d conjugate-gradient steps: %s -- once more with %d\n", kLastResortCg, err->what(), 5 * kLastResortCg);
// ... 141 lines not shown
```

### mesheditor_amd/csrc/mh_spmm.hip

```cpp
#include "mh_common.h"

namespace {
#ifndef MH_SPMM_TB
#define MH_SPMM_TB 64
#endif
constexpr int TB = MH_SPMM_TB;
#ifndef MH_SPMM_U
#define MH_SPMM_U 1
#endif

template<typename T, int CW, int NC, bool WITH_M, bool WITH_A>
__global__ void __launch_bounds__(TB) k_spmm(const uint32_t *__restrict__ row_ptr, const uint32_t *__restrict__ col, const T *__restrict__ vals9,
                                            const T *__restrict__ mscal, const T *__restrict__ x, T *__restrict__ y, T *__restrict__ y2,
                                            uint32_t nnodes, uint32_t w, int xcd_remap) {
    constexpr int RPW = 64 / CW;
    const int lane = threadIdx.x & 63, wave = threadIdx.x >> 6;
    const uint32_t c0 = blockIdx.y * (CW * NC) + (lane % CW);
    const uint32_t nb = gridDim.x, per = (nb + 7) / 8;
    const uint32_t bid = xcd_remap ? (blockIdx.x % 8) * per + blockIdx.x / 8 : blockIdx.x;
    uint32_t row = (bid * (TB / 64) + wave) * RPW + lane / CW;
    if (RPW == 1) row = __builtin_amdgcn_readfirstlane(row);
    if (row >= nnodes) return;
    bool active[NC];
    uint32_t cc[NC];
#pragma unroll
    for (int k = 0; k < NC; ++k) {
        active[k] = c0 + CW * k < w;
        cc[k] = active[k] ? c0 + CW * k : 0;
    }
    T a0[NC], a1[NC], a2[NC], m0[NC], m1[NC], m2[NC];
#pragma unroll
    for (int k = 0; k < NC; ++k) a0[k] = a1[k] = a2[k] = m0[k] = m1[k] = m2[k] = 0;
    const uint32_t p1 = row_ptr[row + 1];
    uint32_t p = row_ptr[row];
    auto step = [&](auto u_tag) {
        constexpr int U = decltype(u_tag)::value;
        uint32_t j[U];
#pragma unroll
        for (int u = 0; u < U; ++u) j[u] = col[p + u];
        T xv[U][NC][3];
#pragma unroll
        for (int u = 0; u < U; ++u) {
            const T *xr = x + size_t(3) * j[u] * w;
#pragma unroll
            for (int k = 0; k < NC; ++k) {
                xv[u][k][0] = xr[cc[k]];
                xv[u][k][1] = xr[w + cc[k]];
                xv[u][k][2] = xr[2 * size_t(w) + cc[k]];
            }
        }
        T v[U][9], m[U];
#pragma unroll
        for (int u = 0; u < U; ++u) {
            if (WITH_A) {
#pragma unroll
                for (int e = 0; e < 9; ++e) v[u][e] = vals9[size_t(9) * (p + u) + e];
            }
            m[u] = WITH_M ? mscal[p + u] : T(0);
        }
#pragma unroll
        for (int u = 0; u < U; ++u) {
#pragma unroll
            for (int k = 0; k < NC; ++k) {
                const T x0 = xv[u][k][0], x1 = xv[u][k][1], x2 = xv[u][k][2];
                if (WITH_A) {
                    a0[k] += v[u][0] * x0 + v[u][1] * x1 + v[u][2] * x2;
                    a1[k] += v[u][3] * x0 + v[u][4] * x1 + v[u][5] * x2;
                    a2[k] += v[u][6] * x0 + v[u][7] * x1 + v[u][8] * x2;
                }
                if (WITH_M) {
                    m0[k] += m[u] * x0;
                    m1[k] += m[u] * x1;
                    m2[k] += m[u] * x2;
                }
            }
        }
        p += U;
    };
    constexpr int UMAX = NC >= 3 ? 2 : (NC == 2 ? 4 : 8);
    while (p + UMAX <= p1) step(std::integral_constant<int, UMAX>{});
    if (UMAX >= 8 && p + 4 <= p1) step(std::integral_constant<int, 4>{});
    if (UMAX >= 4 && p + 2 <= p1) step(std::integral_constant<int, 2>{});
    while (p < p1) step(std::integral_constant<int, 1>{});
#pragma unroll
    for (int k = 0; k < NC; ++k) {
        if (!active[k]) continue;
        const size_t o = size_t(3) * row * w + c0 + CW * k;
        if (WITH_A) { y[o] = a0[k]; y[o + w] = a1[k]; y[o + 2 * size_t(w)] = a2[k]; }
        if (WITH_M) { y2[o] = m0[k]; y2[o + w] = m1[k]; y2[o + 2 * size_t(w)] = m2[k]; }
    }
}

struct ChebStep {
    float *r = nullptr;
    const float *dinv = nullptr;
    float *d_out = nullptr;
    float *x = nullptr;
    float c1 = 0.f, c2 = 0.f;
};
struct ResidualEpilogue {
    const double *theta = nullptr;
    double *r_out = nullptr;
    double *partial = nullptr;
    const double *dinv = nullptr;
};
#ifdef MH_SPMM_WAVES
#define MH_SPMM_OCC __attribute__((amdgpu_waves_per_eu(MH_SPMM_WAVES, 8)))
#else
#define MH_SPMM_OCC
#endif
template<typename TV, typename TX, typename TY, int V, int CL, bool WITH_M, bool WITH_A, bool MAPOUT = false, int EPI = 0, int UR = MH_SPMM_U, bool PRE = false>
__global__ void __launch_bounds__(TB) MH_SPMM_OCC k_spmm_wide(const uint32_t *__restrict__ row_ptr, const uint32_t *__restrict__ col, const TV *__restrict__ vals9,
                                                 const TV *__restrict__ mscal, const TX *__restrict__ x, TY *__restrict__ y, TY *__restrict__ y2, uint32_t nnodes,
                                                 uint32_t w, int xcd_remap, uint32_t ldy = 0, uint32_t wreal = 0, const uint32_t *__restrict__ omap = nullptr, ChebStep epi = ChebStep{},
                                                 uint32_t xpitch = 0, ResidualEpilogue res = ResidualEpilogue{}) {
    constexpr int G = 64 / CL, STRIP = 64, VP = sizeof(TV) == 4 ? 12 : 10, U = UR;
    typedef TX Vec __attribute__((ext_vector_type(V)));
    typedef TY Acc __attribute__((ext_vector_type(V)));
    __shared__ __attribute__((aligned(16))) TV sv[TB / 64][WITH_A ? (STRIP + 1) * VP : 1];
    __shared__ TV sm[TB / 64][WITH_M ? STRIP + 1 : 1];
    __shared__ uint32_t sc[TB / 64][STRIP + 1];
    const int lane = threadIdx.x & 63, wave = threadIdx.x >> 6;
    const uint32_t c = lane % CL, g = lane / CL;
    const uint32_t nb_grid = gridDim.x, per = (nb_grid + 7) / 8;
    const uint32_t bid = xcd_remap ? (blockIdx.x % 8) * per + blockIdx.x / 8 : blockIdx.x;
    const uint32_t row = __builtin_amdgcn_readfirstlane(bid * (TB / 64) + wave);
    if (row >= nnodes) return;
    const bool act = V * c < w && g < G;
    const uint32_t coff = act ? V * c : 0;
    Acc acc[3], macc[3];
#pragma unroll
    for (int i = 0; i < 3; ++i) acc[i] = macc[i] = Acc(0);
    Acc er[PRE ? 3 : 1], ed[PRE ? 3 : 1], ex[PRE ? 3 : 1];
    TY edinv[PRE ? 3 : 1];
    if constexpr (EPI == 1 && PRE) {
        if (g == 0 && act) {
            const size_t o = size_t(3) * row * w + coff;
#pragma unroll
            for (int i = 0; i < 3; ++i) {
                er[i] = *reinterpret_cast<const Acc *>(epi.r + o + size_t(i) * w);
                ed[i] = __builtin_convertvector(*reinterpret_cast<const Vec *>(x + o + size_t(i) * w), Acc);
                ex[i] = *reinterpret_cast<const Acc *>(epi.x + o + size_t(i) * w);
                edinv[i] = epi.dinv[size_t(3) * row + i];
            }
        }
    }
    const uint32_t p0 = __builtin_amdgcn_readfirstlane(row_ptr[row]), p1 = __builtin_amdgcn_readfirstlane(row_ptr[row + 1]);
    TV *svw = sv[wave];
    TV *smw = sm[wave];
    uint32_t *scw = sc[wave];
    for (uint32_t base = p0; base < p1; base += STRIP) {
        const uint32_t nb = min(uint32_t(STRIP), p1 - base);
        if (base != p0) __builtin_amdgcn_fence(__ATOMIC_ACQ_REL, "wavefront");
        scw[lane] = uint32_t(lane) < nb ? col[base + lane] : 0u;
        if (WITH_A) {
            const TV *src = vals9 + size_t(9) * base;
            TV tmp[9];
#pragma unroll
            for (int i = 0; i < 9; ++i) {
                const uint32_t f = lane + 64 * i;
                tmp[i] = f < 9 * nb ? src[f] : TV(0);
            }
#pragma unroll
            for (int i = 0; i < 9; ++i) {
                const uint32_t f = lane + 64 * i;
                if (f < 9 * nb) svw[(f / 9) * VP + f % 9] = tmp[i];
            }
        }
        if (WITH_M) smw[lane] = uint32_t(lane) < nb ? mscal[base + lane] : TV(0);
        if (lane == 0) {
            scw[nb] = row;
            if (WITH_M) smw[nb] = TV(0);
        }
        if (WITH_A && lane < VP) svw[nb * VP + lane] = TV(0);
        __builtin_amdgcn_fence(__ATOMIC_ACQ_REL, "wavefront");
        const uint32_t rounds = (nb + G - 1) / G;
        for (uint32_t t0 = 0; t0 < rounds; t0 += U) {
            Vec xv[U][3];
            uint32_t bi[U];
#pragma unroll
            for (int u = 0; u < U; ++u) {
                if (t0 + u < rounds) {
                    bi[u] = min((t0 + u) * G + g, nb);
                    const uint32_t xp = MAPOUT ? xpitch : w;
                    const TX *xr = x + size_t(3) * scw[bi[u]] * xp + coff;
                    xv[u][0] = *reinterpret_cast<const Vec *>(xr);
                    xv[u][1] = *reinterpret_cast<const Vec *>(xr + xp);
                    xv[u][2] = *reinterpret_cast<const Vec *>(xr + 2 * size_t(xp));
                }
            }
#pragma unroll
            for (int u = 0; u < U; ++u) {
                if (t0 + u < rounds) {
                    const Acc x0 = __builtin_convertvector(xv[u][0], Acc), x1 = __builtin_convertvector(xv[u][1], Acc), x2 = __builtin_convertvector(xv[u][2], Acc);
                    if (WITH_A) {
                        TY v[9];
#pragma unroll
                        for (int e = 0; e < 9; ++e) v[e] = TY(svw[bi[u] * VP + e]);
                        acc[0] += v[0] * x0; acc[0] += v[1] * x1; acc[0] += v[2] * x2;
                        acc[1] += v[3] * x0; acc[1] += v[4] * x1; acc[1] += v[5] * x2;
                        acc[2] += v[6] * x0; acc[2] += v[7] * x1; acc[2] += v[8] * x2;
                    }
                    if (WITH_M) {
                        const TY m = TY(smw[bi[u]]);
                        macc[0] += m * x0;
                        macc[1] += m * x1;
                        macc[2] += m * x2;
                    }
                }
            }
        }
    }
    if constexpr ((G & (G - 1)) == 0) {
#pragma unroll
        for (int sft = G / 2; sft >= 1; sft >>= 1) {
#pragma unroll
            for (int i = 0; i < 3; ++i) {
#pragma unroll
                for (int e = 0; e < V; ++e) {
                    if (WITH_A) acc[i][e] += __shfl_down(acc[i][e], sft * CL, 64);
                    if (WITH_M) macc[i][e] += __shfl_down(macc[i][e], sft * CL, 64);
                }
            }
        }
    } else {
#pragma unroll
        for (int i = 0; i < 3; ++i) {
#pragma unroll
            for (int e = 0; e < V; ++e) {
                TY sa = acc[i][e], sm_ = macc[i][e];
#pragma unroll
                for (int j = 1; j < G; ++j) {
                    if (WITH_A) sa += __shfl_down(acc[i][e], j * CL, 64);
                    if (WITH_M) sm_ += __shfl_down(macc[i][e], j * CL, 64);
                }
                acc[i][e] = sa;
                macc[i][e] = sm_;
            }
        }
    }
    if constexpr (EPI == 1) {
        if (g == 0 && act) {
            const size_t o = size_t(3) * row * w + coff;
#pragma unroll
            for (int i = 0; i < 3; ++i) {
                const size_t oi = o + size_t(i) * w;
                Acc rv, dv, xn;
                if constexpr (PRE) {
                    rv = er[i] - acc[i];
                    dv = epi.c1 * ed[i] + (epi.c2 * edinv[i]) * rv;
                    xn = ex[i] + dv;
                } else {
                    rv = *reinterpret_cast<const Acc *>(epi.r + oi) - acc[i];
                    dv = epi.c1 * __builtin_convertvector(*reinterpret_cast<const Vec *>(x + oi), Acc) + (epi.c2 * epi.dinv[size_t(3) * row + i]) * rv;
                    xn = *reinterpret_cast<const Acc *>(epi.x + oi) + dv;
                }
                *reinterpret_cast<Acc *>(epi.r + oi) = rv;
                *reinterpret_cast<Acc *>(epi.d_out + oi) = dv;
                *reinterpret_cast<Acc *>(epi.x + oi) = xn;
            }
        }
        return;
    }
    if (MAPOUT) {
        if (g == 0 && act) {
#pragma unroll
            for (int e = 0; e < V; ++e) {
                if (coff + e >= wreal) continue;
                const size_t o = size_t(3) * row * ldy + omap[coff + e];
                if (WITH_A) { y[o] = acc[0][e]; y[o + ldy] = acc[1][e]; y[o + 2 * size_t(ldy)] = acc[2][e]; }
                if (WITH_M) { y2[o] = macc[0][e]; y2[o + ldy] = macc[1][e]; y2[o + 2 * size_t(ldy)] = macc[2][e]; }
            }
            if constexpr (WITH_A && WITH_M && std::is_same<TY, double>::value && V == 2) {
                if (res.r_out) {
                    Acc th, sr = Acc(0), sm = Acc(0);
                    th[0] = res.theta[coff];
                    th[1] = res.theta[coff + 1];
#pragma unroll
                    for (int i = 0; i < 3; ++i) {
                        const Acc r = acc[i] - th * macc[i];
                        const TY wgt = res.dinv ? res.dinv[size_t(3) * row + i] : TY(1);
                        *reinterpret_cast<Acc *>(res.r_out + (size_t(3) * row + i) * w + coff) = r;
                        sr += wgt * (r * r);
                        sm += wgt * (macc[i] * macc[i]);
                    }
                    *reinterpret_cast<Acc *>(res.partial + (size_t(2) * row) * w + coff) = sr;
                    *reinterpret_cast<Acc *>(res.partial + (size_t(2) * row + 1) * w + coff) = sm;
                }
            }
        }
        return;
    }
    if (g == 0 && act) {
        const size_t o = size_t(3) * row * w + coff;
        if (WITH_A) {
            *reinterpret_cast<Acc *>(y + o) = acc[0];
            *reinterpret_cast<Acc *>(y + o + w) = acc[1];
            *reinterpret_cast<Acc *>(y + o + 2 * size_t(w)) = acc[2];
        }
        if (WITH_M) {
            *reinterpret_cast<Acc *>(y2 + o) = macc[0];
            *reinterpret_cast<Acc *>(y2 + o + w) = macc[1];
            *reinterpret_cast<Acc *>(y2 + o + 2 * size_t(w)) = macc[2];
        }
    }
}

inline bool latency_bound_level(const BsrLevel &lvl) {
    constexpr bool on = false;
    return on && lvl.n_nodes < 32768;
}

template<typename TV, typename TX, typename TY, bool WITH_M, bool WITH_A>
bool launch_spmm_wide(mh_context *ctx, const BsrLevel &lvl, const TV *vals9, const TX *x, TY *y, const TV *mscal, TY *y2, uint32_t w) {
    constexpr uint32_t VFULL = 16 / sizeof(TX);
    constexpr bool legacy = false;
    constexpr bool mixed = !std::is_same<TV, TX>::value || !std::is_same<TX, TY>::value;
    if (legacy && !mixed) return false;
    constexpr int xcd = 1;
    const unsigned grid = (div_up(lvl.n_nodes, TB / 64) + 7) / 8 * 8;
    auto run = [&](auto v_tag) {
        constexpr int V = decltype(v_tag)::value;
        auto go = [&](auto cl_tag) {
            constexpr int CL = decltype(cl_tag)::value;
            if (latency_bound_level(lvl))
                k_spmm_wide<TV, TX, TY, V, CL, WITH_M, WITH_A, false, 0, 4><<<grid, TB, 0, ctx->stream>>>(lvl.row_ptr, lvl.col, vals9, mscal, x, y, y2, lvl.n_nodes, w, xcd);
            else
                k_spmm_wide<TV, TX, TY, V, CL, WITH_M, WITH_A><<<grid, TB, 0, ctx->stream>>>(lvl.row_ptr, lvl.col, vals9, mscal, x, y, y2, lvl.n_nodes, w, xcd);
        };
        const uint32_t lanes = div_up(w, uint32_t(V));
        if (lanes <= 8) go(std::integral_constant<int, 8>{});
        else if (lanes <= 16) go(std::integral_constant<int, 16>{});
        else if (lanes <= 20 && V == 4) go(std::integral_constant<int, 20>{});
        else if (lanes <= 32) go(std::integral_constant<int, 32>{});
        else go(std::integral_constant<int, 64>{});
    };
    const bool aligned16 = !((reinterpret_cast<uintptr_t>(x) | reinterpret_cast<uintptr_t>(y) | reinterpret_cast<uintptr_t>(y2)) & 15);
    if (w % VFULL == 0 && w <= 64 * VFULL && aligned16) run(std::integral_constant<int, int(VFULL)>{});
    else if (!mixed && w <= 16) run(std::integral_constant<int, 1>{});
    else return false;
    KERNEL_CHECK();
    return true;
}

template<typename T, bool WITH_M, bool WITH_A>
void launch_spmm(mh_context *ctx, const BsrLevel &lvl, const T *vals9, const T *x, T *y, const T *mscal, T *y2, uint32_t w) {
    if (launch_spmm_wide<T, T, T, WITH_M, WITH_A>(ctx, lvl, vals9, x, y, mscal, y2, w)) return;
    const uint32_t n = lvl.n_nodes;
    auto go = [&](auto cw_tag, auto nc_tag) {
        constexpr int CW = decltype(cw_tag)::value, NC = decltype(nc_tag)::value;
        constexpr int RPW = 64 / CW;
        constexpr int xcd = 1;
        dim3 grid((div_up(n, (TB / 64) * RPW) + 7) / 8 * 8, div_up(w, CW * NC));
        k_spmm<T, CW, NC, WITH_M, WITH_A><<<grid, TB, 0, ctx->stream>>>(lvl.row_ptr, lvl.col, vals9, mscal, x, y, y2, n, w, xcd);
    };
    using I = std::integral_constant<int, 0>;
    (void)sizeof(I);
    auto ic = [](auto v) { return v; };
    (void)ic;
#define MH_GO(CWV, NCV) go(std::integral_constant<int, CWV>{}, std::integral_constant<int, NCV>{})
    if (w <= 8) MH_GO(8, 1);
    else if (w <= 64) MH_GO(64, 1);
    else if (w <= 128) MH_GO(64, 2);
    else if (w <= 192) MH_GO(64, 3);
    else MH_GO(64, 4);
#undef MH_GO
    KERNEL_CHECK();
}

}

void mh_timer_flush(mh_context *ctx) {
    if (!ctx->timer_used) return;
    HIP_CHECK(hipStreamSynchronize(ctx->stream));
    for (size_t i = 0; i < ctx->timer_used; ++i) {
        float ms = 0;
        HIP_CHECK(hipEventElapsedTime(&ms, ctx->timer_events[i].first, ctx->timer_events[i].second));
        auto &t = ctx->totals[ctx->timer_class[i]];
        t.ms += ms;
        t.work += ctx->timer_work[i];
        ++t.launches;
    }
    ctx->timer_used = 0;
}

namespace {
double spmm_bytes(const BsrLevel &lvl, uint32_t w, size_t value_bytes, size_t x_bytes, size_t y_bytes, bool with_a, bool with_m) {
    const double per_block = (with_a ? 9.0 : 0.0) * value_bytes + (with_m ? 1.0 : 0.0) * value_bytes + 4.0;
    const double panel = 3.0 * double(lvl.n_nodes) * w;
    return per_block * double(lvl.n_blocks) + 4.0 * (double(lvl.n_nodes) + 1) + panel * x_bytes + panel * y_bytes * ((with_a ? 1 : 0) + (with_m ? 1 : 0));
}
}

void mh_spmm(mh_context *ctx, const BsrLevel &lvl, const double *vals9, const double *x, double *y, const double *mscal, double *y2, uint32_t w) {
    if (w == 0) return;
    TimedLaunch timed(ctx, MH_KERNEL_SPMM, spmm_bytes(lvl, w, 8, 8, 8, vals9 != nullptr, mscal != nullptr));
    if (vals9 && mscal) launch_spmm<double, true, true>(ctx, lvl, vals9, x, y, mscal, y2, w);
    else if (vals9) {
        launch_spmm<double, false, true>(ctx, lvl, vals9, x, y, nullptr, nullptr, w);
    }
    else launch_spmm<double, true, false>(ctx, lvl, nullptr, x, nullptr, mscal, y2, w);
}

void mh_spmm_mapped(mh_context *ctx, const BsrLevel &lvl, const double *vals9, const double *x, double *y, const double *mscal, double *y2, uint32_t w, uint32_t ldy,
                    uint32_t wreal, const uint32_t *omap, const double *res_theta, double *res_out, double *res_partial, const double *res_dinv) {
    if (w == 0 || wreal == 0) return;
    ResidualEpilogue res;
    if (res_out && w <= 128) {
        res.theta = res_theta;
        res.r_out = res_out;
        res.partial = res_partial;
        res.dinv = res_dinv;
    } else if (res_out) {
        mh_throw(MH_EINVAL, "residual epilogue needs a panel of at most 128 columns (got %u)", w);
    }
    if (w % 2 || (reinterpret_cast<uintptr_t>(x) & 15)) mh_throw(MH_EINVAL, "mapped product needs an even pitch and an aligned panel (got %u)", w);
    constexpr int xcd = 1;
    const unsigned grid = (div_up(lvl.n_nodes, TB / 64) + 7) / 8 * 8;
    const uint32_t ranges = div_up(w, 128u), step = (div_up(w, ranges) + 1u) & ~1u;
    for (uint32_t c0 = 0; c0 < wreal; c0 += step) {
        const uint32_t wc = std::min(step, w - c0), wr = std::min(wc, wreal - c0);
        TimedLaunch timed(ctx, MH_KERNEL_SPMM, spmm_bytes(lvl, wr, 8, 8, 8, true, true) + (res.r_out ? 8.0 * double(wr) * (3.0 + 2.0) * double(lvl.n_nodes) : 0.0));
        auto go = [&](auto cl_tag) {
            constexpr int CL = decltype(cl_tag)::value;
            k_spmm_wide<double, double, double, 2, CL, true, true, true><<<grid, TB, 0, ctx->stream>>>(lvl.row_ptr, lvl.col, vals9, mscal, x + c0, y, y2, lvl.n_nodes, wc, xcd, ldy, wr, omap + c0,
                                                                                                  ChebStep{}, w, res);
        };
        const uint32_t lanes = wc / 2;
        if (lanes <= 8) go(std::integral_constant<int, 8>{});
        else if (lanes <= 16) go(std::integral_constant<int, 16>{});
        else if (lanes <= 32) go(std::integral_constant<int, 32>{});
        else go(std::integral_constant<int, 64>{});
        KERNEL_CHECK();
    }
}

bool mh_spmm_f32_cheb_step(mh_context *ctx, const BsrLevel &lvl, const float *d_in, float *d_out, float *r, float *x, const float *dinv, float c1, float c2, uint32_t w) {
    if (w == 0) return true;
    const bool aligned16 = !((reinterpret_cast<uintptr_t>(d_in) | reinterpret_cast<uintptr_t>(d_out) | reinterpret_cast<uintptr_t>(r) | reinterpret_cast<uintptr_t>(x)) & 15);
    if (w % 4 || w > 256 || !aligned16) return false;
    TimedLaunch timed(ctx, MH_KERNEL_SPMM, spmm_bytes(lvl, w, 4, 4, 0, true, false) + 5.0 * 4.0 * 3.0 * double(lvl.n_nodes) * w);
    constexpr int xcd = 1;
    const unsigned grid = (div_up(lvl.n_nodes, TB / 64) + 7) / 8 * 8;
    ChebStep epi;
    epi.r = r; epi.dinv = dinv; epi.d_out = d_out; epi.x = x; epi.c1 = c1; epi.c2 = c2;
    auto go = [&](auto cl_tag) {
        constexpr int CL = decltype(cl_tag)::value;
        if (latency_bound_level(lvl))
            k_spmm_wide<float, float, float, 4, CL, false, true, false, 1, 4, true><<<grid, TB, 0, ctx->stream>>>(lvl.row_ptr, lvl.col, lvl.aval32.get(), static_cast<const float *>(nullptr), d_in,
                                                                                                                static_cast<float *>(nullptr), static_cast<float *>(nullptr), lvl.n_nodes, w, xcd, 0, 0, nullptr, epi);
        else
            k_spmm_wide<float, float, float, 4, CL, false, true, false, 1><<<grid, TB, 0, ctx->stream>>>(lvl.row_ptr, lvl.col, lvl.aval32.get(), static_cast<const float *>(nullptr), d_in,
                                                                                                       static_cast<float *>(nullptr), static_cast<float *>(nullptr), lvl.n_nodes, w, xcd, 0, 0, nullptr, epi);
    };
    const uint32_t lanes = w / 4;
    if (lanes <= 8) go(std::integral_constant<int, 8>{});
    else if (lanes <= 16) go(std::integral_constant<int, 16>{});
    else if (lanes <= 20) go(std::integral_constant<int, 20>{});
    else if (lanes <= 32) go(std::integral_constant<int, 32>{});
    else go(std::integral_constant<int, 64>{});
    KERNEL_CHECK();
    return true;
}

void mh_spmm_f32(mh_context *ctx, const BsrLevel &lvl, const float *x, float *y, uint32_t w) {
    if (w == 0) return;
    TimedLaunch timed(ctx, MH_KERNEL_SPMM, spmm_bytes(lvl, w, 4, 4, 4, true, false));
    launch_spmm<float, false, true>(ctx, lvl, lvl.aval32.get(), x, y, static_cast<const float *>(nullptr), static_cast<float *>(nullptr), w);
}

void mh_spmm_mixed(mh_context *ctx, const BsrLevel &lvl, const float *x, double *y, uint32_t w) {
    if (w == 0) return;
    TimedLaunch timed(ctx, MH_KERNEL_SPMM, spmm_bytes(lvl, w, 8, 4, 8, true, false));
    if (!launch_spmm_wide<double, float, double, false, true>(ctx, lvl, lvl.aval.get(), x, y, static_cast<const double *>(nullptr), static_cast<double *>(nullptr), w))
        mh_throw(MH_EINVAL, "mixed-precision product needs a 16-byte aligned panel of pitch %% 4 == 0 (got %u)", w);
}
```

Measured before the change: 611.2 eigenpairs/s.

## Defer host syncs, fuse Chebyshev init into first step, and dual-write combine output

```diff
diff --git a/mesheditor_amd/csrc/mh_common.h b/mesheditor_amd/csrc/mh_common.h
--- a/mesheditor_amd/csrc/mh_common.h
+++ b/mesheditor_amd/csrc/mh_common.h
@@ -498,9 +498,10 @@
 template<typename T>
 void mh_apply_patches(mh_context *ctx, const PatchSet &ps, const T *in, const T *minus, uint32_t w, T coef, T *d, T *x, double *z, uint32_t wz, T *scratch);
 void mh_gram(mh_context *ctx, size_t n, const double *x, uint32_t wa, const double *y, uint32_t wb, double *g, uint32_t ld, uint32_t ldy = 0, const uint32_t *ymap = nullptr);
-void mh_combine(mh_context *ctx, size_t n, const double *x, uint32_t wx, const double *w, uint32_t ww, const double *p, uint32_t wp, const double *ct, uint32_t nc,
+bool mh_combine(mh_context *ctx, size_t n, const double *x, uint32_t wx, const double *w, uint32_t ww, const double *p, uint32_t wp, const double *ct, uint32_t nc,
                 double *out1, uint32_t n1, double *out2, bool accumulate = false, uint32_t ldx = 0, const uint32_t *xmap = nullptr, uint32_t ld1 = 0,
-                const uint32_t *omap = nullptr, uint32_t col_begin = 0, uint32_t col_count = 0);
+                const uint32_t *omap = nullptr, uint32_t col_begin = 0, uint32_t col_count = 0, double *out1b = nullptr, uint32_t ld1b = 0,
+                const uint32_t *omapb = nullptr);
 bool mh_tridiag_lowest_wide(mh_context *ctx, const double *d, const double *e, uint32_t m, uint32_t k, double *w, double *z, uint32_t ldz, double *work, int *info2,
                             double *quality_host);
 void mh_apply_q(mh_context *ctx, const double *a, const double *tau, uint32_t m, double *z, uint32_t ldz, uint32_t ncols);
@@ -532,7 +533,8 @@
                     uint32_t wreal, const uint32_t *omap, const double *res_theta = nullptr, double *res_out = nullptr, double *res_partial = nullptr,
                     const double *res_dinv = nullptr);
 bool mh_spmm_f32_cheb_step(mh_context *ctx, const BsrLevel &lvl, const float *d_in, float *d_out, float *r, float *x, const float *dinv, float c1, float c2,
-                           uint32_t w);
+                           uint32_t w, const float *r_in = nullptr, const float *x_in = nullptr);
+bool mh_spmm_f32_cheb_step_serves(const float *d_in, const float *d_out, const float *r, const float *x, uint32_t w);
 void mh_spmm_f32(mh_context *ctx, const BsrLevel &lvl, const float *x, float *y, uint32_t w);
 void mh_spmm_mixed(mh_context *ctx, const BsrLevel &lvl, const float *x, double *y, uint32_t w);
 const uint32_t *mh_identity_map(mh_context *ctx);
diff --git a/mesheditor_amd/csrc/mh_dense.hip b/mesheditor_amd/csrc/mh_dense.hip
--- a/mesheditor_amd/csrc/mh_dense.hip
+++ b/mesheditor_amd/csrc/mh_dense.hip
@@ -193,7 +193,8 @@
 __global__ void __launch_bounds__(256) k_combine(const double *__restrict__ X, int wx, int ldx, const uint32_t *__restrict__ xmap, const double *__restrict__ W, int ww,
                                                 const double *__restrict__ P, int wp,
                                                 const double *__restrict__ Ct, int ldc, int c0, int nc, size_t n, double *__restrict__ out1, int n1,
-                                                double *__restrict__ out2, size_t split_stride, int ld1, const uint32_t *__restrict__ omap) {
+                                                double *__restrict__ out2, size_t split_stride, int ld1, const uint32_t *__restrict__ omap, double *out1b = nullptr,
+                                                int ld1b = 0, const uint32_t *__restrict__ omapb = nullptr) {
     extern __shared__ __attribute__((aligned(16))) double smem[];
     const int m = wx + ww + wp;
     const int kslice = (((m + int(gridDim.y) - 1) / int(gridDim.y)) + CK - 1) / CK * CK;
@@ -226,9 +227,14 @@
     const int col_l = lane & 15, row_l = lane >> 4;
     const int pitch2 = ldc - n1;
     uint32_t ocol[MAPPED ? NT : 1];
+    uint32_t ocolb[MAPPED ? NT : 1];
     if (MAPPED) {
 #pragma unroll
         for (int t = 0; t < NT; ++t) ocol[t] = omap[min(c0 + 16 * t + col_l, max(n1, 1) - 1)] * 8u;
+        if (out1b) {
+#pragma unroll
+            for (int t = 0; t < NT; ++t) ocolb[t] = omapb[min(c0 + 16 * t + col_l, max(n1, 1) - 1)] * 8u;
+        }
     }
     double ps[SJ], pc[NT];
     const size_t tiles = (n + 63) / 64;
@@ -303,6 +309,7 @@
                 else if (s0 >= n1) dst = reinterpret_cast<double *>(row2 + 128 * t);
                 else dst = s0 + col_l < n1 ? reinterpret_cast<double *>(row1 + (MAPPED ? size_t(ocol[t]) : size_t(128 * t))) : reinterpret_cast<double *>(row2 + 128 * t);
                 *dst = ACCUMULATE ? *dst + acc[t][reg] : acc[t][reg];
+                if (MAPPED && out1b && s0 + col_l < n1) *reinterpret_cast<double *>(reinterpret_cast<char *>(out1b + r * size_t(ld1b)) + ocolb[t]) = acc[t][reg];
             }
         }
     }
@@ -445,11 +452,12 @@
     return ctx->iota;
 }
 
-void mh_combine(mh_context *ctx, size_t n, const double *x, uint32_t wx, const double *w, uint32_t ww, const double *p, uint32_t wp, const double *ct, uint32_t nc,
+bool mh_combine(mh_context *ctx, size_t n, const double *x, uint32_t wx, const double *w, uint32_t ww, const double *p, uint32_t wp, const double *ct, uint32_t nc,
                 double *out1, uint32_t n1, double *out2, bool accumulate, uint32_t ldx, const uint32_t *xmap, uint32_t ld1, const uint32_t *omap, uint32_t col_begin,
-                uint32_t col_count) {
-    if (!nc) return;
+                uint32_t col_count, double *out1b, uint32_t ld1b, const uint32_t *omapb) {
+    if (!nc) return false;
     if (!col_count) { col_begin = 0; col_count = nc; }
+    if (out1b && (!xmap || !omapb || !ld1b)) mh_throw(MH_EINVAL, "combine: the second copy of out1 needs a column map on X and a map and a pitch of its own");
     const bool caller_omap = omap != nullptr;
     if (col_begin + col_count > nc) mh_throw(MH_EINVAL, "combine: columns %u + %u exceed %u", col_begin, col_count, nc);
     const bool mapped = xmap != nullptr;
@@ -492,8 +500,9 @@
         if (col_begin < n1) emit(out1 + col_begin, ld1 ? ld1 : n1, col_begin, std::min(c_end, n1) - col_begin);
         if (c_end > n1) emit(out2 + (std::max(col_begin, n1) - n1), nc - n1, std::max(col_begin, n1), c_end - std::max(col_begin, n1));
         if (mapped) HIP_CHECK(hipStreamSynchronize(ctx->stream));
-        return;
-    }
+        return false;
+    }
+    if (col_count > 256) out1b = nullptr;
     const uint32_t chunks = div_up(col_count, 256), step = (div_up(col_count, chunks) + 15) / 16 * 16;
     for (uint32_t c0 = col_begin; c0 < col_begin + col_count; c0 += step) {
         const uint32_t ncc = std::min(step, col_begin + col_count - c0);
@@ -506,7 +515,7 @@
             const unsigned grid = unsigned(std::min<size_t>(div_up(n, 64), size_t(per_cu) * ctx->cu_count));
 #define MH_COMBINE_ARGS x, int(wx), int(ldx ? ldx : wx), xmap, w, int(ww), p, int(wp), ct, int(nc), int(c0), int(ncc), n, out1, int(n1), out2, 0, int(ld1 ? ld1 : n1), omap
             if (accumulate) k_combine<NT, true, false><<<grid, 256, lds, ctx->stream>>>(MH_COMBINE_ARGS);
-            else if (mapped) k_combine<NT, false, true><<<grid, 256, lds_m, ctx->stream>>>(MH_COMBINE_ARGS);
+            else if (mapped) k_combine<NT, false, true><<<grid, 256, lds_m, ctx->stream>>>(MH_COMBINE_ARGS, out1b, int(ld1b), omapb);
             else k_combine<NT, false, false><<<grid, 256, lds, ctx->stream>>>(MH_COMBINE_ARGS);
 #undef MH_COMBINE_ARGS
         };
@@ -523,6 +532,7 @@
         }
         KERNEL_CHECK();
     }
+    return out1b != nullptr;
 }
 
 namespace {
diff --git a/mesheditor_amd/csrc/mh_eigs.hip b/mesheditor_amd/csrc/mh_eigs.hip
--- a/mesheditor_amd/csrc/mh_eigs.hip
+++ b/mesheditor_amd/csrc/mh_eigs.hip
@@ -32,6 +32,8 @@
     bool lmax_low = getenv("MH_TEST") && strstr(getenv("MH_TEST"), "lmax_low");
     bool potrf_chain = getenv("MH_TEST") && strstr(getenv("MH_TEST"), "potrf_chain");
     bool no_poly_start = getenv("MH_TEST") && strstr(getenv("MH_TEST"), "no_poly_start");
+    bool eager_readbacks = getenv("MH_TEST") && strstr(getenv("MH_TEST"), "eager_readbacks");
+    bool qr_explicit = getenv("MH_TEST") && strstr(getenv("MH_TEST"), "qr_explicit");
     Switches() {
         if (const char *c = getenv("MH_CYCLE")) {
             double v[5] = {0, 0, 0, 0, 0};
@@ -127,6 +129,47 @@
         (void)hipEventDestroy(b);
     }
 };
+struct SpanTimer {
+    static constexpr size_t kPairs = 32;
+    mh_context *ctx;
+    std::vector<hipEvent_t> ev;
+    size_t used = 0;
+    double total = 0;
+    explicit SpanTimer(mh_context *c) : ctx(c) {}
+    SpanTimer(const SpanTimer &) = delete;
+    SpanTimer &operator=(const SpanTimer &) = delete;
+    void begin() {
+        if (used == kPairs) drain();
+        while (ev.size() < 2 * (used + 1)) {
+            hipEvent_t e;
+            HIP_CHECK(hipEventCreate(&e));
+            ev.push_back(e);
+        }
+        HIP_CHECK(hipEventRecord(ev[2 * used], ctx->stream));
+    }
+    void end() {
+        HIP_CHECK(hipEventRecord(ev[2 * used + 1], ctx->stream));
+        ++used;
+        if (switches().eager_readbacks) HIP_CHECK(hipEventSynchronize(ev[2 * used - 1]));
+    }
+    void drain() {
+        if (!used) return;
+        HIP_CHECK(hipEventSynchronize(ev[2 * used - 1]));
+        for (size_t k = 0; k < used; ++k) {
+            float ms = 0;
+            HIP_CHECK(hipEventElapsedTime(&ms, ev[2 * k], ev[2 * k + 1]));
+            total += ms * 1e-3;
+        }
+        used = 0;
+    }
+    double seconds() {
+        drain();
+        return total;
+    }
+    ~SpanTimer() {
+        for (hipEvent_t e : ev) (void)hipEventDestroy(e);
+    }
+};
 
 __global__ void k_random_panel(double *__restrict__ x, size_t count, uint64_t seed) {
     const size_t i = size_t(blockIdx.x) * blockDim.x + threadIdx.x;
@@ -197,6 +240,16 @@
     r[i] = rv;
     d[i] = dv;
     x[i] = dv;
+}
+__global__ void k_cheb_init_convert2(const double *__restrict__ src, uint32_t ws, const float *__restrict__ dinv, float inv_theta, float *__restrict__ b32,
+                                     float *__restrict__ d, size_t rows, uint32_t w) {
+    const size_t i = size_t(blockIdx.x) * blockDim.x + threadIdx.x;
+    if (i >= rows * w) return;
+    const size_t row = i / w;
+    const uint32_t c = uint32_t(i % w);
+    const float rv = c < ws ? float(src[row * ws + c]) : 0.f;
+    b32[i] = rv;
+    d[i] = dinv[row] * rv * inv_theta;
 }
 template<typename T>
 __global__ void k_cheb_step(const T *__restrict__ t, const T *__restrict__ dinv, T c1, T c2, T *__restrict__ r, T *__restrict__ d, T *__restrict__ x, size_t rows,
@@ -637,10 +690,12 @@
     DevArray<double> zl(ctx, partial ? size_t(m) * nwant : 0);
     double *zres = z.get();
     uint32_t ncols = m;
+    bool back_transformed = false;
     HIP_CHECK(hipMemcpyAsync(z.get(), gA, size_t(m) * m * sizeof(double), hipMemcpyDeviceToDevice, ctx->stream));
     for (int attempt = 0; attempt < 2; ++attempt) {
         mh_sytrd_small(ctx, gA, m, evals, ework, tau, attempt == 0 ? -1 : 0);
         int gave_up = 0;
+        back_transformed = false;
         const bool flagged = attempt == 0 && ctx->sytrd_flag;
         if (flagged) HIP_CHECK(hipMemcpyAsync(&gave_up, ctx->sytrd_flag, sizeof(int), hipMemcpyDeviceToHost, ctx->stream));
         if (partial) {
@@ -651,6 +706,8 @@
                 std::vector<double> lam_host(host_evals ? nwant : 0);
                 HIP_CHECK(hipMemcpyAsync(qv, wv.get() + m, sizeof(qv), hipMemcpyDeviceToHost, ctx->stream));
                 if (host_evals) HIP_CHECK(hipMemcpyAsync(lam_host.data(), wv.get(), size_t(nwant) * sizeof(double), hipMemcpyDeviceToHost, ctx->stream));
+                back_transformed = !switches().eager_readbacks;
+                if (back_transformed) mh_apply_q(ctx, gA, tau, m, zout, m, nwant);
                 HIP_CHECK(hipStreamSynchronize(ctx->stream));
                 if (flagged && sytrd_gave_up(ctx, gave_up, gA, z, m)) continue;
                 if (switches().verbose)
@@ -662,6 +719,7 @@
                     zres = zout, ncols = nwant;
                     break;
                 }
+                back_transformed = false;
             }
         }
         if (flagged) {
@@ -673,7 +731,7 @@
         break;
     }
     if (ctx->rr_trace) ctx->rr_trace->solver = ncols < m ? MhRrTrace::SMALL_PARTIAL : MhRrTrace::SMALL_STEDC;
-    mh_apply_q(ctx, gA, tau, m, zres, m, ncols);
+    if (!back_transformed) mh_apply_q(ctx, gA, tau, m, zres, m, ncols);
     if (zres == zl.get()) rr_selfcheck(ctx, z.get(), m, zres, m, evals, ncols);
     HIP_CHECK(hipMemcpyAsync(gA, zres, size_t(m) * ncols * sizeof(double), hipMemcpyDeviceToDevice, ctx->stream));
     return 0;
@@ -856,8 +914,12 @@
         double rho = 1.0 / sig;
         const T *dinv = dinv_of(lvl);
         if (!zero_init) spmm(lvl, x, t, w);
+        const PatchSet &ps = patches_of(lvl);
+        bool first_reads_inputs = false;
         if constexpr (!kDouble) {
-            if (b_src && zero_init) k_cheb_init_convert<<<grid1(rows * w), TB, 0, ctx->stream>>>(b_src, w_src, dinv, float(1.0 / theta), b_copy, r, d, x, rows, w);
+            first_reads_inputs = b_src && zero_init && !ps.any() && deg >= 2 && !(z_out && deg == 2) && mh_spmm_f32_cheb_step_serves(d, t, r, x, w);
+            if (first_reads_inputs) k_cheb_init_convert2<<<grid1(rows * w), TB, 0, ctx->stream>>>(b_src, w_src, dinv, float(1.0 / theta), b_copy, d, rows, w);
+            else if (b_src && zero_init) k_cheb_init_convert<<<grid1(rows * w), TB, 0, ctx->stream>>>(b_src, w_src, dinv, float(1.0 / theta), b_copy, r, d, x, rows, w);
             else k_cheb_init_v4<<<grid1(rows * (w / 4)), TB, 0, ctx->stream>>>(reinterpret_cast<const f4_t *>(b), zero_init ? nullptr : reinterpret_cast<const f4_t *>(t), dinv,
                                                                                float(1.0 / theta), reinterpret_cast<f4_t *>(r), reinterpret_cast<f4_t *>(d),
                                                                                reinterpret_cast<f4_t *>(x), zero_init ? 0 : 1, rows, w / 4);
@@ -865,8 +927,7 @@
             k_cheb_init<T><<<grid1(rows * w), TB, 0, ctx->stream>>>(b, zero_init ? nullptr : t, dinv, T(1.0 / theta), r, d, x, zero_init ? 0 : 1, rows, w);
         }
         KERNEL_CHECK();
-        const PatchSet &ps = patches_of(lvl);
-        mh_apply_patches<T>(ctx, ps, r, nullptr, w, T(1.0 / theta), d, x, nullptr, 0, patch_y.get());
+        if (!first_reads_inputs) mh_apply_patches<T>(ctx, ps, r, nullptr, w, T(1.0 / theta), d, x, nullptr, 0, patch_y.get());
         constexpr bool fuse_steps = true;
         T *cur = d, *alt = t;
         for (int k = 1; k < deg; ++k) {
@@ -874,7 +935,10 @@
             const bool last = z_out && k + 1 == deg;
             bool fused = false;
             if constexpr (!kDouble) {
-                if (fuse_steps && !last) fused = mh_spmm_f32_cheb_step(ctx, lvl, cur, alt, r, x, dinv, float(rho_new * rho), float(2 * rho_new / delta), w);
+                const bool separate = first_reads_inputs && k == 1;
+                if (fuse_steps && !last)
+                    fused = mh_spmm_f32_cheb_step(ctx, lvl, cur, alt, r, x, dinv, float(rho_new * rho), float(2 * rho_new / delta), w, separate ? b_copy : nullptr, separate ? cur : nullptr);
+                if (separate && !fused) mh_throw(MH_EHIP, "Chebyshev smoother: the fused first step was refused for a panel of %u columns", w);
             }
             if (fused) {
                 std::swap(cur, alt);
@@ -902,7 +966,7 @@
         }
     }
     void apply(const double *r_in, double *z_out, uint32_t w_in) {
-        mh_finish_hierarchy(sys);
+        if (switches().eager_readbacks) mh_finish_hierarchy(sys);
         const uint32_t w = pitch(w_in);
         const uint32_t nn = sys->n_nodes, np = sys->n_points, na = sys->n_agg;
         const size_t n2 = size_t(3) * nn, n1 = size_t(3) * np, n0 = size_t(6) * na;
@@ -933,11 +997,13 @@
                 k_restrict_agg<double><<<grid1(n0 * w), TB, 0, ctx->stream>>>(r1d.get(), t1d.get(), sys->agg_t, r0, sys->agg_ptr, sys->agg_nodes, na, w);
             }
             KERNEL_CHECK();
+            mh_finish_hierarchy(sys);
             mh_short_product(ctx, n0, sys->a0, uint32_t(n0), r0, w, x0, x0_partial, COARSE_SLICES);
             k_prolong_agg<T><<<grid1(n1 * w), TB, 0, ctx->stream>>>(x0, sys->agg_t, x1.get(), sys->agg_of, np, w);
             KERNEL_CHECK();
             cheb(sys->L1, deg1, r1, x1, false, rr1, d1, t1, w);
         }
+        mh_finish_hierarchy(sys);
         if constexpr (kDouble) k_prolong_p1<T><<<grid1(n2 * w), TB, 0, ctx->stream>>>(x1.get(), sys->parent_a, sys->parent_b, z, nn, w);
         else k_prolong_p1_v4<<<grid1(n2 * (w / 4)), TB, 0, ctx->stream>>>(reinterpret_cast<const f4_t *>(x1.get()), sys->parent_a, sys->parent_b, reinterpret_cast<f4_t *>(z), nn, w / 4);
         KERNEL_CHECK();
@@ -1032,15 +1098,15 @@
     }
     mh_finish_hierarchy(sys);
     hipStream_t main_stream = ctx->stream;
-    for (BsrLevel *lvl : {&sys->L2, &sys->L1}) {
+    auto shifted_level = [&](BsrLevel *lvl) {
         lvl->aval.reset(ctx, lvl->n_blocks * 9);
         lvl->dinv.reset(ctx, size_t(3) * lvl->n_nodes);
         k_shift_values<<<grid1(lvl->n_blocks * 9), TB, 0, ctx->stream>>>(lvl->kval, lvl->mval, lvl->n_blocks, sigma, lvl->aval);
         KERNEL_CHECK();
         k_diag_inverse<<<grid1(lvl->n_nodes), TB, 0, ctx->stream>>>(lvl->row_ptr, lvl->col, lvl->aval, lvl->n_nodes, lvl->dinv);
         KERNEL_CHECK();
-        mh_build_patch_inverses(ctx, *lvl, lvl->id == 2 ? sys->patches2 : sys->patches1);
-    }
+    };
+    shifted_level(&sys->L1);
     const size_t n0 = size_t(6) * sys->n_agg;
     sys->a0.reset(ctx, n0 * n0);
     sys->a0.zero();
@@ -1141,6 +1207,9 @@
         if (!sys->coarse_done) HIP_CHECK(hipEventCreateWithFlags(&sys->coarse_done, hipEventDisableTiming));
         HIP_CHECK(hipEventRecord(sys->coarse_done, side ? ctx->aux_stream : main_stream));
         sys->coarse_pending = true;
+        shifted_level(&sys->L2);
+        mh_build_patch_inverses(ctx, sys->L2, sys->patches2);
+        mh_build_patch_inverses(ctx, sys->L1, sys->patches1);
         smoother_setup();
         if (side) (void)hipEventDestroy(forked);
     }
@@ -1292,7 +1361,7 @@
     mh_profile *profile;
     SharedPhase iterating;
     Timer t_iter;
-    double precond_seconds = 0;
+    SpanTimer t_precond;
     double best_worst_active = 1e300;
     int floor_strikes = 0;
     std::vector<double> hist_active;
@@ -1319,6 +1388,8 @@
     bool w_implicit = false;
     int last_spread = 1 << 20;
     bool p_needs_explicit = false;
+    bool rr_prefilled = false;
+    bool qr_explicit_pending = switches().qr_explicit;
     uint32_t wp = 0;
     uint32_t iters = 0, nconv = 0, redos_at_start = 0;
     bool poly_allowed = true;
@@ -1336,7 +1407,7 @@
                 uint32_t seed_cols_, const volatile unsigned char *cancel_, volatile float *progress_, mh_profile &prof_, mh_profile *profile_, int inner_cg_ = 0)
         : sys(system), ctx(system->ctx), st(system->ctx->stream), n(size_t(3) * system->n_nodes), nev(nev_), b(block), mmax(3 * block), sigma(sigma_), residual_tol(residual_tol_),
           max_iters(max_iters_), seed_basis(seed_basis_), seed_rows(seed_rows_), seed_cols(seed_cols_), cancel(cancel_), progress(progress_), prof(prof_), profile(profile_),
-          iterating(system->ctx->device, true), t_iter(system->ctx), pproj_ok(block <= 128), scaled_norms(system->patches2.any()), theta(block), rn(block), mn(block), xn(block), norms(3 * size_t(block)),
+          iterating(system->ctx->device, true), t_iter(system->ctx), t_precond(system->ctx), pproj_ok(block <= 128), scaled_norms(system->patches2.any()), theta(block), rn(block), mn(block), xn(block), norms(3 * size_t(block)),
           theta_act(block), order(block), locked(block, 0) {
         inner_cg = inner_cg_;
         for (DevArray<double> *panel : {&X, &AX, &MX, &Xn, &AXn, &MXn, &W, &AW, &MW, &P, &Pn, &R, &Rw}) panel->reset(ctx, n * b);
@@ -1386,16 +1457,21 @@
         double *Gs = G.get() + size_t(w) * w;
         int hinfo = 0;
         bool fused_inverse = false;
+        bool speculated = false;
+        rr_prefilled = false;
         {
             last_spread = 1 << 20;
             if (w <= 128) {
                 fused_inverse = !switches().potrf_chain;
                 if (fused_inverse) mh_potrf_small_inverse(ctx, Gs, w, info, dscale, Linv);
                 else mh_potrf_small(ctx, Gs, w, info);
+                speculated = allow_implicit && !transform_images && !switches().eager_readbacks;
+                if (speculated) rr_tall_blocks(hp != nullptr);
                 int both[2] = {0, 0};
                 info.download(both, 2);
                 hinfo = both[0];
                 last_spread = both[1];
+                if (hp && qr_explicit_pending) last_spread = std::max(last_spread, 16 * 8), qr_explicit_pending = false;
             } else {
                 mh_potrf(ctx, Gs, w, w, info);
                 info.download(&hinfo, 1);
@@ -1421,6 +1497,7 @@
                 ROCBLAS_CHECK(rocblas_dtrtri(ctx->blas, rocblas_fill_lower, rocblas_diagonal_non_unit, w, Gs, w, Linv, w));
             }
             w_implicit = allow_implicit && !transform_images && last_spread < 16 * 8;
+            rr_prefilled = speculated && w_implicit;
             if (!w_implicit) mh_combine(ctx, n, V, w, nullptr, 0, nullptr, 0, Linv, w, V, w, nullptr);
             if (MV && transform_images) mh_combine(ctx, n, MV, w, nullptr, 0, nullptr, 0, Linv, w, MV, w, nullptr);
             if (AV && transform_images) mh_combine(ctx, n, AV, w, nullptr, 0, nullptr, 0, Linv, w, AV, w, nullptr);
@@ -1493,11 +1570,11 @@
         if (!warm) {
             {
                 mh_spmm(ctx, sys->L2, nullptr, X, nullptr, sys->L2.mval, MX, b);
-                Timer tp(ctx);
+                t_precond.begin();
                 precondition(MX, Xn, b);
-                precond_seconds += tp.stop();
+                t_precond.end();
                 prof.op_applications += b;
-                HIP_CHECK(hipMemcpyAsync(X, Xn.get(), n * b * sizeof(double), hipMemcpyDeviceToDevice, st));
+                std::swap(X, Xn);
             }
             if (seed_rigid) inject_rigid_modes();
         }
@@ -1646,9 +1723,9 @@
         for (uint32_t k = 0; k < w; ++k) theta_act[k] = theta[act[k]];
         theta_act_d.upload(theta_act.data(), w);
         {
-            Timer tp(ctx);
+            t_precond.begin();
             precondition(residuals, W, w);
-            precond_seconds += tp.stop();
+            t_precond.end();
             prof.op_applications += w;
         }
         bool ok = true;
@@ -1686,21 +1763,30 @@
         }
     }
 
+    void rr_tall_blocks(bool with_p) {
+        wa = w;
+        m = wa + w + wp;
+        HIP_CHECK(hipMemsetAsync(gA, 0, size_t(m) * m * sizeof(double), st));
+        HIP_CHECK(hipMemsetAsync(gM, 0, size_t(m) * m * sizeof(double), st));
+        k_set_identity_blocks<<<grid1(wa), TB, 0, st>>>(gA, gM, theta_act_d, wa, m);
+        KERNEL_CHECK();
+        mh_gram(ctx, n, W, w, AX, wa, gA.get() + wa, m, b, idx_d);
+        gram(ctx, n, W, w, AW, w, gA.get() + size_t(wa) * m + wa, m);
+        if (with_p && wp) gram(ctx, n, P, wp, AW, w, gA.get() + size_t(wa) * m + wa + w, m);
+    }
+
     void rayleigh_ritz(uint32_t it) {
         wa = w;
         m = wa + w + wp;
         for (int attempt = 0; attempt < 2; ++attempt) {
-            HIP_CHECK(hipMemsetAsync(gA, 0, size_t(m) * m * sizeof(double), st));
-            HIP_CHECK(hipMemsetAsync(gM, 0, size_t(m) * m * sizeof(double), st));
-            k_set_identity_blocks<<<grid1(wa), TB, 0, st>>>(gA, gM, theta_act_d, wa, m);
-            KERNEL_CHECK();
+            if (!(attempt == 0 && rr_prefilled)) rr_tall_blocks(p_implicit);
+            rr_prefilled = false;
             const double unit_one = 1;
             auto left_corrected = [&](double *block, uint32_t cols) {
                 if (w_implicit)
                     ROCBLAS_CHECK(rocblas_dtrmm(ctx->blas, rocblas_side_left, rocblas_fill_lower, rocblas_operation_none, rocblas_diagonal_non_unit, rocblas_int(w),
                                                 rocblas_int(cols), &unit_one, Linv, rocblas_int(w), block, rocblas_int(m), block, rocblas_int(m)));
             };
-            mh_gram(ctx, n, W, w, AX, wa, gA.get() + wa, m, b, idx_d);
             left_corrected(gA.get() + wa, wa);
             const double unit = 1;
             auto untransformed = [&](double *block, uint32_t rows) {
@@ -1708,11 +1794,9 @@
                     ROCBLAS_CHECK(rocblas_dtrmm(ctx->blas, rocblas_side_right, rocblas_fill_lower, rocblas_operation_transpose, rocblas_diagonal_non_unit, rocblas_int(rows),
                                                 rocblas_int(w), &unit, Linv, rocblas_int(w), block, rocblas_int(m), block, rocblas_int(m)));
             };
-            gram(ctx, n, W, w, AW, w, gA.get() + size_t(wa) * m + wa, m);
             if (p_implicit && wp) {
                 const double plus = 1, nil = 0;
                 double *bw = gA.get() + size_t(wa) * m + wa, *bp = gA.get() + size_t(wa) * m + wa + w;
-                gram(ctx, n, P, wp, AW, w, bp, m);
                 small_dgemm(ctx, rocblas_operation_transpose, rocblas_operation_none, rocblas_int(w), rocblas_int(w), rocblas_int(wp), &plus, Hp, rocblas_int(wp), bp,
                                             rocblas_int(m), &nil, Up, rocblas_int(w));
                 small_dgemm(ctx, rocblas_operation_none, rocblas_operation_none, rocblas_int(wp), rocblas_int(w), rocblas_int(wp), &plus, App, rocblas_int(wp), Hp,
@@ -1817,9 +1901,10 @@
                 ROCBLAS_CHECK(rocblas_dgemm(ctx->blas, rocblas_operation_none, rocblas_operation_transpose, pitchc, rocblas_int(wp), rocblas_int(w), &minus, rows_w, pitchc, Hp,
                                             rocblas_int(wp), &plus, rows_p, pitchc));
             }
-            mh_combine(ctx, n, X, wa, W, w, P, wp, Ct, wa + wp_new, Xn, wa, Pn, false, b, idx_d, pitch);
+            const bool x_written = mh_combine(ctx, n, X, wa, W, w, P, wp, Ct, wa + wp_new, Xn, wa, Pn, false, b, idx_d, pitch, nullptr, 0, 0, X, b, idx_d);
             if (wp_new && !pproj_ok) mh_spmm(ctx, sys->L2, nullptr, Pn, nullptr, sys->L2.mval, MPn, wp_new);
-            if (pitch == wa) k_scatter_cols<<<grid1(n * wa), TB, 0, st>>>(Xn.get(), idx_d, X.get(), n, b, wa);
+            if (x_written) {}
+            else if (pitch == wa) k_scatter_cols<<<grid1(n * wa), TB, 0, st>>>(Xn.get(), idx_d, X.get(), n, b, wa);
             else k_scatter_cols_pitch<<<grid1(n * wa), TB, 0, st>>>(Xn.get(), pitch, idx_d, X.get(), n, b, wa);
             KERNEL_CHECK();
             if (Rr.count) {
@@ -1843,7 +1928,7 @@
 
     void finish(double *eigenvalues) {
         prof.restarts = iters;
-        prof.op_solve = precond_seconds;
+        prof.op_solve = t_precond.seconds();
         if (!converged) mh_throw(MH_ENOTCONVERGED, "LOBPCG: %u of %u pairs converged in %u iterations", nconv, nev, iters);
         for (uint32_t k = 0; k < nev; ++k) eigenvalues[k] = theta[order[k]] + sigma;
         sys->plain_residual = -1.0;
diff --git a/mesheditor_amd/csrc/mh_spmm.hip b/mesheditor_amd/csrc/mh_spmm.hip
--- a/mesheditor_amd/csrc/mh_spmm.hip
+++ b/mesheditor_amd/csrc/mh_spmm.hip
@@ -92,6 +92,7 @@
 }
 
 struct ChebStep {
+    const float *r_in = nullptr, *x_in = nullptr;
     float *r = nullptr;
     const float *dinv = nullptr;
     float *d_out = nullptr;
@@ -138,9 +139,9 @@
             const size_t o = size_t(3) * row * w + coff;
 #pragma unroll
             for (int i = 0; i < 3; ++i) {
-                er[i] = *reinterpret_cast<const Acc *>(epi.r + o + size_t(i) * w);
+                er[i] = *reinterpret_cast<const Acc *>(epi.r_in + o + size_t(i) * w);
                 ed[i] = __builtin_convertvector(*reinterpret_cast<const Vec *>(x + o + size_t(i) * w), Acc);
-                ex[i] = *reinterpret_cast<const Acc *>(epi.x + o + size_t(i) * w);
+                ex[i] = *reinterpret_cast<const Acc *>(epi.x_in + o + size_t(i) * w);
                 edinv[i] = epi.dinv[size_t(3) * row + i];
             }
         }
@@ -251,9 +252,9 @@
                     dv = epi.c1 * ed[i] + (epi.c2 * edinv[i]) * rv;
                     xn = ex[i] + dv;
                 } else {
-                    rv = *reinterpret_cast<const Acc *>(epi.r + oi) - acc[i];
+                    rv = *reinterpret_cast<const Acc *>(epi.r_in + oi) - acc[i];
                     dv = epi.c1 * __builtin_convertvector(*reinterpret_cast<const Vec *>(x + oi), Acc) + (epi.c2 * epi.dinv[size_t(3) * row + i]) * rv;
-                    xn = *reinterpret_cast<const Acc *>(epi.x + oi) + dv;
+                    xn = *reinterpret_cast<const Acc *>(epi.x_in + oi) + dv;
                 }
                 *reinterpret_cast<Acc *>(epi.r + oi) = rv;
                 *reinterpret_cast<Acc *>(epi.d_out + oi) = dv;
@@ -435,15 +436,22 @@
     }
 }
 
-bool mh_spmm_f32_cheb_step(mh_context *ctx, const BsrLevel &lvl, const float *d_in, float *d_out, float *r, float *x, const float *dinv, float c1, float c2, uint32_t w) {
+bool mh_spmm_f32_cheb_step_serves(const float *d_in, const float *d_out, const float *r, const float *x, uint32_t w) {
+    const bool aligned16 = !((reinterpret_cast<uintptr_t>(d_in) | reinterpret_cast<uintptr_t>(d_out) | reinterpret_cast<uintptr_t>(r) | reinterpret_cast<uintptr_t>(x)) & 15);
+    return !(w % 4 || w > 256 || !aligned16);
+}
+bool mh_spmm_f32_cheb_step(mh_context *ctx, const BsrLevel &lvl, const float *d_in, float *d_out, float *r, float *x, const float *dinv, float c1, float c2, uint32_t w, const float *r_in,
+                           const float *x_in) {
     if (w == 0) return true;
-    const bool aligned16 = !((reinterpret_cast<uintptr_t>(d_in) | reinterpret_cast<uintptr_t>(d_out) | reinterpret_cast<uintptr_t>(r) | reinterpret_cast<uintptr_t>(x)) & 15);
-    if (w % 4 || w > 256 || !aligned16) return false;
+    if (!mh_spmm_f32_cheb_step_serves(d_in, d_out, r, x, w)) return false;
+    if (!r_in) r_in = r;
+    if (!x_in) x_in = x;
+    if ((reinterpret_cast<uintptr_t>(r_in) | reinterpret_cast<uintptr_t>(x_in)) & 15) mh_throw(MH_EINVAL, "Chebyshev step: the separate inputs are not 16-byte aligned");
     TimedLaunch timed(ctx, MH_KERNEL_SPMM, spmm_bytes(lvl, w, 4, 4, 0, true, false) + 5.0 * 4.0 * 3.0 * double(lvl.n_nodes) * w);
     constexpr int xcd = 1;
     const unsigned grid = (div_up(lvl.n_nodes, TB / 64) + 7) / 8 * 8;
     ChebStep epi;
-    epi.r = r; epi.dinv = dinv; epi.d_out = d_out; epi.x = x; epi.c1 = c1; epi.c2 = c2;
+    epi.r_in = r_in; epi.x_in = x_in; epi.r = r; epi.dinv = dinv; epi.d_out = d_out; epi.x = x; epi.c1 = c1; epi.c2 = c2;
     auto go = [&](auto cl_tag) {
         constexpr int CL = decltype(cl_tag)::value;
         if (latency_bound_level(lvl))
```

Result: no change. 610.0 eigenpairs/s (-0.2%).
